# Hongyang-Du/VideoGPA

Measured on AMD Instinct MI355X. Metric: DPO preference-pair steps/sec, CogVideoX-5B 49f@480x720, higher is better.
Workload: dtype bf16; 1 GPU; BASELINE configs[1]: CogVideoX-5B T2V full (42 blocks, D=3072, 48x64 heads), 49f x 480x720 -> paired latents [1,2,13,16,60,90], S=17776 tokens, 42 blocks, LoRA r=64 on to_q/to_k/to_v/to_out.0, 1 pair/GPU/step, optimizer step every step; random-init weights; layers=42, pairs_per_gpu=1, parallelism=dp1

## Files before the change

### include/videogpa_hip.h

```cpp
#ifndef VIDEOGPA_HIP_H
#define VIDEOGPA_HIP_H

#include <stddef.h>
#include <stdint.h>

#ifdef __cplusplus
extern "C" {
#endif

typedef struct ihipStream_t* vgpa_stream_t;

#define VGPA_OK 0
#define VGPA_ERR_INVALID (-1)
#define VGPA_ERR_LAUNCH (-2)
#define VGPA_ERR_WORKSPACE (-3)

size_t vgpa_dpo_loss_workspace_bytes(int64_t B);
int32_t vgpa_dpo_loss_fwd(const void* v_win, const void* v_lose, const void* v_win_ref, const void* v_lose_ref,
                          const void* tgt_win, const void* tgt_lose, int64_t B, int64_t N, int64_t stride_pred,
                          int64_t stride_ref, int64_t stride_tgt, int32_t dtype, float beta, float label_smoothing,
                          int32_t loss_type, int32_t flags, float* out5, float* dlogit, float* errs, void* workspace,
                          size_t ws_bytes, vgpa_stream_t stream);
int32_t vgpa_dpo_loss_bwd(const void* v_win, const void* v_lose, const void* tgt_win, const void* tgt_lose, int64_t B,
                          int64_t N, int64_t stride_pred, int64_t stride_tgt, int64_t stride_grad, int32_t dtype, float beta,
                          int32_t flags, const float* dlogit, const float* grad_out, void* grad_win, void* grad_lose,
                          vgpa_stream_t stream);

int32_t vgpa_noise_velocity_paired(const void* x_pair, const void* noise, const int64_t* t, const float* sqrt_abar,
                                   const float* sqrt_1m_abar, int64_t B, int64_t N, int32_t num_train_timesteps,
                                   int32_t dtype, void* x_noisy_pair, void* v_target_pair, vgpa_stream_t stream);

int32_t vgpa_flow_noise_velocity_paired(const void* x_pair, const void* noise, const float* sigma, int64_t B, int64_t N,
                                        int32_t dtype, int32_t xt_f32, void* x_noisy_pair, void* v_target_pair,
                                        vgpa_stream_t stream);

int32_t vgpa_ln_modulate_fwd(const void* x, const float* ln_w, const float* ln_b, const float* shift_v,
                             const float* scale1p_v, const float* shift_t, const float* scale1p_t, int64_t mod_stride,
                             int64_t B, int64_t S, int64_t D, int64_t text_len, float eps, void* out, float* mean,
                             float* rstd, vgpa_stream_t stream);
int32_t vgpa_ln_modulate_bwd(const void* dy, const void* x, const float* mean, const float* rstd, const float* ln_w,
                             const float* scale1p_v, const float* scale1p_t, int64_t mod_stride, int64_t B, int64_t S,
                             int64_t D, int64_t text_len, const void* dres, void* dx, vgpa_stream_t stream);
int32_t vgpa_residual_ln_fwd(const void* x, const void* y, const float* gate_v, const float* gate_t, int64_t gate_stride,
                             const float* ln_w, const float* ln_b, const float* shift_v, const float* scale1p_v,
                             const float* shift_t, const float* scale1p_t, int64_t mod_stride, int64_t B, int64_t S, int64_t D,
                             int64_t text_len, float eps, void* x_new, void* n_out,
                             int64_t n_stride ,
                             float* mean, float* rstd, vgpa_stream_t stream);
int32_t vgpa_residual_ln_bwd(const void* dn, const void* x_new, const float* mean, const float* rstd, const float* ln_w,
                             const float* scale1p_v, const float* scale1p_t, int64_t mod_stride, const float* gate_v,
                             const float* gate_t, int64_t gate_stride, const void* dres, int64_t B, int64_t S, int64_t D,
                             int64_t text_len, void* dx, void* dy, int64_t dy_stride ,
                             vgpa_stream_t stream);
int32_t vgpa_residual_ln_fwd_q8(const void* x, const void* y, const float* gate_v, const float* gate_t, int64_t gate_stride,
                                const float* ln_w, const float* ln_b, const float* shift_v, const float* scale1p_v,
                                const float* shift_t, const float* scale1p_t, int64_t mod_stride, int64_t B, int64_t S, int64_t D,
                                int64_t text_len, float eps, void* x_new, void* q8, float* q8_scale, float* mean, float* rstd,
                                vgpa_stream_t stream);
int32_t vgpa_residual_ln_bwd_q8(const void* dn, const void* x_new, const float* mean, const float* rstd, const float* ln_w,
                                const float* scale1p_v, const float* scale1p_t, int64_t mod_stride, const float* gate_v,
                                const float* gate_t, int64_t gate_stride, const void* dres, int64_t B, int64_t S, int64_t D,
                                int64_t text_len, void* dx, void* dy_q8, float* dy_scale, vgpa_stream_t stream);
int32_t vgpa_gate_residual(const void* x, const void* y, const float* gate_v, const float* gate_t, int64_t mod_stride,
                           int64_t B, int64_t S, int64_t D, int64_t text_len, void* out, vgpa_stream_t stream);
int32_t vgpa_gelu_tanh_fwd(const void* u, int64_t n, void* out, vgpa_stream_t stream);
int32_t vgpa_gelu_tanh_bwd(const void* u, const void* dy, int64_t n, void* du, vgpa_stream_t stream);

int32_t vgpa_qknorm_rope_fwd(const void* q_in, const void* k_in, void* q_out, void* k_out, const int64_t* qin_strides,
                             const int64_t* kin_strides, const int64_t* qout_strides, const int64_t* kout_strides,
                             const float* wq, const float* bq, const float* wk, const float* bk, const float* rope_cos,
                             const float* rope_sin, int64_t text_len, int64_t B, int64_t H, int64_t S, int64_t head_dim,
                             float eps, float q_out_scale, int32_t rope_mode, vgpa_stream_t stream);
int32_t vgpa_qknorm_rope_bwd(const void* dq_out, const void* dk_out, const void* q_in, const void* k_in, void* dq_in,
                             void* dk_in, const int64_t* dqout_strides, const int64_t* dkout_strides,
                             const int64_t* qin_strides, const int64_t* kin_strides, const int64_t* dqin_strides,
                             const int64_t* dkin_strides, const float* wq, const float* wk, const float* rope_cos,
                             const float* rope_sin, int64_t text_len, int64_t B, int64_t H, int64_t S, int64_t head_dim,
                             float eps, int32_t rope_mode, vgpa_stream_t stream);

int32_t vgpa_attn_bwd_delta_res(const void* o, const void* o_res, int32_t res_kind, const void* d_o, const int64_t* o_strides, const int64_t* ores_strides,
                                const int64_t* do_strides, float* delta, int64_t B, int64_t H, int64_t S, int64_t head_dim,
                                vgpa_stream_t stream);
size_t vgpa_attn_bwd_split_workspace_bytes(int64_t B, int64_t H, int64_t S);
int32_t vgpa_attn_bwd_dq_w1(const void* q, const void* k, const void* v, const void* d_o, const float* lse2, const float* delta,
                            void* dq, const int64_t* q_strides, const int64_t* k_strides, const int64_t* v_strides,
                            const int64_t* do_strides, const int64_t* dq_strides, int64_t B, int64_t H, int64_t S, int64_t head_dim,
                            float scale, int32_t split_mode, void* workspace, size_t ws_bytes, vgpa_stream_t stream);
size_t vgpa_attn_fwd_w1_workspace_bytes(int64_t B, int64_t H, int64_t S);
#define VGPA_RES_NONE 0
#define VGPA_RES_BF16 1
#define VGPA_RES_8 2
int32_t vgpa_attn_fwd_w1_res(const void* q, const void* k, const void* v, void* o, void* o_res, int32_t res_kind, float* lse2, const int64_t* q_strides,
                             const int64_t* k_strides, const int64_t* v_strides, const int64_t* o_strides, const int64_t* ores_strides,
                             int64_t B, int64_t H, int64_t S, int64_t head_dim, float scale, int32_t split_mode, void* workspace,
                             size_t ws_bytes, vgpa_stream_t stream);
int32_t vgpa_attn_fwd_online_res(const void* q, const void* k, const void* v, void* o, void* o_res, int32_t res_kind, float* lse2, const int64_t* q_strides,
                                 const int64_t* k_strides, const int64_t* v_strides, const int64_t* o_strides, const int64_t* ores_strides,
                                 int64_t B, int64_t H, int64_t S, int64_t head_dim, float scale, int32_t split_mode, void* workspace,
                                 size_t ws_bytes, vgpa_stream_t stream);
int32_t vgpa_attn_bwd_prep_w1_res(const void* o, const void* o_res, int32_t res_kind, const void* d_o, const float* lse2, const int64_t* o_strides,
                                  const int64_t* ores_strides, const int64_t* do_strides, float* delta, float* stats, int64_t B, int64_t H,
                                  int64_t S, int64_t head_dim, vgpa_stream_t stream);
int32_t vgpa_attn_bwd_dkv_w1(const void* q, const void* k, const void* v, const void* d_o, const float* stats, void* dk, void* dv,
                             const int64_t* q_strides, const int64_t* k_strides, const int64_t* v_strides, const int64_t* do_strides,
                             const int64_t* dk_strides, const int64_t* dv_strides, int64_t B, int64_t H, int64_t S, int64_t head_dim,
                             float scale, int32_t split_mode, void* workspace, size_t ws_bytes, vgpa_stream_t stream);

int32_t vgpa_lora_down(const void* X, int64_t ldx, const void* A, void* T, int64_t ldt, int64_t M, int64_t K, int64_t R,
                       vgpa_stream_t stream);
int32_t vgpa_lora_up_add(void* Y, int64_t ldy, const void* T, int64_t ldt, const void* Bw, int64_t ldb, float s, int64_t M,
                         int64_t N, int64_t rp, int32_t accumulate, vgpa_stream_t stream);
size_t vgpa_lora_grad_workspace_bytes(int64_t M, int64_t P, int64_t Q);
int32_t vgpa_lora_grad_ws(const void* U, int64_t ldu, const void* V, int64_t ldv, float* G, int64_t ldg, float s, int64_t M,
                          int64_t P, int64_t Q, void* workspace, size_t ws_bytes, vgpa_stream_t stream);
int32_t vgpa_lora_ext_refresh(const float* A, const float* B, float s, int64_t r, int64_t K, int64_t Dn, void* a_cat, void* wt_tail, int64_t ld_wt,
                              void* w_tail, int64_t ld_w, void* sbt, vgpa_stream_t stream);

#ifdef VGPA_VARIANTS
int32_t vgpa_gemm_bf16(const void* X, int64_t ldx, const void* W, int64_t ldw, const void* bias, void* C, int64_t ldc, void* aux,
                       int64_t ldaux, int32_t M, int32_t N, int32_t K, int32_t epilogue, vgpa_stream_t stream);
#endif

size_t vgpa_attn128_fwd_workspace_bytes(int64_t B, int64_t H, int64_t Sq);
int32_t vgpa_attn128_fwd(const void* q, const void* k, const void* v, void* o, float* lse2, const int64_t* q_strides, const int64_t* k_strides,
                         const int64_t* v_strides, const int64_t* o_strides, void* o_res8, const int64_t* ores_strides, int64_t B, int64_t H,
                         int64_t Sq, int64_t Skv, float scale, void* workspace, size_t ws_bytes, vgpa_stream_t stream);
size_t vgpa_attn128_fwd_f8_workspace_bytes(int64_t B, int64_t H, int64_t Sq, int64_t Skv);
int32_t vgpa_attn128_fwd_f8(const void* q, const void* k, const void* v, void* o, float* lse2, const int64_t* q_strides, const int64_t* k_strides,
                            const int64_t* v_strides, const int64_t* o_strides, void* o_res8, const int64_t* ores_strides, void* q_deq, void* k_deq,
                            void* v_deq, const int64_t* qd_strides, const int64_t* kd_strides, const int64_t* vd_strides, int64_t B, int64_t H,
                            int64_t Sq, int64_t Skv, float scale, void* workspace, size_t ws_bytes, vgpa_stream_t stream);
size_t vgpa_attn128_bwd_workspace_bytes(int64_t B, int64_t H, int64_t Sq);
int32_t vgpa_attn128_bwd(const void* q, const void* k, const void* v, const void* o, const void* d_o, const float* lse2, void* dq, void* dk,
                         void* dv, const int64_t* q_strides, const int64_t* k_strides, const int64_t* v_strides,
                         const int64_t* o_strides, const int64_t* do_strides, const int64_t* dq_strides, const int64_t* dk_strides,
                         const int64_t* dv_strides, const void* o_res8, const int64_t* ores_strides, int64_t B, int64_t H, int64_t Sq, int64_t Skv,
                         float scale, int32_t dkv_mode, void* workspace, size_t ws_bytes, vgpa_stream_t stream);
int32_t vgpa_attn128_bwd_prescaled(const void* q, const void* k, const void* v, const void* o, const void* d_o, const float* lse2, void* dq, void* dk,
                                   void* dv, const int64_t* q_strides, const int64_t* k_strides, const int64_t* v_strides,
                                   const int64_t* o_strides, const int64_t* do_strides, const int64_t* dq_strides, const int64_t* dk_strides,
                                   const int64_t* dv_strides, const void* o_res8, const int64_t* ores_strides, int64_t B, int64_t H, int64_t Sq, int64_t Skv,
                                   float scale, int32_t dkv_mode, void* workspace, size_t ws_bytes, vgpa_stream_t stream);

int32_t vgpa_wan_ln_mod_fwd(const void* x, int32_t x_dtype, const void* y, const float* gate, float* x_out, const int32_t* gid, const float* ln_w,
                            const float* ln_b, const float* shift, const float* scale, int64_t mod_stride, int64_t rows, int64_t D, float eps,
                            int32_t round_xhat, void* out, int32_t out_dtype, int64_t out_ld, void* q8, float* q8_scale, float* mean, float* rstd,
                            vgpa_stream_t stream);
int32_t vgpa_wan_ln_mod_bwd(const void* dy, int32_t dy_dtype, const void* x, int32_t x_dtype, const float* mean, const float* rstd, const int32_t* gid,
                            const float* ln_w, const float* scale, int64_t mod_stride, int64_t rows, int64_t D, const float* dres, float* dx,
                            const float* gate_prev, void* dy_prev, int64_t ld_dy_prev, vgpa_stream_t stream);
int32_t vgpa_wan_gate_residual(const float* x, const void* y, const int32_t* gid, const float* gate, int64_t mod_stride, int64_t rows, int64_t D, float* out,
                               vgpa_stream_t stream);
int32_t vgpa_wan_gate_bwd(const float* dout, const int32_t* gid, const float* gate, int64_t mod_stride, int64_t rows, int64_t D, void* dy, int64_t ld_dy,
                          vgpa_stream_t stream);
int32_t vgpa_wan_gate_bwd_q8(const float* dout, const int32_t* gid, const float* gate, int64_t mod_stride, int64_t rows, int64_t D, void* q8,
                             float* q8_scale, vgpa_stream_t stream);
int32_t vgpa_wan_rms_rope_fwd(const void* u, int64_t ld_u, const void* w, const float* rope_cos, const float* rope_sin, int64_t L, int64_t head_dim,
                              int64_t rows, int64_t D, float eps, void* out, int64_t ld_out, float* rstd, vgpa_stream_t stream);
int32_t vgpa_wan_rms_rope_bwd(const void* dout, int64_t ld_dout, const void* u, int64_t ld_u, const float* rstd, const void* w, const float* rope_cos,
                              const float* rope_sin, int64_t L, int64_t head_dim, int64_t rows, int64_t D, void* du, int64_t ld_du, vgpa_stream_t stream);

int32_t vgpa_quant_fp8_rows(const void* x, int64_t ldx, void* q, float* scale, int64_t M, int64_t K, vgpa_stream_t stream);
int32_t vgpa_gelu_tanh_fwd_q8(const void* u, int64_t rows, int64_t K, void* q8, float* q8_scale, vgpa_stream_t stream);
int32_t vgpa_gelu_tanh_bwd_q8(const void* u, const void* dy, int64_t rows, int64_t K, void* q8, float* q8_scale, vgpa_stream_t stream);

int32_t vgpa_preprocess_shape(int32_t H, int32_t W, int32_t mode, int32_t* out_h, int32_t* out_w);
size_t vgpa_preprocess_workspace_bytes(int32_t T, int32_t H, int32_t W, int32_t mode);
int32_t vgpa_preprocess_frames(const void* frames, int32_t T, int32_t H, int32_t W, int32_t mode, float* out, void* workspace,
                               size_t ws_bytes, vgpa_stream_t stream);

size_t vgpa_grad_norm_workspace_bytes(void);
int32_t vgpa_grad_norm(const float* grad, int64_t n, float grad_scale, float* norm_out, void* workspace, size_t ws_bytes,
                       vgpa_stream_t stream);
int32_t vgpa_adamw_step(float* param, const float* grad, float* exp_avg, float* exp_avg_sq, int64_t n, float lr, float beta1,
                        float beta2, float eps, float weight_decay, int64_t step, float grad_scale, float max_norm,
                        const float* total_norm, vgpa_stream_t stream);

size_t vgpa_project_points_workspace_bytes(int64_t T, int64_t H, int64_t W);
int32_t vgpa_project_points(const float* pc, const float* colors, const float* conf, float conf_thr,
                            const float* conf_thr_dev , const float* K,
                            const float* E, int32_t e_rows, int64_t N, int64_t T, int64_t H, int64_t W, uint8_t* canvas,
                            float* out_f, void* workspace, size_t ws_bytes, vgpa_stream_t stream);
int32_t vgpa_motion_score(const float* E, int32_t e_rows, int64_t T, float* out, vgpa_stream_t stream);
int32_t vgpa_epipolar_sampson(const float* p1, const float* p2, const int64_t* offsets, int64_t n_pairs, float* err_out,
                              float* F_out, vgpa_stream_t stream);

size_t vgpa_conf_threshold_workspace_bytes(void);
int32_t vgpa_conf_threshold(const float* conf, int64_t N, float conf_thres, float* thr_out, void* workspace, size_t ws_bytes,
                            vgpa_stream_t stream);
size_t vgpa_frame_metric_workspace_bytes(void);
int32_t vgpa_frame_metric(const void* gt, int32_t gt_dtype, int32_t gt_layout, int32_t gt_is_tensor, const void* rep,
                          int32_t rep_dtype, int32_t rep_layout, int32_t rep_is_tensor, int64_t T, int64_t C, int64_t H,
                          int64_t W, int64_t H2, int64_t W2, int32_t psnr, float* out, void* workspace, size_t ws_bytes,
                          vgpa_stream_t stream);
size_t vgpa_frame_ssim_workspace_bytes(int64_t T, int64_t C, int64_t H, int64_t W);
int32_t vgpa_frame_ssim(const void* gt, int32_t gt_dtype, int32_t gt_layout, int32_t gt_is_tensor, const void* rep, int32_t rep_dtype,
                        int32_t rep_layout, int32_t rep_is_tensor, int64_t T, int64_t C, int64_t H, int64_t W, int32_t downsample,
                        float* out_per_frame, float* out_mean, void* workspace, size_t ws_bytes, vgpa_stream_t stream);
int32_t vgpa_frames_to_pm1(const void* src, int32_t dtype, int32_t layout, int32_t is_tensor, int64_t T, int64_t C, int64_t H,
                           int64_t W, int64_t Ho, int64_t Wo, float* out, void* workspace, size_t ws_bytes, vgpa_stream_t stream);
size_t vgpa_mvcs_workspace_bytes(int64_t T);
int32_t vgpa_mvcs(const float* depth, const float* K, int32_t k_dim, const float* E, int32_t e_rows, int64_t T, int64_t H,
                  int64_t W, float* out, void* workspace, size_t ws_bytes, vgpa_stream_t stream);
int32_t vgpa_unproject_depth(const float* depth, const float* K, const float* E, int32_t e_rows, int64_t T, int64_t H,
                             int64_t W, float* world, vgpa_stream_t stream);
int32_t vgpa_pose_decode(const float* pose_enc, int64_t n, float image_h, float image_w, float* ext, float* intr,
                         vgpa_stream_t stream);

int32_t vgpa_conv3x3_f32(const float* x, const float* w_packed, const float* bias, const float* res, const float* res2, float* out,
                         int64_t N, int64_t H, int64_t W, int64_t Cin, int64_t Cout, int64_t stride, int32_t flags,
                         vgpa_stream_t stream);
int32_t vgpa_conv1x1_f32(const float* x, const float* w_packed, const float* bias, float* out, int64_t M, int64_t Cin, int64_t Cout,
                         vgpa_stream_t stream);
int32_t vgpa_dpt_tail_f32(const float* x, const float* xtab, const float* ytab, const float* w1_packed, const float* b1,
                          const float* w2, const float* b2, float* preds, float* conf, int64_t N, int64_t h, int64_t w, int64_t C,
                          int64_t H, int64_t W, int32_t output_dim, int32_t activation, vgpa_stream_t stream);
int32_t vgpa_upsample_bilinear_ac_f32(const float* x, const float* xtab, const float* ytab, float* out, int64_t N, int64_t h,
                                      int64_t w, int64_t C, int64_t H, int64_t W, vgpa_stream_t stream);
int32_t vgpa_attn_small_f32(const float* q, const float* k, const float* v, int64_t stride_b, int64_t stride_h, int64_t stride_s,
                            float* o, int64_t B, int64_t H, int64_t S, int64_t D, float scale, vgpa_stream_t stream);

int32_t vgpa_dino_embed(const void* images, int32_t in_dtype, const float* w_packed, int64_t k_packed, const float* bias,
                        const float* cls_token, const float* register_tokens, const float* pos, void* out, int32_t out_dtype, int64_t N,
                        int64_t H, int64_t W, int64_t patch, int64_t C, int64_t R, vgpa_stream_t stream);
int32_t vgpa_stream_ln_f32(const float* x, const void* y, const float* gamma, const float* ln_w, const float* ln_b, float* x_new, void* n,
                           int32_t n_dtype, int64_t M, int64_t D, float eps, vgpa_stream_t stream);

int32_t vgpa_lpips_input_f32(const float* x, float* out, int64_t N, int64_t H, int64_t W, float shift0, float shift1, float shift2,
                             float scale0, float scale1, float scale2, int32_t flags, vgpa_stream_t stream);
int32_t vgpa_maxpool2x2_f32(const float* x, float* out, int64_t N, int64_t H, int64_t W, int64_t C, int32_t flags, vgpa_stream_t stream);
size_t vgpa_lpips_layer_workspace_bytes(int64_t N, int64_t H, int64_t W, int64_t C);
int32_t vgpa_lpips_layer_f32(const float* f0, const float* f1, const float* w, float* out, double* total, int64_t N, int64_t H, int64_t W,
                             int64_t C, int32_t flags, void* workspace, size_t ws_bytes, vgpa_stream_t stream);

int32_t vgpa_da3_ref_view(const float* x, int64_t B, int64_t S, int64_t N, int64_t C, int32_t strategy, double* metrics, int32_t* ref_idx,
                          vgpa_stream_t stream);
int32_t vgpa_da3_view_gather(const float* a_in, float* a_out, const float* b_in, float* b_out, const int32_t* ref_idx, int32_t inverse, int64_t B,
                             int64_t S, int64_t N, int64_t C, vgpa_stream_t stream);
int32_t vgpa_da3_cam_token(float* x, const float* cam, int32_t per_view, int64_t B, int64_t S, int64_t N, int64_t C, vgpa_stream_t stream);
int32_t vgpa_da3_tap(const float* local_x, const float* x, const float* ln_w, const float* ln_b, float eps, const int32_t* ref_idx, float* feats,
                     float* cam, int64_t B, int64_t S, int64_t N, int64_t C, vgpa_stream_t stream);
int32_t vgpa_da3_pose_decode(const float* pose_enc, int64_t n, float image_h, float image_w, float* ext, float* intr, vgpa_stream_t stream);
int32_t vgpa_dualdpt_aux_tail_f32(const float* x, const float* xtab, const float* ytab, const float* w1_packed, const float* b1,
                                  const float* ln_w, const float* ln_b, float eps, const float* w2, const float* b2, float* preds, float* conf,
                                  int64_t N, int64_t h, int64_t w, int64_t C, int32_t output_dim, vgpa_stream_t stream);

#ifdef __cplusplus
}
#endif
#endif
```

### videogpa_amd/_lib.py

```python
import ctypes
import os

import torch

from ctypes import c_float, c_int32, c_int64, c_size_t, c_void_p

_HERE = os.path.dirname(os.path.abspath(__file__))
LIB_PATH = os.environ.get("VGPA_LIB") or os.path.join(_HERE, "csrc", "libvgpa_hip.so")

P, I64, I32, F32, SZ = c_void_p, c_int64, c_int32, c_float, c_size_t

SIGNATURES = {
    "vgpa_dpo_loss_workspace_bytes": (SZ, [I64]),
    "vgpa_dpo_loss_fwd": (I32, [P, P, P, P, P, P, I64, I64, I64, I64, I64, I32, F32, F32, I32, I32, P, P, P, P, SZ, P]),
    "vgpa_dpo_loss_bwd": (I32, [P, P, P, P, I64, I64, I64, I64, I64, I32, F32, I32, P, P, P, P, P]),
    "vgpa_noise_velocity_paired": (I32, [P, P, P, P, P, I64, I64, I32, I32, P, P, P]),
    "vgpa_flow_noise_velocity_paired": (I32, [P, P, P, I64, I64, I32, I32, P, P, P]),
    "vgpa_ln_modulate_fwd": (I32, [P, P, P, P, P, P, P, I64, I64, I64, I64, I64, F32, P, P, P, P]),
    "vgpa_ln_modulate_bwd": (I32, [P, P, P, P, P, P, P, I64, I64, I64, I64, I64, P, P, P]),
    "vgpa_residual_ln_fwd": (I32, [P, P, P, P, I64, P, P, P, P, P, P, I64, I64, I64, I64, I64, F32, P, P, I64, P, P, P]),
    "vgpa_residual_ln_bwd": (I32, [P, P, P, P, P, P, P, I64, P, P, I64, P, I64, I64, I64, I64, P, P, I64, P]),
    "vgpa_residual_ln_fwd_q8": (I32, [P, P, P, P, I64, P, P, P, P, P, P, I64, I64, I64, I64, I64, F32, P, P, P, P, P, P]),
    "vgpa_residual_ln_bwd_q8": (I32, [P, P, P, P, P, P, P, I64, P, P, I64, P, I64, I64, I64, I64, P, P, P, P]),
    "vgpa_gate_residual": (I32, [P, P, P, P, I64, I64, I64, I64, I64, P, P]),
    "vgpa_gelu_tanh_fwd": (I32, [P, I64, P, P]),
    "vgpa_gelu_tanh_bwd": (I32, [P, P, I64, P, P]),
    "vgpa_qknorm_rope_fwd": (I32, [P, P, P, P, P, P, P, P, P, P, P, P, P, P, I64, I64, I64, I64, I64, F32, F32, I32, P]),
    "vgpa_qknorm_rope_bwd": (I32, [P, P, P, P, P, P, P, P, P, P, P, P, P, P, P, P, I64, I64, I64, I64, I64, F32, I32, P]),
    "vgpa_grad_norm_workspace_bytes": (SZ, []),
    "vgpa_grad_norm": (I32, [P, I64, F32, P, P, SZ, P]),
    "vgpa_adamw_step": (I32, [P, P, P, P, I64, F32, F32, F32, F32, F32, I64, F32, F32, P, P]),
    "vgpa_attn_bwd_delta_res": (I32, [P, P, I32, P, P, P, P, P, I64, I64, I64, I64, P]),
    "vgpa_attn_bwd_dq_w1": (I32, [P, P, P, P, P, P, P, P, P, P, P, P, I64, I64, I64, I64, F32, I32, P, SZ, P]),
    "vgpa_attn_fwd_w1_workspace_bytes": (SZ, [I64, I64, I64]),
    "vgpa_attn_bwd_prep_w1_res": (I32, [P, P, I32, P, P, P, P, P, P, P, I64, I64, I64, I64, P]),
    "vgpa_attn_fwd_w1_res": (I32, [P, P, P, P, P, I32, P, P, P, P, P, P, I64, I64, I64, I64, F32, I32, P, SZ, P]),
    "vgpa_attn_fwd_online_res": (I32, [P, P, P, P, P, I32, P, P, P, P, P, P, I64, I64, I64, I64, F32, I32, P, SZ, P]),
    "vgpa_attn_bwd_dkv_w1": (I32, [P, P, P, P, P, P, P, P, P, P, P, P, P, I64, I64, I64, I64, F32, I32, P, SZ, P]),
    "vgpa_attn_bwd_split_workspace_bytes": (SZ, [I64, I64, I64]),
    "vgpa_lora_down": (I32, [P, I64, P, P, I64, I64, I64, I64, P]),
    "vgpa_lora_up_add": (I32, [P, I64, P, I64, P, I64, F32, I64, I64, I64, I32, P]),
    "vgpa_lora_grad_workspace_bytes": (SZ, [I64, I64, I64]),
    "vgpa_lora_grad_ws": (I32, [P, I64, P, I64, P, I64, F32, I64, I64, I64, P, SZ, P]),
    "vgpa_lora_ext_refresh": (I32, [P, P, F32, I64, I64, I64, P, P, I64, P, I64, P, P]),
    "vgpa_attn128_fwd_workspace_bytes": (SZ, [I64, I64, I64]),
    "vgpa_attn128_fwd": (I32, [P, P, P, P, P, P, P, P, P, P, P, I64, I64, I64, I64, F32, P, SZ, P]),
    "vgpa_attn128_fwd_f8_workspace_bytes": (SZ, [I64, I64, I64, I64]),
    "vgpa_attn128_fwd_f8": (I32, [P] * 17 + [I64, I64, I64, I64, F32, P, SZ, P]),
    "vgpa_attn128_bwd_workspace_bytes": (SZ, [I64, I64, I64]),
    "vgpa_attn128_bwd": (I32, [P] * 19 + [I64, I64, I64, I64, F32, I32, P, SZ, P]),
    "vgpa_attn128_bwd_prescaled": (I32, [P] * 19 + [I64, I64, I64, I64, F32, I32, P, SZ, P]),
    "vgpa_wan_ln_mod_fwd": (I32, [P, I32, P, P, P, P, P, P, P, P, I64, I64, I64, F32, I32, P, I32, I64, P, P, P, P, P]),
    "vgpa_wan_ln_mod_bwd": (I32, [P, I32, P, I32, P, P, P, P, P, I64, I64, I64, P, P, P, P, I64, P]),
    "vgpa_wan_gate_residual": (I32, [P, P, P, P, I64, I64, I64, P, P]),
    "vgpa_wan_gate_bwd": (I32, [P, P, P, I64, I64, I64, P, I64, P]),
    "vgpa_wan_gate_bwd_q8": (I32, [P, P, P, I64, I64, I64, P, P, P]),
    "vgpa_wan_rms_rope_fwd": (I32, [P, I64, P, P, P, I64, I64, I64, I64, F32, P, I64, P, P]),
    "vgpa_wan_rms_rope_bwd": (I32, [P, I64, P, I64, P, P, P, P, I64, I64, I64, I64, P, I64, P]),
    "vgpa_quant_fp8_rows": (I32, [P, I64, P, P, I64, I64, P]),
    "vgpa_gelu_tanh_fwd_q8": (I32, [P, I64, I64, P, P, P]),
    "vgpa_gelu_tanh_bwd_q8": (I32, [P, P, I64, I64, P, P, P]),
    "vgpa_preprocess_shape": (I32, [I32, I32, I32, P, P]),
    "vgpa_preprocess_workspace_bytes": (SZ, [I32, I32, I32, I32]),
    "vgpa_preprocess_frames": (I32, [P, I32, I32, I32, I32, P, P, SZ, P]),
    "vgpa_project_points_workspace_bytes": (SZ, [I64, I64, I64]),
    "vgpa_project_points": (I32, [P, P, P, F32, P, P, P, I32, I64, I64, I64, I64, P, P, P, SZ, P]),
    "vgpa_conf_threshold_workspace_bytes": (SZ, []),
    "vgpa_conf_threshold": (I32, [P, I64, F32, P, P, SZ, P]),
    "vgpa_frame_metric_workspace_bytes": (SZ, []),
    "vgpa_frame_metric": (I32, [P, I32, I32, I32, P, I32, I32, I32, I64, I64, I64, I64, I64, I64, I32, P, P, SZ, P]),
    "vgpa_frame_ssim_workspace_bytes": (SZ, [I64, I64, I64, I64]),
    "vgpa_frame_ssim": (I32, [P, I32, I32, I32, P, I32, I32, I32, I64, I64, I64, I64, I32, P, P, P, SZ, P]),
    "vgpa_frames_to_pm1": (I32, [P, I32, I32, I32, I64, I64, I64, I64, I64, I64, P, P, SZ, P]),
    "vgpa_mvcs_workspace_bytes": (SZ, [I64]),
    "vgpa_mvcs": (I32, [P, P, I32, P, I32, I64, I64, I64, P, P, SZ, P]),
    "vgpa_unproject_depth": (I32, [P, P, P, I32, I64, I64, I64, P, P]),
    "vgpa_pose_decode": (I32, [P, I64, F32, F32, P, P, P]),
    "vgpa_motion_score": (I32, [P, I32, I64, P, P]),
    "vgpa_epipolar_sampson": (I32, [P, P, P, I64, P, P, P]),
    "vgpa_conv3x3_f32": (I32, [P, P, P, P, P, P, I64, I64, I64, I64, I64, I64, I32, P]),
    "vgpa_conv1x1_f32": (I32, [P, P, P, P, I64, I64, I64, P]),
    "vgpa_dpt_tail_f32": (I32, [P, P, P, P, P, P, P, P, P, I64, I64, I64, I64, I64, I64, I32, I32, P]),
    "vgpa_upsample_bilinear_ac_f32": (I32, [P, P, P, P, I64, I64, I64, I64, I64, I64, P]),
    "vgpa_attn_small_f32": (I32, [P, P, P, I64, I64, I64, P, I64, I64, I64, I64, F32, P]),
    "vgpa_dino_embed": (I32, [P, I32, P, I64, P, P, P, P, P, I32, I64, I64, I64, I64, I64, I64, P]),
    "vgpa_stream_ln_f32": (I32, [P, P, P, P, P, P, P, I32, I64, I64, F32, P]),
    "vgpa_lpips_input_f32": (I32, [P, P, I64, I64, I64, F32, F32, F32, F32, F32, F32, I32, P]),
    "vgpa_maxpool2x2_f32": (I32, [P, P, I64, I64, I64, I64, I32, P]),
    "vgpa_lpips_layer_workspace_bytes": (SZ, [I64, I64, I64, I64]),
    "vgpa_lpips_layer_f32": (I32, [P, P, P, P, P, I64, I64, I64, I64, I32, P, SZ, P]),
    "vgpa_da3_ref_view": (I32, [P, I64, I64, I64, I64, I32, P, P, P]),
    "vgpa_da3_view_gather": (I32, [P, P, P, P, P, I32, I64, I64, I64, I64, P]),
    "vgpa_da3_cam_token": (I32, [P, P, I32, I64, I64, I64, I64, P]),
    "vgpa_da3_tap": (I32, [P, P, P, P, F32, P, P, P, I64, I64, I64, I64, P]),
    "vgpa_da3_pose_decode": (I32, [P, I64, F32, F32, P, P, P]),
    "vgpa_dualdpt_aux_tail_f32": (I32, [P, P, P, P, P, P, P, F32, P, P, P, P, I64, I64, I64, I64, I32, P]),
}

OPTIONAL_SIGNATURES = {
    "vgpa_gemm_bf16": (I32, [P, I64, P, I64, P, P, I64, P, I64, I32, I32, I32, I32, P]),
}

_ERR = {-1: "invalid argument", -2: "kernel launch failed", -3: "workspace too small"}
_lib = None


def load():
    global _lib
    if _lib is None:
        if not os.path.exists(LIB_PATH):
            raise RuntimeError(
                f"videogpa_amd: HIP library not built ({LIB_PATH} missing). Run `python -m videogpa_amd.build` "
                "(or __graft_entry__.build()). There is no CPU / PyTorch fallback.")
        lib = ctypes.CDLL(LIB_PATH)
        for name, (res, args) in SIGNATURES.items():
            fn = getattr(lib, name)
            fn.restype = res
            fn.argtypes = args
        for name, (res, args) in OPTIONAL_SIGNATURES.items():
            fn = getattr(lib, name, None)
            if fn is not None:
                fn.restype = res
                fn.argtypes = args
        _lib = lib
    return _lib


def _conv(a):
    if a is None:
        return None
    if hasattr(a, "data_ptr"):
        return a.data_ptr()
    return a


def call(name, *args):
    fn = getattr(load(), name)
    rc = fn(*[_conv(a) for a in args])
    if rc != 0:
        raise RuntimeError(f"{name} failed: {_ERR.get(rc, rc)}")


def query(name, *args):
    return getattr(load(), name)(*args)


def has(name):
    return hasattr(load(), name)
```

### videogpa_amd/csrc/attention_w1.hip

```cpp
#include <type_traits>

#include "attn_w1.h"

#define W1_DQ_PART_FLOATS (256 * HD)
#define W1_DKV_PART_FLOATS (2 * 256 * HD)

template <bool SPLIT>
__global__ __launch_bounds__(256, 1) void attn_bwd_dq_w1_kernel(const bf16_t* __restrict__ Q, const bf16_t* __restrict__ K,
                                                                  const bf16_t* __restrict__ V, const bf16_t* __restrict__ dO,
                                                                  const float* __restrict__ LSE2, const float* __restrict__ DELTA,
                                                                  bf16_t* __restrict__ dQ, TStride sq, TStride sk, TStride sv, TStride sdo,
                                                                  TStride sdq, int S, int H, int n_qt, float scale, int task0, int nsplit,
                                                                  float* __restrict__ part) {
    constexpr int QB = 2;
    __shared__ __attribute__((aligned(1024))) uint8_t lds[W1_RING_BYTES];
    int vid, chunk;
    w1_task<SPLIT>(task0, nsplit, vid, chunk);
    const int bh = vid / n_qt, qt = vid % n_qt;
    const int b = bh / H, h = bh % H;
    const int lane = threadIdx.x & 63, hi = lane >> 5;
    const int wave = __builtin_amdgcn_readfirstlane((int)threadIdx.x >> 6);
    const int q0 = (qt * 4 + wave) * (32 * QB);

    bf16x8_t qf[QB][4], dof[QB][4];
// ... 424 lines not shown
    const int c8 = (int)(gid & 7);
    float acc = 0.f;
    int64_t bh = 0;
    int q = 0;
    if (row < total) {
        q = (int)(row % S);
        bh = row / S;
        const int h = (int)(bh % H), b = (int)(bh / H);
        float a[8], o[8];
        unpack8(*reinterpret_cast<const u32x4_t*>(dO + ((size_t)b * sdo.b + (size_t)h * sdo.h + (size_t)q * sdo.s + c8 * 8)), a);
        const u32x4_t ob = *reinterpret_cast<const u32x4_t*>(O + ((size_t)b * so.b + (size_t)h * so.h + (size_t)q * so.s + c8 * 8));
        const size_t ro = (size_t)b * sor.b + (size_t)h * sor.h + (size_t)q * sor.s + c8 * 8;
        if (res_kind == VGPA_RES_8) {
            unpack8_res8(ob, *reinterpret_cast<const u32x2_t*>((const uint8_t*)ORES + ro), o);
        } else {
            unpack8(ob, o);
            if (res_kind == VGPA_RES_BF16) {
                float r[8];
                unpack8(*reinterpret_cast<const u32x4_t*>((const bf16_t*)ORES + ro), r);
#pragma unroll
                for (int j = 0; j < 8; ++j) o[j] += r[j];
            }
        }
#pragma unroll
        for (int j = 0; j < 8; ++j) acc += a[j] * o[j];
    }
    acc += __shfl_xor(acc, 1, 64);
    acc += __shfl_xor(acc, 2, 64);
    acc += __shfl_xor(acc, 4, 64);
    if (row < total && c8 == 0) {
        delta[row] = acc;
        stats[bh * 2 * S + q] = -LSE2[row];
        stats[bh * 2 * S + S + q] = -acc;
    }
}

__global__ __launch_bounds__(256) void w1_dq_merge_kernel(const float* __restrict__ part, int nsplit, int task0, int n_qt, int rows_per_task,
                                                            bf16_t* __restrict__ dQ, TStride sdq, int S, int H, float scale) {
    const int lane = threadIdx.x & 63, rows4 = rows_per_task >> 2;
    const int r = ((int)blockIdx.x % rows4) * 4 + (threadIdx.x >> 6), tl = (int)blockIdx.x / rows4;
    const int vid = task0 + tl, bh = vid / n_qt, qt = vid % n_qt;
    const int q = qt * rows_per_task + r;
    if (q >= S) return;
    const float* pb = part + (size_t)tl * nsplit * rows_per_task * HD + r * HD + lane;
    float acc = 0.f;
    for (int c = 0; c < nsplit; ++c) acc += pb[(size_t)c * rows_per_task * HD];
    const int b = bh / H, h = bh % H;
    dQ[(size_t)b * sdq.b + (size_t)h * sdq.h + (size_t)q * sdq.s + lane] = f32_to_bf16(acc * scale);
}

#define W1_MAX_SPLIT 16
static inline int64_t w1_slots() { return wg_slots() / 2; }

extern "C" {


size_t vgpa_attn_bwd_split_workspace_bytes(int64_t B, int64_t H, int64_t S) {
    if (B <= 0 || H <= 0 || S <= 0) return 0;
    const int64_t tasks = (S + 255) / 256 * B * H;
    const size_t part = W1_DKV_PART_FLOATS > W1_DQ_PART_FLOATS ? W1_DKV_PART_FLOATS : W1_DQ_PART_FLOATS;
    return (size_t)max_split_parts(tasks, W1_MAX_SPLIT, w1_slots()) * part * sizeof(float);
}

int32_t vgpa_attn_bwd_dq_w1(const void* q, const void* k, const void* v, const void* d_o, const float* lse2, const float* delta, void* dq,
                            const int64_t* q_strides, const int64_t* k_strides, const int64_t* v_strides, const int64_t* do_strides,
                            const int64_t* dq_strides, int64_t B, int64_t H, int64_t S, int64_t head_dim, float scale, int32_t split_mode,
                            void* workspace, size_t ws_bytes, hipStream_t stream) {
    if (!q || !k || !v || !d_o || !lse2 || !delta || !dq || head_dim != HD || B <= 0 || H <= 0 || S <= 0 || S > (1 << 24)) return VGPA_ERR_INVALID;
    if (!view_ok(q_strides, B, H, S, HD) || !view_ok(k_strides, B, H, S, HD) || !view_ok(v_strides, B, H, S, HD) || !view_ok(do_strides, B, H, S, HD) ||
        !view_ok(dq_strides, B, H, S, HD) || !al16(q) || !al16(k) || !al16(v) || !al16(d_o) || !al16(dq) || (workspace && !al16(workspace)))
        return VGPA_ERR_INVALID;
    const int rows = 256;
    W1Plan pl;
    const int32_t rc = plan_w1(B, H, S, split_mode, W1_MAX_SPLIT, w1_slots(), W1_DQ_PART_FLOATS * sizeof(float), workspace, ws_bytes, 0, &pl);
    if (rc) return rc;
    const int n_t = pl.n_t;
    const TailSplit& p = pl.p;
    if (p.n_main > 0) {
        VGPA_LAUNCH((attn_bwd_dq_w1_kernel<false>), dim3((unsigned)p.n_main), dim3(256), 0, stream, (const bf16_t*)q, (const bf16_t*)k,
                    (const bf16_t*)v, (const bf16_t*)d_o, lse2, delta, (bf16_t*)dq, mk(q_strides), mk(k_strides), mk(v_strides), mk(do_strides),
                    mk(dq_strides), (int)S, (int)H, n_t, scale, 0, 1, (float*)nullptr);
        VGPA_CHECK_LAUNCH();
    }
    if (p.n_tail > 0) {
        VGPA_LAUNCH((attn_bwd_dq_w1_kernel<true>), dim3((unsigned)(p.n_tail * p.nsplit)), dim3(256), 0, stream, (const bf16_t*)q, (const bf16_t*)k,
                    (const bf16_t*)v, (const bf16_t*)d_o, lse2, delta, (bf16_t*)dq, mk(q_strides), mk(k_strides), mk(v_strides), mk(do_strides),
                    mk(dq_strides), (int)S, (int)H, n_t, scale, (int)p.n_main, p.nsplit, (float*)workspace);
        VGPA_CHECK_LAUNCH();
        VGPA_LAUNCH(w1_dq_merge_kernel, dim3((unsigned)(p.n_tail * (rows / 4))), dim3(256), 0, stream, (const float*)workspace, p.nsplit, (int)p.n_main, n_t,
                    rows, (bf16_t*)dq, mk(dq_strides), (int)S, (int)H, scale);
        VGPA_CHECK_LAUNCH();
    }
    return VGPA_OK;
}


int32_t vgpa_attn_bwd_prep_w1_res(const void* o, const void* o_res, int32_t res_kind, const void* d_o, const float* lse2, const int64_t* o_strides,
                                  const int64_t* ores_strides, const int64_t* do_strides, float* delta, float* stats, int64_t B, int64_t H, int64_t S,
                                  int64_t head_dim, hipStream_t stream) {
    if (!o || !d_o || !lse2 || !delta || !stats || head_dim != HD || B <= 0 || H <= 0 || S <= 0 || S > (1 << 24)) return VGPA_ERR_INVALID;
    if (!view_ok(o_strides, B, H, S, HD) || !view_ok(do_strides, B, H, S, HD) || !al16(o) || !al16(d_o)) return VGPA_ERR_INVALID;
    if (o_res && (!view_ok(ores_strides, B, H, S, HD) || !al16(o_res) || (res_kind != VGPA_RES_BF16 && res_kind != VGPA_RES_8))) return VGPA_ERR_INVALID;
    const int64_t total = B * H * S;
    VGPA_LAUNCH(w1_bwd_prep_kernel, dim3((unsigned)((total * 8 + 255) / 256)), dim3(256), 0, stream, (const bf16_t*)d_o, (const bf16_t*)o, lse2,
                mk(do_strides), mk(o_strides), (int)S, (int)H, total, delta, stats, o_res, o_res ? mk(ores_strides) : mk(o_strides),
                o_res ? (int)res_kind : VGPA_RES_NONE);
    VGPA_CHECK_LAUNCH();
    return VGPA_OK;
}

int32_t vgpa_attn_bwd_dkv_w1(const void* q, const void* k, const void* v, const void* d_o, const float* stats, void* dk, void* dv,
                             const int64_t* q_strides, const int64_t* k_strides, const int64_t* v_strides, const int64_t* do_strides,
                             const int64_t* dk_strides, const int64_t* dv_strides, int64_t B, int64_t H, int64_t S, int64_t head_dim, float scale,
                             int32_t split_mode, void* workspace, size_t ws_bytes, hipStream_t stream) {
    (void)scale;
    if (!q || !k || !v || !d_o || !stats || !dk || !dv || head_dim != HD || B <= 0 || H <= 0 || S <= 0 || S > (1 << 24)) return VGPA_ERR_INVALID;
    if (!view_ok(q_strides, B, H, S, HD) || !view_ok(k_strides, B, H, S, HD) || !view_ok(v_strides, B, H, S, HD) || !view_ok(do_strides, B, H, S, HD) ||
        !view_ok(dk_strides, B, H, S, HD) || !view_ok(dv_strides, B, H, S, HD) || !al16(q) || !al16(k) || !al16(v) || !al16(d_o) || !al16(dk) ||
        !al16(dv) || (workspace && !al16(workspace)))
        return VGPA_ERR_INVALID;
    const float kscale = 0.6931471805599453f;
    W1Plan pl;
    const int32_t rc = plan_w1(B, H, S, split_mode, W1_MAX_SPLIT, w1_slots(), W1_DKV_PART_FLOATS * sizeof(float), workspace, ws_bytes, 0, &pl);
    if (rc) return rc;
    const int n_t = pl.n_t;
    const TailSplit& p = pl.p;
    if (p.n_main > 0) {
        VGPA_LAUNCH((attn_bwd_dkv_w1_kernel<false>), dim3((unsigned)p.n_main), dim3(256), 0, stream, (const bf16_t*)q, (const bf16_t*)k, (const bf16_t*)v,
                    (const bf16_t*)d_o, stats, (bf16_t*)dk, (bf16_t*)dv, mk(q_strides), mk(k_strides), mk(v_strides), mk(do_strides), mk(dk_strides),
                    mk(dv_strides), (int)S, (int)H, n_t, kscale, 0, 1, (float*)nullptr);
        VGPA_CHECK_LAUNCH();
    }
    if (p.n_tail > 0) {
        VGPA_LAUNCH((attn_bwd_dkv_w1_kernel<true>), dim3((unsigned)(p.n_tail * p.nsplit)), dim3(256), 0, stream, (const bf16_t*)q, (const bf16_t*)k,
                    (const bf16_t*)v, (const bf16_t*)d_o, stats, (bf16_t*)dk, (bf16_t*)dv, mk(q_strides), mk(k_strides), mk(v_strides), mk(do_strides),
                    mk(dk_strides), mk(dv_strides), (int)S, (int)H, n_t, kscale, (int)p.n_main, p.nsplit, (float*)workspace);
        VGPA_CHECK_LAUNCH();
        VGPA_LAUNCH(w1_dkv_merge_kernel, dim3((unsigned)(p.n_tail * 64)), dim3(256), 0, stream, (const float*)workspace, p.nsplit, (int)p.n_main, n_t,
                    (bf16_t*)dk, (bf16_t*)dv, mk(dk_strides), mk(dv_strides), (int)S, (int)H, kscale);
        VGPA_CHECK_LAUNCH();
    }
    return VGPA_OK;
}


static inline size_t fwd_w1_ws_head(int64_t B, int64_t H, int64_t tasks) { return (((size_t)(B * H) + (size_t)tasks) * 4 + 255) / 256 * 256; }
size_t vgpa_attn_fwd_w1_workspace_bytes(int64_t B, int64_t H, int64_t S) {
    const int64_t tasks = (S + 255) / 256 * B * H;
    return fwd_w1_ws_head(B, H, tasks) + (size_t)max_split_parts(tasks, W1_MAX_SPLIT, w1_slots()) * W1_FWD_PART_FLOATS * sizeof(float);
}
static int32_t fwd_w1_impl(const void* q, const void* k, const void* v, void* o, void* o_res, int32_t res_kind, float* lse2, const int64_t* q_strides,
                           const int64_t* k_strides, const int64_t* v_strides, const int64_t* o_strides, const int64_t* ores_strides, int64_t B,
                           int64_t H, int64_t S, int64_t head_dim, float scale, int32_t split_mode, void* workspace, size_t ws_bytes,
                           hipStream_t stream, bool force_online) {
    (void)scale;
    if (!q || !k || !v || !o || !lse2 || !workspace || head_dim != HD || B <= 0 || H <= 0 || S <= 0 || S > (1 << 24)) return VGPA_ERR_INVALID;
    if (!view_ok(q_strides, B, H, S, HD) || !view_ok(k_strides, B, H, S, HD) || !view_ok(v_strides, B, H, S, HD) || !view_ok(o_strides, B, H, S, HD) ||
        !al16(q) || !al16(k) || !al16(v) || !al16(o) || !al16(workspace))
        return VGPA_ERR_INVALID;
    if (o_res && (!view_ok(ores_strides, B, H, S, HD) || !al16(o_res) || (res_kind != VGPA_RES_BF16 && res_kind != VGPA_RES_8))) return VGPA_ERR_INVALID;
    void* ores = o_res;
    const int rk = o_res ? (int)res_kind : VGPA_RES_NONE;
    const TStride sor = o_res ? mk(ores_strides) : mk(o_strides);
    if (B * H > 65535) return VGPA_ERR_INVALID;
    const size_t head = fwd_w1_ws_head(B, H, (S + 255) / 256 * B * H);
    W1Plan pl;
    const int32_t rc = plan_w1(B, H, S, force_online ? 0 : split_mode, W1_MAX_SPLIT, w1_slots(), W1_FWD_PART_FLOATS * sizeof(float), workspace, ws_bytes, head, &pl);
    if (rc) return rc;
    if (ws_bytes < head) return VGPA_ERR_WORKSPACE;
    const int n_qt = pl.n_t;
    const int64_t tasks = pl.tasks;
    const TailSplit& p = pl.p;
    unsigned* kmax2 = (unsigned*)workspace;
    int* flags = (int*)workspace + B * H;
    float* part = (float*)((char*)workspace + head);
    if (S < W1_FWD_MIN_S || force_online) {
        if (hipMemsetAsync(workspace, 0xff, head, stream) != hipSuccess) return VGPA_ERR_LAUNCH;
        return vgpa_internal_attn_fwd_redo(q, k, v, o, lse2, mk(q_strides), mk(k_strides), mk(v_strides), mk(o_strides), (int)S, (int)H, n_qt, tasks,
                                           flags, stream, ores, sor, rk);
    }
    if (hipMemsetAsync(workspace, 0, head, stream) != hipSuccess) return VGPA_ERR_LAUNCH;
    VGPA_LAUNCH((w1_kmax_kernel<HD / 8>), dim3(16, (unsigned)(B * H)), dim3(256), 0, stream, (const bf16_t*)k, mk(k_strides), (int)S, (int)H, kmax2);
    VGPA_CHECK_LAUNCH();
    if (p.n_main > 0) {
        VGPA_LAUNCH((attn_fwd_w1_kernel<false>), dim3((unsigned)p.n_main), dim3(256), 0, stream, (const bf16_t*)q, (const bf16_t*)k, (const bf16_t*)v,
                    (bf16_t*)o, lse2, (const unsigned*)kmax2, flags, mk(q_strides), mk(k_strides), mk(v_strides), mk(o_strides), (int)S, (int)H, n_qt, 0, 1,
                    (float*)nullptr, ores, sor, rk);
        VGPA_CHECK_LAUNCH();
    }
    if (p.n_tail > 0) {
        VGPA_LAUNCH((attn_fwd_w1_kernel<true>), dim3((unsigned)(p.n_tail * p.nsplit)), dim3(256), 0, stream, (const bf16_t*)q, (const bf16_t*)k,
                    (const bf16_t*)v, (bf16_t*)o, lse2, (const unsigned*)kmax2, flags, mk(q_strides), mk(k_strides), mk(v_strides), mk(o_strides), (int)S,
                    (int)H, n_qt, (int)p.n_main, p.nsplit, part, ores, sor, rk);
        VGPA_CHECK_LAUNCH();
        VGPA_LAUNCH(w1_fwd_merge_kernel, dim3((unsigned)(p.n_tail * 64)), dim3(256), 0, stream, (const float*)part, p.nsplit, (int)p.n_main, n_qt, (bf16_t*)o,
                    mk(o_strides), lse2, flags, (int)S, (int)H, ores, sor, rk);
        VGPA_CHECK_LAUNCH();
    }
    return vgpa_internal_attn_fwd_redo(q, k, v, o, lse2, mk(q_strides), mk(k_strides), mk(v_strides), mk(o_strides), (int)S, (int)H, n_qt, tasks, flags, stream,
                                       ores, sor, rk);
}
int32_t vgpa_attn_fwd_w1_res(const void* q, const void* k, const void* v, void* o, void* o_res, int32_t res_kind, float* lse2, const int64_t* q_strides,
                             const int64_t* k_strides, const int64_t* v_strides, const int64_t* o_strides, const int64_t* ores_strides, int64_t B,
                             int64_t H, int64_t S, int64_t head_dim, float scale, int32_t split_mode, void* workspace, size_t ws_bytes,
                             hipStream_t stream) {
    return fwd_w1_impl(q, k, v, o, o_res, res_kind, lse2, q_strides, k_strides, v_strides, o_strides, ores_strides, B, H, S, head_dim, scale, split_mode, workspace,
                       ws_bytes, stream, false);
}
int32_t vgpa_attn_fwd_online_res(const void* q, const void* k, const void* v, void* o, void* o_res, int32_t res_kind, float* lse2, const int64_t* q_strides,
                                 const int64_t* k_strides, const int64_t* v_strides, const int64_t* o_strides, const int64_t* ores_strides, int64_t B,
                                 int64_t H, int64_t S, int64_t head_dim, float scale, int32_t split_mode, void* workspace, size_t ws_bytes,
                                 hipStream_t stream) {
    return fwd_w1_impl(q, k, v, o, o_res, res_kind, lse2, q_strides, k_strides, v_strides, o_strides, ores_strides, B, H, S, head_dim, scale, split_mode, workspace,
                       ws_bytes, stream, true);
}

}
```

### videogpa_amd/csrc/attn_w1.h

```cpp
#pragma once
#include "attn_common.h"

#define W1_TILE_BYTES 8192
#define W1_SLOT_BYTES (2 * W1_TILE_BYTES)
#define W1_SLOTS 4
#define W1_RING_BYTES (W1_SLOTS * W1_SLOT_BYTES)
#define W1_STAT_BYTES 1024

typedef __attribute__((address_space(3))) bf16x4_t* w1_lds_b64_t;
typedef __attribute__((ext_vector_type(16))) uint32_t u32x16_t;
typedef __attribute__((ext_vector_type(8))) uint32_t u32x8_t;

__device__ __forceinline__ uint32_t w1_swz(uint32_t r) { return (((r >> 1) & 1u) << 2) | (((r >> 2) & 1u) << 1) | ((r >> 3) & 1u); }
__device__ __forceinline__ uint32_t w1h_swz(uint32_t r) { return ((r & 3u) << 2) | ((r >> 2) & 3u); }

template <int D>
struct W1Tile {
    static constexpr uint32_t ROW_BYTES = 2 * D;
    static constexpr uint32_t TILE_BYTES = 64 * ROW_BYTES;
    static constexpr uint32_t SLOT_BYTES = 2 * TILE_BYTES;
    static constexpr uint32_t RING_BYTES = W1_SLOTS * SLOT_BYTES;
    static constexpr int PW = TILE_BYTES / 1024 / 4;
    static constexpr uint32_t CHUNKS = ROW_BYTES / 16;
    static constexpr uint32_t PIECE_ROWS = 64 / CHUNKS;
// ... 80 lines not shown
__device__ __forceinline__ typename W1Tile<D>::table_t w1_read_offsets(int lane, uint32_t base = 0u) {
    typedef W1Tile<D> G;
    typename G::table_t a;
    const uint32_t m = lane & 31, hi = lane >> 5;
#pragma unroll
    for (int ks = 0; ks < G::KS; ++ks) a[ks] = base + m * G::ROW_BYTES + ((((uint32_t)(2 * ks) + hi) ^ G::swz(m)) << 4);
#pragma unroll
    for (int db = 0; db < D / 32; ++db)
#pragma unroll
        for (int r3 = 0; r3 < 2; ++r3) {
            const uint32_t rr = 4u * hi + ((uint32_t)(lane & 15) >> 2) + 8u * r3;
            const uint32_t c = 4u * db + 2u * ((uint32_t)(lane >> 4) & 1u) + (((uint32_t)lane & 3u) >> 1);
            a[G::KS + 2 * db + r3] = base + rr * G::ROW_BYTES + ((c ^ G::swz(rr)) << 4) + ((uint32_t)lane & 1u) * 8u;
        }
    return a;
}

struct W1Lane {
    uint32_t row[4];
    uint32_t tr[2][2];
};
__device__ __forceinline__ W1Lane w1_lane_offsets(int lane) {
    W1Lane a;
    const uint32_t m = lane & 31, hi = lane >> 5;
    const uint32_t sw = w1_swz(m);
#pragma unroll
    for (int ks = 0; ks < 4; ++ks) a.row[ks] = m * 128u + ((((uint32_t)(2 * ks) + hi) ^ sw) << 4);
    const uint32_t r = 4u * hi + ((uint32_t)(lane & 15) >> 2);
#pragma unroll
    for (int db = 0; db < 2; ++db)
#pragma unroll
        for (int r3 = 0; r3 < 2; ++r3) {
            const uint32_t rr = r + 8u * r3;
            const uint32_t c = 4u * db + 2u * ((uint32_t)(lane >> 4) & 1u) + (((uint32_t)lane & 3u) >> 1);
            a.tr[db][r3] = rr * 128u + ((c ^ w1_swz(rr)) << 4) + ((uint32_t)lane & 1u) * 8u;
        }
    return a;
}

__device__ __forceinline__ bf16x8_t w1_frag_row(const uint8_t* lds, uint32_t tile_off, const W1Lane& a, int rb , int ks) {
    return *reinterpret_cast<const bf16x8_t*>(lds + (tile_off + a.row[ks] + 4096u * rb));
}
__device__ __forceinline__ bf16x8_t w1_frag_tr(const uint8_t* lds, uint32_t tile_off, const W1Lane& a, int rb, int cc, int db) {
    const uint32_t o = tile_off + 4096u * rb + 2048u * cc;
    bf16x4_t lo = __builtin_amdgcn_ds_read_tr16_b64_v4bf16((w1_lds_b64_t)(lds + (o + a.tr[db][0])));
    bf16x4_t hi4 = __builtin_amdgcn_ds_read_tr16_b64_v4bf16((w1_lds_b64_t)(lds + (o + a.tr[db][1])));
    bf16x8_t r;
#pragma unroll
    for (int i = 0; i < 4; ++i) { r[i] = lo[i]; r[i + 4] = hi4[i]; }
    return r;
}

__device__ __forceinline__ u32x16_t w1_pack4(const bf16x8_t& a, const bf16x8_t& b, const bf16x8_t& c, const bf16x8_t& d) {
    const u32x4_t w[4] = {__builtin_bit_cast(u32x4_t, a), __builtin_bit_cast(u32x4_t, b), __builtin_bit_cast(u32x4_t, c), __builtin_bit_cast(u32x4_t, d)};
    u32x16_t r;
#pragma unroll
    for (int i = 0; i < 16; ++i) r[i] = w[i >> 2][i & 3];
    return r;
}

template <bool SPLIT>
__device__ __forceinline__ void w1_task(int task0, int nsplit, int& vid, int& chunk) {
    vid = task0 + (SPLIT ? (int)blockIdx.x / nsplit : xcd_remap(blockIdx.x, gridDim.x));
    chunk = SPLIT ? (int)blockIdx.x % nsplit : 0;
}
struct W1Range { int tb, nt; };
__device__ __forceinline__ W1Range w1_split_range(int S, int chunk, int nsplit, bool split) {
    const int nt_all = (S + TILE - 1) / TILE;
    return W1Range{split ? nt_all * chunk / nsplit : 0, split ? nt_all * (chunk + 1) / nsplit : nt_all};
}

__device__ __forceinline__ void w1_store_part_row(float* part, int r, const f32x16_t (&acc)[2], int hi) {
#pragma unroll
    for (int db = 0; db < 2; ++db)
#pragma unroll
        for (int g = 0; g < 4; ++g) {
            const f32x4_t w = {acc[db][4 * g], acc[db][4 * g + 1], acc[db][4 * g + 2], acc[db][4 * g + 3]};
            *reinterpret_cast<f32x4_t*>(part + r * HD + db * 32 + 8 * g + 4 * hi) = w;
        }
}
__device__ __forceinline__ u32x2_t w1_pack_bf16x4(const f32x16_t& a, int g, float scale, float (&x)[4]) {
#pragma unroll
    for (int i = 0; i < 4; ++i) x[i] = a[4 * g + i] * scale;
    u32x2_t w;
    w[0] = pack_bf16x2(x[0], x[1]);
    w[1] = pack_bf16x2(x[2], x[3]);
    return w;
}
__device__ __forceinline__ void w1_store_bf16_row(bf16_t* row, const f32x16_t (&acc)[2], float scale, int hi) {
#pragma unroll
    for (int db = 0; db < 2; ++db)
#pragma unroll
        for (int gp = 0; gp < 2; ++gp) {
            u32x2_t w[2];
            float x[4];
#pragma unroll
            for (int e = 0; e < 2; ++e) w[e] = w1_pack_bf16x4(acc[db], 2 * gp + e, scale, x);
            *reinterpret_cast<u32x4_t*>(row + db * 32 + 8 * (2 * gp + hi)) = pair_rows8(w[0], w[1]);
        }
}

#define W1_L_MIN 7.8886e-31f
#define W1_L_MAX 3.3230699e35f
#define W1_SAMPLE_KEYS 64
#define W1_SAMPLE_UP 64.0f
#define W1_M_MAX 1024.0f

__device__ __forceinline__ bool w1_stats_bad(float l, float M) { return !(l >= W1_L_MIN && l < W1_L_MAX) || !(M <= W1_M_MAX); }
template <int NB>
__device__ __forceinline__ bool w1_strip_bad(float l, float M, const f32x16_t (&o)[NB]) {
    float oabs = 0.f;
#pragma unroll
    for (int db = 0; db < NB; ++db)
#pragma unroll
        for (int i = 0; i < 16; ++i) oabs += fabsf(o[db][i]);
    return w1_stats_bad(l, M) || !(oabs < INFINITY);
}

template <int KS, void (*LOAD)(const bf16_t*, uint32_t, int, int, int, bf16x8_t (&)[KS])>
__device__ __forceinline__ void w1_sampled_max(const bf16_t* Ks, uint32_t row_stride, int S, int lane, const bf16x8_t (&qf)[2][KS], float (&ms)[2]) {
    const uint32_t step = (uint32_t)S / W1_SAMPLE_KEYS;
#pragma unroll
    for (int j = 0; j < 2; ++j) ms[j] = -INFINITY;
#pragma unroll
    for (int kb = 0; kb < W1_SAMPLE_KEYS / 32; ++kb) {
        bf16x8_t kf[KS];
        LOAD(Ks, row_stride * step, 32 * kb, W1_SAMPLE_KEYS, lane, kf);
#pragma unroll
        for (int ks = 0; ks < KS; ++ks) asm volatile("" ::"v"(kf[ks]));
#pragma unroll
        for (int j = 0; j < 2; ++j) {
            f32x16_t acc = {0.f, 0.f, 0.f, 0.f, 0.f, 0.f, 0.f, 0.f, 0.f, 0.f, 0.f, 0.f, 0.f, 0.f, 0.f, 0.f};
#pragma unroll
            for (int ks = 0; ks < KS; ++ks) acc = mfma32(kf[ks], qf[j][ks], acc);
            float m = acc[0];
#pragma unroll
            for (int i = 1; i < 16; ++i) m = fmaxf(m, acc[i]);
            ms[j] = fmaxf(ms[j], fmaxf(m, other_half(m)));
        }
    }
}

template <int LANES_PER_ROW>
__global__ __launch_bounds__(256) void w1_kmax_kernel(const bf16_t* __restrict__ K, TStride sk, int S, int H, unsigned* __restrict__ kmax2) {
    constexpr int SH = LANES_PER_ROW == 8 ? 3 : 4;
    static_assert(LANES_PER_ROW == 1 << SH, "8 or 16 lanes per row");
    const int bh = blockIdx.y, b = bh / H, h = bh % H;
    const bf16_t* Kb = K + ((size_t)b * sk.b + (size_t)h * sk.h);
    float mx = 0.f;
    for (int64_t i = (int64_t)blockIdx.x * 256 + threadIdx.x; i < (int64_t)S * LANES_PER_ROW; i += (int64_t)gridDim.x * 256) {
        const int row = (int)(i >> SH), c = (int)(i & (LANES_PER_ROW - 1));
        float f[8];
        unpack8(*reinterpret_cast<const u32x4_t*>(Kb + ((size_t)row * sk.s + c * 8)), f);
        float a = 0.f;
#pragma unroll
        for (int j = 0; j < 8; ++j) a += f[j] * f[j];
        a += __shfl_xor(a, 1, 64);
        a += __shfl_xor(a, 2, 64);
        a += __shfl_xor(a, 4, 64);
        if (LANES_PER_ROW == 16) a += __shfl_xor(a, 8, 64);
        mx = fmaxf(mx, a);
    }
    mx = wave_max(mx);
    if ((threadIdx.x & 63) == 0) atomicMax(kmax2 + bh, __float_as_uint(mx));
}
```

### videogpa_amd/csrc/common.h

```cpp
#pragma once
#include <hip/hip_runtime.h>
#include <stdint.h>

#define VGPA_OK 0
#define VGPA_ERR_INVALID (-1)
#define VGPA_ERR_LAUNCH (-2)
#define VGPA_ERR_WORKSPACE (-3)

#define VGPA_DTYPE_F32 0
#define VGPA_DTYPE_BF16 1

#define VGPA_LAUNCH(...)                 \
    do {                                 \
        (void)hipGetLastError();         \
        hipLaunchKernelGGL(__VA_ARGS__); \
    } while (0)

#define VGPA_CHECK_LAUNCH()                               \
    do {                                                  \
        if (hipGetLastError() != hipSuccess) return VGPA_ERR_LAUNCH; \
    } while (0)

typedef uint16_t bf16_t;
typedef __attribute__((ext_vector_type(8))) __bf16 bf16x8_t;
typedef __attribute__((ext_vector_type(16))) float f32x16_t;
typedef __attribute__((ext_vector_type(4))) float f32x4_t;
typedef __attribute__((ext_vector_type(4))) uint32_t u32x4_t;
typedef __attribute__((ext_vector_type(2))) uint32_t u32x2_t;

__device__ __forceinline__ float bf16_to_f32(bf16_t h) { return __uint_as_float(((uint32_t)h) << 16); }
__device__ __forceinline__ float bf16lo_to_f32(uint32_t w) { return __uint_as_float(w << 16); }
__device__ __forceinline__ float bf16hi_to_f32(uint32_t w) { return __uint_as_float(w & 0xffff0000u); }

typedef __attribute__((ext_vector_type(2))) float vgpa_f32x2_t;
typedef __attribute__((ext_vector_type(2))) __bf16 vgpa_bf16x2_t;
__device__ __forceinline__ uint32_t pack_bf16x2(float lo, float hi) {
    const vgpa_f32x2_t f = {lo, hi};
    return __builtin_bit_cast(uint32_t, __builtin_convertvector(f, vgpa_bf16x2_t));
}
__device__ __forceinline__ bf16_t f32_to_bf16(float f) { return (bf16_t)(pack_bf16x2(f, 0.f) & 0xffffu); }
__device__ __forceinline__ float round_bf16(float f) { return bf16_to_f32(f32_to_bf16(f)); }

__device__ __forceinline__ void unpack8(const u32x4_t v, float* f) {
#pragma unroll
    for (int i = 0; i < 4; ++i) {
        f[2 * i] = bf16lo_to_f32(v[i]);
        f[2 * i + 1] = bf16hi_to_f32(v[i]);
    }
}
__device__ __forceinline__ u32x4_t pack8(const float* f) {
    u32x4_t v;
#pragma unroll
    for (int i = 0; i < 4; ++i) v[i] = pack_bf16x2(f[2 * i], f[2 * i + 1]);
    return v;
}

#define VGPA_RES_NONE 0
#define VGPA_RES_BF16 1
#define VGPA_RES_8 2
__device__ __forceinline__ uint32_t res8_byte(float x, uint32_t xb ) {
    const uint32_t E = (xb >> 7) & 0xffu;
    const float r = x - __uint_as_float(xb << 16);
    const float t = __builtin_rintf(r * __uint_as_float((269u - E) << 23));
    const int q = E > 15u ? (int)fminf(fmaxf(t, -128.f), 127.f) : 0;
    return (uint32_t)(q + 128);
}
__device__ __forceinline__ uint32_t res8_pack4(const float* x, u32x2_t packed) {
    return res8_byte(x[0], packed[0] & 0xffffu) | (res8_byte(x[1], packed[0] >> 16) << 8) | (res8_byte(x[2], packed[1] & 0xffffu) << 16) |
           (res8_byte(x[3], packed[1] >> 16) << 24);
}
__device__ __forceinline__ float res8_value(uint32_t xb , uint32_t byte) {
    const uint32_t E = (xb >> 7) & 0xffu;
    const float sc = E > 15u ? __uint_as_float((E - 15u) << 23) : 0.f;
    return __uint_as_float(xb << 16) + ((float)byte - 128.f) * sc;
}
__device__ __forceinline__ void unpack8_res8(const u32x4_t v, const u32x2_t r, float* f) {
#pragma unroll
    for (int i = 0; i < 4; ++i) {
        const uint32_t rb = r[i >> 1] >> (16 * (i & 1));
        f[2 * i] = res8_value(v[i] & 0xffffu, rb & 0xffu);
        f[2 * i + 1] = res8_value(v[i] >> 16, (rb >> 8) & 0xffu);
    }
}

__device__ __forceinline__ u32x4_t pair_rows8(u32x2_t even, u32x2_t odd) {
    const auto a = __builtin_amdgcn_permlane32_swap(even[0], odd[0], false, false);
    const auto b = __builtin_amdgcn_permlane32_swap(even[1], odd[1], false, false);
    return u32x4_t{a[0], b[0], a[1], b[1]};
}
__device__ __forceinline__ u32x2_t pair_rows8_dword(uint32_t even, uint32_t odd) {
    const auto a = __builtin_amdgcn_permlane32_swap(even, odd, false, false);
    return u32x2_t{a[0], a[1]};
}

template <typename T>
__device__ __forceinline__ T wave_sum(T v) {
#pragma unroll
    for (int o = 32; o > 0; o >>= 1) v += __shfl_xor(v, o, 64);
    return v;
}
__device__ __forceinline__ float wave_max(float v) {
#pragma unroll
    for (int o = 32; o > 0; o >>= 1) v = fmaxf(v, __shfl_xor(v, o, 64));
    return v;
}

template <typename T>
__device__ __forceinline__ T block_sum(T v, T* smem ) {
    v = wave_sum(v);
    const int lane = threadIdx.x & 63, wid = threadIdx.x >> 6, nw = blockDim.x >> 6;
    __syncthreads();
    if (lane == 0) smem[wid] = v;
    __syncthreads();
    T r = 0;
    for (int i = 0; i < nw; ++i) r += smem[i];
    return r;
}

template <int DT>
__device__ __forceinline__ void load8(const void* base, size_t idx, float* f) {
    if (DT == VGPA_DTYPE_BF16) {
        u32x4_t v = *reinterpret_cast<const u32x4_t*>(reinterpret_cast<const bf16_t*>(base) + idx);
        unpack8(v, f);
    } else {
        const float4* p = reinterpret_cast<const float4*>(reinterpret_cast<const float*>(base) + idx);
        float4 a = p[0], b = p[1];
        f[0] = a.x; f[1] = a.y; f[2] = a.z; f[3] = a.w; f[4] = b.x; f[5] = b.y; f[6] = b.z; f[7] = b.w;
    }
}
template <int DT>
__device__ __forceinline__ void store8(void* base, size_t idx, const float* f) {
    if (DT == VGPA_DTYPE_BF16) {
        *reinterpret_cast<u32x4_t*>(reinterpret_cast<bf16_t*>(base) + idx) = pack8(f);
    } else {
        float4* p = reinterpret_cast<float4*>(reinterpret_cast<float*>(base) + idx);
        p[0] = make_float4(f[0], f[1], f[2], f[3]);
        p[1] = make_float4(f[4], f[5], f[6], f[7]);
    }
}
template <int DT>
struct Raw8;
template <>
struct Raw8<VGPA_DTYPE_BF16> {
    u32x4_t a;
    __device__ __forceinline__ void load(const void* base, size_t idx, bool in) {
        const u32x4_t z = {0u, 0u, 0u, 0u};
        a = in ? *reinterpret_cast<const u32x4_t*>(reinterpret_cast<const bf16_t*>(base) + idx) : z;
    }
    __device__ __forceinline__ void get(float* f) const { unpack8(a, f); }
};
template <>
struct Raw8<VGPA_DTYPE_F32> {
    f32x4_t a, b;
    __device__ __forceinline__ void load(const void* base, size_t idx, bool in) {
        const f32x4_t z = {0.f, 0.f, 0.f, 0.f};
        const f32x4_t* p = reinterpret_cast<const f32x4_t*>(reinterpret_cast<const float*>(base) + idx);
        a = in ? p[0] : z;
        b = in ? p[1] : z;
    }
    __device__ __forceinline__ void get(float* f) const {
        f[0] = a[0]; f[1] = a[1]; f[2] = a[2]; f[3] = a[3]; f[4] = b[0]; f[5] = b[1]; f[6] = b[2]; f[7] = b[3];
    }
};

#define FP8_E4M3_MAX 448.0f
__device__ __forceinline__ float e4m3_row_scale(float amax) { return amax > 0.f ? amax / FP8_E4M3_MAX : 1.f; }
__device__ __forceinline__ void store8_e4m3(uint8_t* row, int i0, const float* v, float sc) {
    float t[8];
#pragma unroll
    for (int j = 0; j < 8; ++j) t[j] = fminf(fmaxf(v[j] / sc, -FP8_E4M3_MAX), FP8_E4M3_MAX);
    u32x2_t w;
    int p = 0;
    p = __builtin_amdgcn_cvt_pk_fp8_f32(t[0], t[1], p, false);
    p = __builtin_amdgcn_cvt_pk_fp8_f32(t[2], t[3], p, true);
    w[0] = (uint32_t)p;
    p = 0;
    p = __builtin_amdgcn_cvt_pk_fp8_f32(t[4], t[5], p, false);
    p = __builtin_amdgcn_cvt_pk_fp8_f32(t[6], t[7], p, true);
    w[1] = (uint32_t)p;
    *reinterpret_cast<u32x2_t*>(row + i0) = w;
}

#define GELU_K1 (-2.302208198f)
#define GELU_K2 (-0.1029432396f)
__device__ __forceinline__ float gelu_sig(float x, float x2) {
    return __builtin_amdgcn_rcpf(1.f + __builtin_amdgcn_exp2f(x * (GELU_K1 + GELU_K2 * x2)));
}
__device__ __forceinline__ float gelu_tanh_value(float x) { return x * gelu_sig(x, x * x); }
__device__ __forceinline__ float gelu_tanh_deriv(float x) {
    const float x2 = x * x, sg = gelu_sig(x, x2);
    const float dz2 = 1.5957691216057308f + 0.2140644488f * x2;
    return sg + x * (sg - sg * sg) * dz2;
}

template <int DT>
__device__ __forceinline__ float load1(const void* base, size_t idx) {
    if (DT == VGPA_DTYPE_BF16) return bf16_to_f32(reinterpret_cast<const bf16_t*>(base)[idx]);
    return reinterpret_cast<const float*>(base)[idx];
}
template <int DT>
__device__ __forceinline__ void store1(void* base, size_t idx, float f) {
    if (DT == VGPA_DTYPE_BF16) reinterpret_cast<bf16_t*>(base)[idx] = f32_to_bf16(f);
    else reinterpret_cast<float*>(base)[idx] = f;
}
```

### videogpa_amd/csrc/lora.hip

```cpp
#include "attn_w1.h"

#ifndef LORA_DOWN_DMA
#define LORA_DOWN_DMA 1
#endif
#ifndef LORA_DOWN_DMA_NCB
#define LORA_DOWN_DMA_NCB 2
#endif
#ifndef LORA_DOWN_NS
#define LORA_DOWN_NS 4
#endif
#ifndef LORA_GRAD_WGS
#define LORA_GRAD_WGS 768
#endif

#include <cstdlib>

__device__ __forceinline__ void tile_load_zfill(const bf16_t* base, int64_t ld, int64_t row0, int64_t nrows, int col0, int ncols,
                                                u32x4_t (&r)[2]) {
#pragma unroll
    for (int j = 0; j < 2; ++j) {
        const int c = threadIdx.x + 256 * j;
        const int64_t row = row0 + (c >> 3);
        const int col = col0 + (c & 7) * 8;
        u32x4_t z = {0u, 0u, 0u, 0u};
        r[j] = (row < nrows && col < ncols) ? *reinterpret_cast<const u32x4_t*>(base + row * ld + col) : z;
    }
}

template <int NCB>
__global__ __launch_bounds__(256) void lora_down_kernel(const bf16_t* __restrict__ X, int64_t ldx, const bf16_t* __restrict__ A,
                                                          bf16_t* __restrict__ T, int64_t ldt, int64_t M, int K, int R) {
    extern __shared__ __attribute__((aligned(16))) bf16_t smem[];
    constexpr int RP = 32 * NCB;
    constexpr int NACC = (NCB + 1) / 2;
    constexpr int BUF = (64 + RP) * PITCH;
    const int lane = threadIdx.x & 63, wave = threadIdx.x >> 6, hi = lane >> 5;
    const int rb = wave & 1, cg = wave >> 1;
    const int64_t row0 = (int64_t)blockIdx.x * 64;

    f32x16_t acc[NACC];
#pragma unroll
    for (int a = 0; a < NACC; ++a)
#pragma unroll
        for (int i = 0; i < 16; ++i) acc[a][i] = 0.f;

    u32x4_t xr[2], ar[NCB];
    auto load = [&](int k0) {
        tile_load_zfill(X, ldx, row0, M, k0, K, xr);
#pragma unroll
        for (int j = 0; j < NCB; ++j) {
            const int c = threadIdx.x + 256 * j;
            const int row = c >> 3;
            u32x4_t z = {0u, 0u, 0u, 0u};
            ar[j] = (row < R) ? *reinterpret_cast<const u32x4_t*>(A + (int64_t)row * K + k0 + (c & 7) * 8) : z;
        }
    };
    auto store = [&](int buf) {
        bf16_t* xl = smem + buf * BUF;
        bf16_t* al = xl + 64 * PITCH;
        tile_store(xl, xr);
#pragma unroll
        for (int j = 0; j < NCB; ++j) {
            const int c = threadIdx.x + 256 * j;
            *reinterpret_cast<u32x4_t*>(al + (c >> 3) * PITCH + (c & 7) * 8) = ar[j];
        }
    };
    const int nk = K / 64;
    load(0);
    store(0);
    __syncthreads();
    for (int t = 0; t < nk; ++t) {
        const bf16_t* xl = smem + (t & 1) * BUF;
        const bf16_t* al = xl + 64 * PITCH;
        if (t + 1 < nk) load((t + 1) * 64);
#pragma unroll
        for (int ks = 0; ks < 4; ++ks) {
            const bf16x8_t xf = frag_row(xl, rb * 32, ks, lane);
#pragma unroll
            for (int a = 0; a < NACC; ++a) {
                const int cb = cg + 2 * a;
                if (cb < NCB) acc[a] = mfma32(frag_row(al, cb * 32, ks, lane), xf, acc[a]);
            }
        }
        if (t + 1 < nk) store((t + 1) & 1);
        __syncthreads();
    }
    const int64_t m = row0 + rb * 32 + (lane & 31);
    if (m < M) {
#pragma unroll
        for (int a = 0; a < NACC; ++a) {
            const int cb = cg + 2 * a;
            if (cb < NCB) {
#pragma unroll
                for (int g = 0; g < 4; ++g) {
                    const int n = cb * 32 + 8 * g + 4 * hi;
                    if (n + 3 < R || n < R) {
                        if (n + 3 < R) {
                            u32x2_t w;
                            w[0] = pack_bf16x2(acc[a][4 * g], acc[a][4 * g + 1]);
                            w[1] = pack_bf16x2(acc[a][4 * g + 2], acc[a][4 * g + 3]);
                            *reinterpret_cast<u32x2_t*>(T + m * ldt + n) = w;
                        } else {
                            for (int i = 0; i < 4; ++i)
                                if (n + i < R) T[m * ldt + n + i] = f32_to_bf16(acc[a][4 * g + i]);
                        }
                    }
                }
            }
        }
    }
}

template <int N>
__device__ __forceinline__ void lora_wait_vm() { asm volatile("s_waitcnt vmcnt(%0) lgkmcnt(0)" ::"n"(N) : "memory"); }

template <int NCB, int NS>
__global__ __launch_bounds__(256) void lora_down_dma_kernel(const bf16_t* __restrict__ X, int64_t ldx, const bf16_t* __restrict__ A, bf16_t* __restrict__ T,
                                                              int64_t ldt, int64_t M, int K, int R) {
    constexpr int RP = 32 * NCB;
    constexpr int NACC = (NCB + 1) / 2;
    constexpr int STAGE = 8192 + RP * 128;
    constexpr int PW = 2 + NCB;
    __shared__ __attribute__((aligned(1024))) uint8_t lds[NS * STAGE];
    const int lane = threadIdx.x & 63, hi = lane >> 5;
    const int wave = __builtin_amdgcn_readfirstlane((int)threadIdx.x >> 6);
    const int rb = wave & 1, cg = wave >> 1;
    const int64_t row0 = (int64_t)blockIdx.x * 64;
    const int64_t rows = (M - row0) < 64 ? (M - row0) : 64;

    const W1Rsrc xrs = w1_rsrc(X + row0 * ldx, (uint32_t)(((rows - 1) * ldx + K) * 2));
    const W1Rsrc ars = w1_rsrc(A, (uint32_t)((int64_t)R * K * 2));
    uint32_t xo[2], ao[NCB];
#pragma unroll
    for (int i = 0; i < 2; ++i) {
        const uint32_t row = 8u * (uint32_t)(wave * 2 + i) + (uint32_t)(lane >> 3);
        xo[i] = (uint32_t)((row * (uint64_t)ldx + (((uint32_t)(lane & 7) ^ w1_swz(row)) * 8u)) * 2u);
    }
#pragma unroll
    for (int i = 0; i < NCB; ++i) {
        const uint32_t row = 8u * (uint32_t)(wave * NCB + i) + (uint32_t)(lane >> 3);
        ao[i] = (row * (uint32_t)K + (((uint32_t)(lane & 7) ^ w1_swz(row)) * 8u)) * 2u;
    }
    const uint32_t lds0 = (uint32_t)(uintptr_t)(__attribute__((address_space(3))) uint8_t*)lds;
    const uint32_t xdst = __builtin_amdgcn_readfirstlane(lds0 + (uint32_t)wave * 2048u);
    const uint32_t adst = __builtin_amdgcn_readfirstlane(lds0 + 8192u + (uint32_t)wave * (uint32_t)NCB * 1024u);
    auto issue = [&](int slot) {
        const uint32_t so = (uint32_t)slot * (uint32_t)STAGE;
#pragma unroll
        for (int i = 0; i < 2; ++i) { w1_dma(xdst + so + 1024u * i, xrs, xo[i], 0u); xo[i] += 128u; }
#pragma unroll
        for (int i = 0; i < NCB; ++i) { w1_dma(adst + so + 1024u * i, ars, ao[i], 0u); ao[i] += 128u; }
    };
    f32x16_t acc[NACC];
#pragma unroll
    for (int a = 0; a < NACC; ++a)
#pragma unroll
        for (int i = 0; i < 16; ++i) acc[a][i] = 0.f;
    const W1Lane la = w1_lane_offsets(lane);
    const int nk = K / 64;
#pragma unroll
    for (int t = 0; t < NS - 1; ++t) issue(t);
    for (int t = 0; t < nk; ++t) {
        lora_wait_vm<PW * (NS - 2)>();
        __syncthreads();
        issue((t + NS - 1) % NS);
        const uint32_t xb = (uint32_t)(t % NS) * (uint32_t)STAGE, ab = xb + 8192u;
#pragma unroll
        for (int ks = 0; ks < 4; ++ks) {
            const bf16x8_t xf = w1_frag_row(lds, xb, la, rb, ks);
#pragma unroll
            for (int a = 0; a < NACC; ++a) {
                const int cb = cg + 2 * a;
                if (cb < NCB) acc[a] = mfma32(w1_frag_row(lds, ab, la, cb, ks), xf, acc[a]);
            }
        }
    }
    lora_wait_vm<0>();
    const int64_t m = row0 + rb * 32 + (lane & 31);
    if (m < M) {
#pragma unroll
        for (int a = 0; a < NACC; ++a) {
            const int cb = cg + 2 * a;
            if (cb < NCB) {
#pragma unroll
                for (int g = 0; g < 4; ++g) {
                    const int n = cb * 32 + 8 * g + 4 * hi;
                    if (n + 3 < R) {
                        u32x2_t w;
                        w[0] = pack_bf16x2(acc[a][4 * g], acc[a][4 * g + 1]);
                        w[1] = pack_bf16x2(acc[a][4 * g + 2], acc[a][4 * g + 3]);
                        *reinterpret_cast<u32x2_t*>(T + m * ldt + n) = w;
                    } else {
                        for (int i = 0; i < 4; ++i)
                            if (n + i < R) T[m * ldt + n + i] = f32_to_bf16(acc[a][4 * g + i]);
                    }
                }
            }
        }
    }
}

#ifndef UP_COLS
#define UP_COLS 128
#endif
#define UP_PITCH (UP_COLS + 4)
template <int KS>
__global__ __launch_bounds__(256) void lora_up_add_kernel(bf16_t* __restrict__ Y, int64_t ldy, const bf16_t* __restrict__ T, int64_t ldt,
                                                            const bf16_t* __restrict__ Bw, int64_t ldb, float s, int64_t M, int N,
                                                            int accumulate) {
    __shared__ __attribute__((aligned(16))) float tile[64 * UP_PITCH];
    const int lane = threadIdx.x & 63, wave = threadIdx.x >> 6, hi = lane >> 5;
    const int64_t m0 = (int64_t)blockIdx.x * 64;
    const int n0 = blockIdx.y * UP_COLS;
    const int rb = wave & 1, cg = wave >> 1;
    int64_t mr = m0 + rb * 32 + (lane & 31);
    mr = mr < M ? mr : M - 1;
    bf16x8_t tf[KS];
#pragma unroll
    for (int ks = 0; ks < KS; ++ks) tf[ks] = *reinterpret_cast<const bf16x8_t*>(T + mr * ldt + ks * 16 + hi * 8);
#pragma unroll
    for (int cbi = 0; cbi < UP_COLS / 64; ++cbi) {
        const int nl = cg * (UP_COLS / 2) + cbi * 32;
        int nrow = n0 + nl + (lane & 31);
        nrow = nrow < N ? nrow : N - 1;
        f32x16_t acc;
#pragma unroll
        for (int i = 0; i < 16; ++i) acc[i] = 0.f;
        const bf16_t* bp = Bw + (int64_t)nrow * ldb + hi * 8;
#pragma unroll
        for (int ks = 0; ks < KS; ++ks) acc = mfma32(*reinterpret_cast<const bf16x8_t*>(bp + ks * 16), tf[ks], acc);
        float* tp = tile + (rb * 32 + (lane & 31)) * UP_PITCH + nl + 4 * hi;
#pragma unroll
        for (int g = 0; g < 4; ++g) {
            f32x4_t v = {s * acc[4 * g], s * acc[4 * g + 1], s * acc[4 * g + 2], s * acc[4 * g + 3]};
            *reinterpret_cast<f32x4_t*>(tp + 8 * g) = v;
        }
    }
    __syncthreads();
#pragma unroll
    for (int j = 0; j < UP_COLS / 32; ++j) {
        const int c = threadIdx.x + 256 * j;
        const int row = c / (UP_COLS / 8), col = (c % (UP_COLS / 8)) * 8;
        const int64_t m = m0 + row;
        if (m < M && n0 + col < N) {
            const float* tp = tile + row * UP_PITCH + col;
            const f32x4_t a0 = *reinterpret_cast<const f32x4_t*>(tp), a1 = *reinterpret_cast<const f32x4_t*>(tp + 4);
            float o[8] = {a0[0], a0[1], a0[2], a0[3], a1[0], a1[1], a1[2], a1[3]};
            bf16_t* yp = Y + m * ldy + n0 + col;
            if (accumulate) {
                float y[8];
                unpack8(*reinterpret_cast<const u32x4_t*>(yp), y);
#pragma unroll
                for (int i = 0; i < 8; ++i) o[i] += y[i];
            }
            *reinterpret_cast<u32x4_t*>(yp) = pack8(o);
        }
    }
}

__global__ __launch_bounds__(256) void lora_grad_kernel(const bf16_t* __restrict__ U, int64_t ldu, const bf16_t* __restrict__ V, int64_t ldv,
                                                          float* __restrict__ G, int64_t ldg, float s, int64_t M, int P, int Q,
                                                          int64_t rows_per_split, int n_qt, float* __restrict__ part) {
    __shared__ __attribute__((aligned(16))) bf16_t lds[4 * TILE_ELEMS];
    const int lane = threadIdx.x & 63, wave = threadIdx.x >> 6, hi = lane >> 5;
    const int pb = wave & 1, qb = wave >> 1;
    const int p0 = (blockIdx.x / n_qt) * 64, q0 = (blockIdx.x % n_qt) * 64;
    const int64_t mbeg = (int64_t)blockIdx.y * rows_per_split;
    int64_t mend = mbeg + rows_per_split;
    mend = mend < M ? mend : M;
    if (mbeg >= mend) return;
    f32x16_t acc;
#pragma unroll
    for (int i = 0; i < 16; ++i) acc[i] = 0.f;
    u32x4_t ur[2], vr[2];
    const int nt = (int)((mend - mbeg + 63) / 64);
    tile_load_zfill(U, ldu, mbeg, mend, p0, P, ur);
    tile_load_zfill(V, ldv, mbeg, mend, q0, Q, vr);
    tile_store(lds, ur);
    tile_store(lds + 2 * TILE_ELEMS, vr);
    __syncthreads();
    for (int t = 0; t < nt; ++t) {
        const bf16_t* ul = lds + (t & 1) * TILE_ELEMS;
        const bf16_t* vl = lds + (2 + (t & 1)) * TILE_ELEMS;
        if (t + 1 < nt) {
            tile_load_zfill(U, ldu, mbeg + (int64_t)(t + 1) * 64, mend, p0, P, ur);
            tile_load_zfill(V, ldv, mbeg + (int64_t)(t + 1) * 64, mend, q0, Q, vr);
        }
#pragma unroll
        for (int kc = 0; kc < 4; ++kc) acc = mfma32(frag_tr(ul, 16 * kc, pb * 32, lane), frag_tr(vl, 16 * kc, qb * 32, lane), acc);
        if (t + 1 < nt) {
            tile_store(lds + ((t + 1) & 1) * TILE_ELEMS, ur);
            tile_store(lds + (2 + ((t + 1) & 1)) * TILE_ELEMS, vr);
        }
        __syncthreads();
    }
    const int q = q0 + qb * 32 + (lane & 31);
    if (q < Q) {
        float* slab = part ? part + (int64_t)blockIdx.y * P * Q : nullptr;
#pragma unroll
        for (int r = 0; r < 16; ++r) {
            const int p = p0 + pb * 32 + acc_row(r, hi);
            if (p < P) {
                if (slab) slab[(int64_t)p * Q + q] = acc[r];
                else atomicAdd(&G[(int64_t)p * ldg + q], s * acc[r]);
            }
        }
    }
}

__global__ __launch_bounds__(256) void lora_grad_merge_kernel(const float* __restrict__ part, int nsplit, float* __restrict__ G, int64_t ldg, float s,
                                                                int P, int Q) {
    const int64_t i = (int64_t)blockIdx.x * 256 + threadIdx.x;
    if (i >= (int64_t)P * Q) return;
    float a = 0.f;
    for (int c = 0; c < nsplit; ++c) a += part[(int64_t)c * P * Q + i];
    G[(i / Q) * ldg + (i % Q)] = s * a;
}

__global__ __launch_bounds__(256) void lora_ext_refresh_kernel(const float* __restrict__ A, const float* __restrict__ B, float s, int r, int K, int Dn,
                                                                 bf16_t* __restrict__ a_cat, bf16_t* __restrict__ wt_tail, int64_t ld_wt,
                                                                 bf16_t* __restrict__ w_tail, int64_t ld_w, bf16_t* __restrict__ sbt) {
    const int64_t idx = (int64_t)blockIdx.x * 256 + threadIdx.x;
    const int64_t na = (int64_t)r * K;
    if (idx < na) {
        const int rr = (int)(idx / K), kk = (int)(idx % K);
        const bf16_t a = f32_to_bf16(A[idx]);
        a_cat[idx] = a;
        wt_tail[(int64_t)kk * ld_wt + rr] = a;
    } else if (idx < na + (int64_t)Dn * r) {
        const int64_t e = idx - na;
        const int n = (int)(e / r), rr = (int)(e % r);
        const bf16_t v = f32_to_bf16(bf16_to_f32(f32_to_bf16(B[e])) * s);
        w_tail[(int64_t)n * ld_w + rr] = v;
        sbt[(int64_t)rr * Dn + n] = v;
    }
}

static inline bool a16(const void* p) { return ((uintptr_t)p & 15) == 0; }

extern "C" {

int32_t vgpa_lora_down(const void* X, int64_t ldx, const void* A, void* T, int64_t ldt, int64_t M, int64_t K, int64_t R, hipStream_t stream) {
    if (!X || !A || !T || M <= 0 || K <= 0 || K % 64 != 0 || R <= 0 || R > 256 || ldx % 8 || ldt % 8 || ldt < R || !a16(X) || !a16(A)) return VGPA_ERR_INVALID;
    if (M > ((int64_t)1 << 31) * 32) return VGPA_ERR_INVALID;
    const int ncb = (int)((R + 31) / 32);
    const dim3 grid((unsigned)((M + 63) / 64));
    constexpr bool dma_off = LORA_DOWN_DMA == 0;
    constexpr int dma_max_ncb = LORA_DOWN_DMA_NCB;
    if (!dma_off && ncb <= dma_max_ncb && (uint64_t)64 * (uint64_t)ldx * 2 + (uint64_t)K * 2 + 1024 < (1ull << 32) && ((uint64_t)R + 8) * (uint64_t)K * 2 + 1024 < (1ull << 32)) {
#define LDD(N, S) VGPA_LAUNCH((lora_down_dma_kernel<N, S>), grid, dim3(256), 0, stream, (const bf16_t*)X, ldx, (const bf16_t*)A, (bf16_t*)T, ldt, M, (int)K, (int)R)
        constexpr int ns = LORA_DOWN_NS;
        switch (ncb * 10 + ns) {
            case 14: LDD(1, 4); break; case 24: LDD(2, 4); break;
            case 13: LDD(1, 3); break; case 23: LDD(2, 3); break;
            case 63: LDD(6, 3); break; case 64: LDD(6, 4); break;
            default: return VGPA_ERR_INVALID;
        }
#undef LDD
        VGPA_CHECK_LAUNCH();
        return VGPA_OK;
    }
    const size_t shmem = (size_t)2 * (64 + 32 * ncb) * PITCH * sizeof(bf16_t);
#define LD(N)                                                                                                                      \
    if (hipFuncSetAttribute((const void*)lora_down_kernel<N>, hipFuncAttributeMaxDynamicSharedMemorySize, (int)shmem) != hipSuccess) \
        return VGPA_ERR_LAUNCH;                                                                                                    \
    VGPA_LAUNCH((lora_down_kernel<N>), grid, dim3(256), shmem, stream, (const bf16_t*)X, ldx, (const bf16_t*)A, (bf16_t*)T, ldt, M, (int)K, (int)R)
    switch (ncb) {
        case 1: LD(1); break; case 2: LD(2); break; case 3: LD(3); break; case 4: LD(4); break;
        case 5: LD(5); break; case 6: LD(6); break; case 7: LD(7); break; case 8: LD(8); break;
        default: return VGPA_ERR_INVALID;
    }
#undef LD
    VGPA_CHECK_LAUNCH();
    return VGPA_OK;
}

int32_t vgpa_lora_up_add(void* Y, int64_t ldy, const void* T, int64_t ldt, const void* Bw, int64_t ldb, float s, int64_t M, int64_t N,
                         int64_t rp, int32_t accumulate, hipStream_t stream) {
    if (!Y || !T || !Bw || M <= 0 || N <= 0 || N % 8 != 0 || ldy % 8 || ldt % 8 || ldb % 8 || !a16(T) || !a16(Bw) || !a16(Y))
        return VGPA_ERR_INVALID;
    const dim3 grid((unsigned)((M + 63) / 64), (unsigned)((N + UP_COLS - 1) / UP_COLS));
#define UP(KS) VGPA_LAUNCH((lora_up_add_kernel<KS>), grid, dim3(256), 0, stream, (bf16_t*)Y, ldy, (const bf16_t*)T, ldt, (const bf16_t*)Bw, ldb, s, M, (int)N, (int)accumulate)
    switch (rp) {
        case 16: UP(1); break; case 32: UP(2); break; case 48: UP(3); break; case 64: UP(4); break;
        case 96: UP(6); break; case 128: UP(8); break; case 192: UP(12); break;
        default: return VGPA_ERR_INVALID;
    }
#undef UP
    VGPA_CHECK_LAUNCH();
    return VGPA_OK;
}

static void lora_grad_plan(int64_t M, int64_t P, int64_t Q, int* n_pt, int* n_qt, int64_t* rows, int64_t* splits) {
    *n_pt = (int)((P + 63) / 64);
    *n_qt = (int)((Q + 63) / 64);
    constexpr int64_t target = LORA_GRAD_WGS;
    int64_t sp = target / ((int64_t)*n_pt * *n_qt);
    if (sp < 1) sp = 1;
    const int64_t max_splits = (M + 255) / 256;
    if (sp > max_splits) sp = max_splits;
    int64_t r = (M + sp - 1) / sp;
    r = (r + 63) / 64 * 64;
    *rows = r;
    *splits = (M + r - 1) / r;
}

size_t vgpa_lora_grad_workspace_bytes(int64_t M, int64_t P, int64_t Q) {
    if (M <= 0 || P <= 0 || Q <= 0) return 0;
    int n_pt, n_qt;
    int64_t rows, splits;
    lora_grad_plan(M, P, Q, &n_pt, &n_qt, &rows, &splits);
    return (size_t)splits * (size_t)P * (size_t)Q * sizeof(float);
}
int32_t vgpa_lora_grad_ws(const void* U, int64_t ldu, const void* V, int64_t ldv, float* G, int64_t ldg, float s, int64_t M, int64_t P,
                          int64_t Q, void* workspace, size_t ws_bytes, hipStream_t stream) {
    if (!U || !V || !G || !workspace || M <= 0 || P <= 0 || Q <= 0 || P % 8 || Q % 8 || ldu % 8 || ldv % 8 || !a16(U) || !a16(V) || !a16(workspace))
        return VGPA_ERR_INVALID;
    int n_pt, n_qt;
    int64_t rows, splits;
    lora_grad_plan(M, P, Q, &n_pt, &n_qt, &rows, &splits);
    if (ws_bytes < (size_t)splits * (size_t)P * (size_t)Q * sizeof(float)) return VGPA_ERR_WORKSPACE;
    VGPA_LAUNCH(lora_grad_kernel, dim3((unsigned)(n_pt * n_qt), (unsigned)splits), dim3(256), 0, stream, (const bf16_t*)U, ldu, (const bf16_t*)V, ldv,
                G, ldg, s, M, (int)P, (int)Q, rows, n_qt, (float*)workspace);
    VGPA_CHECK_LAUNCH();
    VGPA_LAUNCH(lora_grad_merge_kernel, dim3((unsigned)((P * Q + 255) / 256)), dim3(256), 0, stream, (const float*)workspace, (int)splits, G, ldg, s,
                (int)P, (int)Q);
    VGPA_CHECK_LAUNCH();
    return VGPA_OK;
}

int32_t vgpa_lora_ext_refresh(const float* A, const float* B, float s, int64_t r, int64_t K, int64_t Dn, void* a_cat, void* wt_tail, int64_t ld_wt, void* w_tail,
                              int64_t ld_w, void* sbt, hipStream_t stream) {
    if (!A || !B || !a_cat || !wt_tail || !w_tail || !sbt || r <= 0 || K <= 0 || Dn <= 0 || ld_wt < r || ld_w < r) return VGPA_ERR_INVALID;
    const int64_t total = r * K + Dn * r;
    if (total >= ((int64_t)1 << 31)) return VGPA_ERR_INVALID;
    VGPA_LAUNCH(lora_ext_refresh_kernel, dim3((unsigned)((total + 255) / 256)), dim3(256), 0, stream, A, B, s, (int)r, (int)K, (int)Dn, (bf16_t*)a_cat, (bf16_t*)wt_tail,
                ld_wt, (bf16_t*)w_tail, ld_w, (bf16_t*)sbt);
    VGPA_CHECK_LAUNCH();
    return VGPA_OK;
}

}
```

### videogpa_amd/csrc/qknorm.hip

```cpp
#include "common.h"

struct QStride { int64_t b, h, s; };

__device__ __forceinline__ float group8_sum(float v) {
    v += __shfl_xor(v, 1, 64);
    v += __shfl_xor(v, 2, 64);
    v += __shfl_xor(v, 4, 64);
    return v;
}

__global__ __launch_bounds__(256) void qknorm_rope_fwd_kernel(const bf16_t* __restrict__ q_in, const bf16_t* __restrict__ k_in,
                                                                bf16_t* __restrict__ q_out, bf16_t* __restrict__ k_out, QStride si_q,
                                                                QStride si_k, QStride so_q, QStride so_k, const float* __restrict__ wq,
                                                                const float* __restrict__ bq, const float* __restrict__ wk,
                                                                const float* __restrict__ bk, const float* __restrict__ rope_cos,
                                                                const float* __restrict__ rope_sin, int text_len, int B, int H, int S,
                                                                float eps, float q_out_scale, int rope_mode) {
    const int64_t nvec = (int64_t)B * S * H;
    const int64_t gid = (int64_t)blockIdx.x * 256 + threadIdx.x;
    const int64_t vid = gid >> 3;
    const int c8 = (int)(gid & 7);
    if (vid >= 2 * nvec) return;
    const int which = vid >= nvec;
    uint32_t r = (uint32_t)(which ? vid - nvec : vid);
    const int h = (int)(r % (uint32_t)H); r /= (uint32_t)H;
    const int s = (int)(r % (uint32_t)S);
    const int b = (int)(r / (uint32_t)S);
    const bf16_t* ip = which ? (k_in + b * si_k.b + h * si_k.h + (int64_t)s * si_k.s) : (q_in + b * si_q.b + h * si_q.h + (int64_t)s * si_q.s);
    bf16_t* op = which ? (k_out + b * so_k.b + h * so_k.h + (int64_t)s * so_k.s) : (q_out + b * so_q.b + h * so_q.h + (int64_t)s * so_q.s);
    const float* w = which ? wk : wq;
    const float* bb = which ? bk : bq;
    float x[8];
    unpack8(*reinterpret_cast<const u32x4_t*>(ip + c8 * 8), x);
    float sum = 0.f;
#pragma unroll
    for (int j = 0; j < 8; ++j) sum += x[j];
    const float mean = group8_sum(sum) * (1.f / 64.f);
    float sq = 0.f;
#pragma unroll
    for (int j = 0; j < 8; ++j) { const float d = x[j] - mean; sq += d * d; }
    const float rstd = rsqrtf(group8_sum(sq) * (1.f / 64.f) + eps);
    float y[8];
#pragma unroll
    for (int j = 0; j < 8; ++j) y[j] = (x[j] - mean) * rstd * w[c8 * 8 + j] + bb[c8 * 8 + j];
    if (rope_cos && rope_mode == 1) {
        const bool on = s >= text_len;
        const float* cp = rope_cos + (int64_t)(on ? s - text_len : 0) * 64 + c8 * 8;
        const float* sp = rope_sin + (int64_t)(on ? s - text_len : 0) * 64 + c8 * 8;
        const float sgn = (c8 & 2) ? 1.f : -1.f;
#pragma unroll
        for (int j = 0; j < 8; ++j) {
            const float partner = __shfl_xor(y[j], 2, 64);
            if (on) y[j] = y[j] * cp[j] + sgn * partner * sp[j];
        }
    } else if (rope_cos && s >= text_len) {
        const float* cp = rope_cos + (int64_t)(s - text_len) * 64 + c8 * 8;
        const float* sp = rope_sin + (int64_t)(s - text_len) * 64 + c8 * 8;
#pragma unroll
        for (int j = 0; j < 8; j += 2) {
            const float a = y[j], bq2 = y[j + 1];
            y[j] = a * cp[j] - bq2 * sp[j];
            y[j + 1] = bq2 * cp[j + 1] + a * sp[j + 1];
        }
    }
    if (!which) {
#pragma unroll
        for (int j = 0; j < 8; ++j) y[j] *= q_out_scale;
    }
    *reinterpret_cast<u32x4_t*>(op + c8 * 8) = pack8(y);
}

__global__ __launch_bounds__(256) void qknorm_rope_bwd_kernel(const bf16_t* __restrict__ dq_out, const bf16_t* __restrict__ dk_out,
                                                                const bf16_t* __restrict__ q_in, const bf16_t* __restrict__ k_in,
                                                                bf16_t* __restrict__ dq_in, bf16_t* __restrict__ dk_in, QStride sg_q,
                                                                QStride sg_k, QStride si_q, QStride si_k, QStride sd_q, QStride sd_k,
                                                                const float* __restrict__ wq, const float* __restrict__ wk,
                                                                const float* __restrict__ rope_cos, const float* __restrict__ rope_sin,
                                                                int text_len, int B, int H, int S, float eps, int rope_mode) {
    const int64_t nvec = (int64_t)B * S * H;
    const int64_t gid = (int64_t)blockIdx.x * 256 + threadIdx.x;
    const int64_t vid = gid >> 3;
    const int c8 = (int)(gid & 7);
    if (vid >= 2 * nvec) return;
    const int which = vid >= nvec;
    uint32_t r = (uint32_t)(which ? vid - nvec : vid);
    const int h = (int)(r % (uint32_t)H); r /= (uint32_t)H;
    const int s = (int)(r % (uint32_t)S);
    const int b = (int)(r / (uint32_t)S);
    const QStride sg = which ? sg_k : sg_q, si = which ? si_k : si_q, sd = which ? sd_k : sd_q;
    const bf16_t* gp = (which ? dk_out : dq_out) + b * sg.b + h * sg.h + (int64_t)s * sg.s;
    const bf16_t* ip = (which ? k_in : q_in) + b * si.b + h * si.h + (int64_t)s * si.s;
    bf16_t* op = (which ? dk_in : dq_in) + b * sd.b + h * sd.h + (int64_t)s * sd.s;
    const float* w = which ? wk : wq;
    float g[8], x[8];
    unpack8(*reinterpret_cast<const u32x4_t*>(gp + c8 * 8), g);
    unpack8(*reinterpret_cast<const u32x4_t*>(ip + c8 * 8), x);
    if (rope_cos && rope_mode == 1) {
        const bool on = s >= text_len;
        const int64_t row = (int64_t)(on ? s - text_len : 0) * 64;
        const float* cp = rope_cos + row + c8 * 8;
        const float* spp = rope_sin + row + (c8 ^ 2) * 8;
        const float sgn = (c8 & 2) ? -1.f : 1.f;
#pragma unroll
        for (int j = 0; j < 8; ++j) {
            const float partner = __shfl_xor(g[j], 2, 64);
            if (on) g[j] = g[j] * cp[j] + sgn * partner * spp[j];
        }
    } else if (rope_cos && s >= text_len) {
        const float* cp = rope_cos + (int64_t)(s - text_len) * 64 + c8 * 8;
        const float* sp = rope_sin + (int64_t)(s - text_len) * 64 + c8 * 8;
#pragma unroll
        for (int j = 0; j < 8; j += 2) {
            const float d0 = g[j], d1 = g[j + 1];
            g[j] = d0 * cp[j] + d1 * sp[j + 1];
            g[j + 1] = d1 * cp[j + 1] - d0 * sp[j];
        }
    }
    float sum = 0.f;
#pragma unroll
    for (int j = 0; j < 8; ++j) sum += x[j];
    const float mean = group8_sum(sum) * (1.f / 64.f);
    float sq = 0.f;
#pragma unroll
    for (int j = 0; j < 8; ++j) { x[j] -= mean; sq += x[j] * x[j]; }
    const float rstd = rsqrtf(group8_sum(sq) * (1.f / 64.f) + eps);
    float s1 = 0.f, s2 = 0.f;
#pragma unroll
    for (int j = 0; j < 8; ++j) {
        x[j] *= rstd;
        g[j] *= w[c8 * 8 + j];
        s1 += g[j];
        s2 += g[j] * x[j];
    }
    const float c1 = group8_sum(s1) * (1.f / 64.f), c2 = group8_sum(s2) * (1.f / 64.f);
#pragma unroll
    for (int j = 0; j < 8; ++j) g[j] = rstd * (g[j] - c1 - x[j] * c2);
    *reinterpret_cast<u32x4_t*>(op + c8 * 8) = pack8(g);
}

static inline bool qs_ok(const int64_t* st) { return st && (st[0] % 8 == 0) && (st[1] % 8 == 0) && (st[2] % 8 == 0); }
static inline QStride qmk(const int64_t* st) { QStride t; t.b = st[0]; t.h = st[1]; t.s = st[2]; return t; }

extern "C" {

int32_t vgpa_qknorm_rope_fwd(const void* q_in, const void* k_in, void* q_out, void* k_out, const int64_t* qin_strides,
                             const int64_t* kin_strides, const int64_t* qout_strides, const int64_t* kout_strides, const float* wq,
                             const float* bq, const float* wk, const float* bk, const float* rope_cos, const float* rope_sin,
                             int64_t text_len, int64_t B, int64_t H, int64_t S, int64_t head_dim, float eps, float q_out_scale,
                             int32_t rope_mode, hipStream_t stream) {
    if (!q_in || !k_in || !q_out || !k_out || !wq || !bq || !wk || !bk || head_dim != 64 || B <= 0 || H <= 0 || S <= 0) return VGPA_ERR_INVALID;
    if (!qs_ok(qin_strides) || !qs_ok(kin_strides) || !qs_ok(qout_strides) || !qs_ok(kout_strides)) return VGPA_ERR_INVALID;
    if ((rope_cos == nullptr) != (rope_sin == nullptr) || text_len < 0 || text_len > S || (rope_mode != 0 && rope_mode != 1)) return VGPA_ERR_INVALID;
    const int64_t threads = 2 * B * S * H * 8;
    if (2 * B * S * H >= ((int64_t)1 << 31) || threads / 256 >= ((int64_t)1 << 31)) return VGPA_ERR_INVALID;
    VGPA_LAUNCH(qknorm_rope_fwd_kernel, dim3((unsigned)((threads + 255) / 256)), dim3(256), 0, stream, (const bf16_t*)q_in,
                       (const bf16_t*)k_in, (bf16_t*)q_out, (bf16_t*)k_out, qmk(qin_strides), qmk(kin_strides), qmk(qout_strides),
                       qmk(kout_strides), wq, bq, wk, bk, rope_cos, rope_sin, (int)text_len, (int)B, (int)H, (int)S, eps, q_out_scale, (int)rope_mode);
    VGPA_CHECK_LAUNCH();
    return VGPA_OK;
}

int32_t vgpa_qknorm_rope_bwd(const void* dq_out, const void* dk_out, const void* q_in, const void* k_in, void* dq_in, void* dk_in,
                             const int64_t* dqout_strides, const int64_t* dkout_strides, const int64_t* qin_strides,
                             const int64_t* kin_strides, const int64_t* dqin_strides, const int64_t* dkin_strides, const float* wq,
                             const float* wk, const float* rope_cos, const float* rope_sin, int64_t text_len, int64_t B, int64_t H,
                             int64_t S, int64_t head_dim, float eps, int32_t rope_mode, hipStream_t stream) {
    if (!dq_out || !dk_out || !q_in || !k_in || !dq_in || !dk_in || !wq || !wk || head_dim != 64 || B <= 0 || H <= 0 || S <= 0) return VGPA_ERR_INVALID;
    if (!qs_ok(dqout_strides) || !qs_ok(dkout_strides) || !qs_ok(qin_strides) || !qs_ok(kin_strides) || !qs_ok(dqin_strides) || !qs_ok(dkin_strides))
        return VGPA_ERR_INVALID;
    if ((rope_cos == nullptr) != (rope_sin == nullptr) || text_len < 0 || text_len > S || (rope_mode != 0 && rope_mode != 1)) return VGPA_ERR_INVALID;
    const int64_t threads = 2 * B * S * H * 8;
    if (2 * B * S * H >= ((int64_t)1 << 31) || threads / 256 >= ((int64_t)1 << 31)) return VGPA_ERR_INVALID;
    VGPA_LAUNCH(qknorm_rope_bwd_kernel, dim3((unsigned)((threads + 255) / 256)), dim3(256), 0, stream, (const bf16_t*)dq_out,
                       (const bf16_t*)dk_out, (const bf16_t*)q_in, (const bf16_t*)k_in, (bf16_t*)dq_in, (bf16_t*)dk_in, qmk(dqout_strides),
                       qmk(dkout_strides), qmk(qin_strides), qmk(kin_strides), qmk(dqin_strides), qmk(dkin_strides), wq, wk, rope_cos,
                       rope_sin, (int)text_len, (int)B, (int)H, (int)S, eps, (int)rope_mode);
    VGPA_CHECK_LAUNCH();
    return VGPA_OK;
}

}
```

### videogpa_amd/ops.py

```python
import contextlib as _contextlib
import contextvars as _contextvars
import ctypes
import os as _os

import torch

from . import _lib

_DT = {torch.float32: 0, torch.bfloat16: 1}


def _stream():
    return torch.cuda.current_stream().cuda_stream


def _req(t, dtype=None, contiguous=True):
    if not t.is_cuda:
        raise RuntimeError("videogpa_amd ops need GPU tensors (no CPU fallback)")
    if dtype is not None and t.dtype != dtype:
        raise RuntimeError(f"expected {dtype}, got {t.dtype}")
    if contiguous and not t.is_contiguous():
        raise RuntimeError("expected a contiguous tensor")
    return t

# ... 205 lines not shown
    def backward(ctx, dy):
        x, mean, rstd, ln_w, mod = ctx.saved_tensors
        B, S, D = x.shape
        dy = dy.contiguous()
        dx = torch.empty_like(x)
        if mod is not None:
            s1v, s1t, stride = mod[:, 1], mod[:, 3], mod.stride(0)
        else:
            s1v = s1t = None
            stride = 0
        _lib.call("vgpa_ln_modulate_bwd", dy, x, mean, rstd, ln_w, s1v, s1t, stride, B, S, D, ctx.text_len, None, dx, _stream())
        return dx, None, None, None, None, None


def ln_modulate(x, ln_w, ln_b, mod=None, text_len=0, eps=1e-5, n_pad=0):
    return _ResidualLNFn.apply(x, None, None, ln_w, ln_b, mod, text_len, eps, n_pad, 0)[1]


def ln_modulate_recompute(x, ln_w, ln_b, mod=None, text_len=0, eps=1e-5):
    B, S, D = x.shape
    n = torch.empty_like(x)
    mean = torch.empty(B, S, dtype=torch.float32, device=x.device)
    rstd = torch.empty_like(mean)
    sv, s1v, st, s1t, mstride = _mod_ptrs(mod)
    _timed("ln_modulate_fwd", 4.0 * B * S * D, lambda: _lib.call("vgpa_residual_ln_fwd", x, None, None, None, 0, ln_w, ln_b, sv, s1v, st, s1t, mstride, B, S, D,
                                                                  text_len, float(eps), None, n, D, mean, rstd, _stream()), "byte")
    return n


def ln_modulate_v1(x, ln_w, ln_b, mod=None, text_len=0, eps=1e-5):
    return _LNModulateFn.apply(x, ln_w, ln_b, mod, text_len, eps)


def _mod_ptrs(mod):
    if mod is None:
        return None, None, None, None, 0
    return mod[:, 0], mod[:, 1], mod[:, 2], mod[:, 3], mod.stride(0)


class _ResidualLNFn(torch.autograd.Function):

    @staticmethod
    def forward(ctx, x, y, gates, ln_w, ln_b, mod, text_len, eps, n_pad, dy_pad):
        _req(x, torch.bfloat16), _req(ln_w, torch.float32), _req(ln_b, torch.float32)
        B, S, D = x.shape
        n = _padded_empty((B, S), D, n_pad, x.dtype, x.device) if n_pad else _empty_rows(x.shape, x.dtype, x.device)
        mean = torch.empty(B, S, dtype=torch.float32, device=x.device)
        rstd = torch.empty_like(mean)
        sv, s1v, st, s1t, mstride = _mod_ptrs(mod)
        if y is not None:
            _req(y, torch.bfloat16), _req(gates, torch.float32)
            x_new = torch.empty_like(x)
            gv, gt, gstride = gates[:, 0], gates[:, 1], gates.stride(0)
        else:
            x_new, gv, gt, gstride = None, None, None, 0
        _timed("residual_ln_fwd" if y is not None else "ln_modulate_fwd", (8.0 if y is not None else 4.0) * B * S * D,
               lambda: _lib.call("vgpa_residual_ln_fwd", x, y, gv, gt, gstride, ln_w, ln_b, sv, s1v, st, s1t, mstride, B, S, D, text_len,
                                 float(eps), x_new, n, D + n_pad, mean, rstd, _stream()), "byte")
        xs = x if y is None else x_new
        ctx.save_for_backward(xs, mean, rstd, ln_w, mod, gates if y is not None else None)
        ctx.text_len = text_len
        ctx.has_y = y is not None
        ctx.dy_pad = dy_pad
        return x_new, n

    @staticmethod
    def backward(ctx, dx_new, dn):
        xs, mean, rstd, ln_w, mod, gates = ctx.saved_tensors
        B, S, D = xs.shape
        if dn is None:
            dn = torch.zeros_like(xs)
        dn = dn.contiguous()
        dres = None if dx_new is None else dx_new.contiguous()
        dx = torch.empty_like(xs)
        _, s1v, _, s1t, mstride = _mod_ptrs(mod)
        dyp = ctx.dy_pad
        if ctx.has_y:
            dy = _padded_empty((B, S), D, dyp, xs.dtype, xs.device) if dyp else _empty_rows(xs.shape, xs.dtype, xs.device)
            gv, gt, gstride = gates[:, 0], gates[:, 1], gates.stride(0)
        else:
            dy, gv, gt, gstride = None, None, None, 0
        passes = 3 + (1 if dres is not None else 0) + (1 if ctx.has_y else 0)
        _timed("residual_ln_bwd" if ctx.has_y else "ln_modulate_bwd", 2.0 * passes * B * S * D,
               lambda: _lib.call("vgpa_residual_ln_bwd", dn, xs, mean, rstd, ln_w, s1v, s1t, mstride, gv, gt, gstride, dres, B, S, D,
                                 ctx.text_len, dx, dy, D + dyp, _stream()), "byte")
        return dx, dy, None, None, None, None, None, None, None, None


def residual_ln(x, y, gates, ln_w, ln_b, mod=None, text_len=0, eps=1e-5, n_pad=0, dy_pad=0):
    return _ResidualLNFn.apply(x, y, gates, ln_w, ln_b, mod, text_len, eps, n_pad, dy_pad)


class _GateResidualFn(torch.autograd.Function):
    @staticmethod
    def forward(ctx, x, y, gates, text_len):
        _req(x, torch.bfloat16), _req(y, torch.bfloat16), _req(gates, torch.float32)
        B, S, D = x.shape
        out = torch.empty_like(x)
        _lib.call("vgpa_gate_residual", x, y, gates[:, 0], gates[:, 1], gates.stride(0), B, S, D, text_len, out, _stream())
        ctx.save_for_backward(gates)
        ctx.text_len = text_len
        return out

    @staticmethod
    def backward(ctx, dout):
        (gates,) = ctx.saved_tensors
        dout = dout.contiguous()
        B, S, D = dout.shape
        dy = _empty_rows(dout.shape, dout.dtype, dout.device)
        _lib.call("vgpa_gate_residual", None, dout, gates[:, 0], gates[:, 1], gates.stride(0), B, S, D, ctx.text_len, dy, _stream())
        return dout, dy, None, None


def gate_residual(x, y, gates, text_len):
    return _GateResidualFn.apply(x, y, gates, text_len)


class _GeluTanhFn(torch.autograd.Function):
    @staticmethod
    def forward(ctx, u):
        _req(u, torch.bfloat16)
        out = _empty_rows(u.shape, u.dtype, u.device, wide=True)
        _timed("gelu_tanh_fwd", 4.0 * u.numel(), lambda: _lib.call("vgpa_gelu_tanh_fwd", u, u.numel(), out, _stream()), "byte")
        ctx.save_for_backward(u)
        return out

    @staticmethod
    def backward(ctx, dy):
        (u,) = ctx.saved_tensors
        dy = dy.contiguous()
        du = _empty_rows(u.shape, u.dtype, u.device, wide=True)
        _timed("gelu_tanh_bwd", 6.0 * u.numel(), lambda: _lib.call("vgpa_gelu_tanh_bwd", u, dy, u.numel(), du, _stream()), "byte")
        return du


def gelu_tanh(u):
    return _GeluTanhFn.apply(u)


def _pad_rank(r):
    rp = 16
    while rp < r:
        rp *= 2
    return rp


def lora_down(x2, a_cat, out=None):
    M, K = x2.shape
    R = a_cat.shape[0]
    t = torch.empty(M, R, dtype=torch.bfloat16, device=x2.device) if out is None else out
    _timed("lora_down_kernel", 2.0 * M * (K + R), lambda: _lib.call("vgpa_lora_down", x2, x2.stride(0), a_cat, t, t.stride(0), M, K, R, _stream()),
           "byte")
    return t


def lora_up_add(y2, t, bw, s, accumulate=True):
    M, N = y2.shape
    _timed("lora_up_add_kernel", (4.0 if accumulate else 2.0) * M * N + 2.0 * M * t.shape[1],
           lambda: _lib.call("vgpa_lora_up_add", y2, y2.stride(0), t, t.stride(0), bw, bw.stride(0), float(s), M, N, t.shape[1],
                             1 if accumulate else 0, _stream()), "byte")


def lora_grad(u, v, s=1.0):
    M, P = u.shape
    Q = v.shape[1]
    g = torch.empty(P, Q, dtype=torch.float32, device=u.device)
    ws_bytes = _lib.query("vgpa_lora_grad_workspace_bytes", M, P, Q)
    ws = torch.empty(ws_bytes, dtype=torch.uint8, device=u.device)
    _timed("lora_grad_kernel", 2.0 * M * (P + Q), lambda: _lib.call("vgpa_lora_grad_ws", u, u.stride(0), v, v.stride(0), g, Q, float(s), M, P, Q,
                                                                     ws, ws_bytes, _stream()), "byte")
    return g


TUNED_GEMM_FILE = _os.path.join(_os.path.dirname(_os.path.abspath(__file__)), "tuned", "tunableop_gfx950.csv")
_TUNED_GEMMS = None


def use_tuned_gemms(enabled=True, path=None):
    global _TUNED_GEMMS
    import torch.cuda.tunable as tn
    if _os.environ.get("PYTORCH_TUNABLEOP_ENABLED") is not None:
        gpu = torch.cuda.is_available()
        _TUNED_GEMMS = {"enabled": tn.is_enabled() if gpu else False, "file": tn.get_filename() if gpu else None, "entries": None,
                        "note": "PYTORCH_TUNABLEOP_* set by the caller: left as is"}
        return _TUNED_GEMMS
    path = path or TUNED_GEMM_FILE
    if not torch.cuda.is_available():
        _TUNED_GEMMS = {"enabled": False, "file": None, "entries": 0}
        return _TUNED_GEMMS
    if not enabled or not _os.path.isfile(path):
        if _TUNED_GEMMS is not None and _TUNED_GEMMS.get("enabled"):
            tn.enable(False)
        _TUNED_GEMMS = {"enabled": False, "file": None, "entries": 0}
        return _TUNED_GEMMS
    if _TUNED_GEMMS is not None and _TUNED_GEMMS.get("enabled") and _TUNED_GEMMS.get("file") == path:
        return _TUNED_GEMMS
    with open(path) as f:
        entries = sum(1 for ln in f if ln.startswith(("Gemm", "ScaledGemm")))
    tn.enable(True)
    tn.tuning_enable(False)
    tn.record_untuned_enable(False)
    tn.set_filename(path, False)
    _TUNED_GEMMS = {"enabled": True, "file": path, "entries": entries}
    return _TUNED_GEMMS


def tuned_gemms_state():
    return _TUNED_GEMMS


_WT_CACHE = True


def _transposed(W):
    if not _WT_CACHE:
        return None
    c = getattr(W, "_vgpa_wt", None)
    if c is None or c[0] != W._version or c[1].device != W.device or c[1].dtype != W.dtype:
        c = (W._version, W.detach().t().contiguous())
        W._vgpa_wt = c
    return c[1]


GEMM_SPLIT_OVERRIDE = None
GEMM_SPLIT_EXT_ONLY = False
_GEMM_ROWS = _contextvars.ContextVar("vgpa_gemm_rows_per_call", default=0)


@_contextlib.contextmanager
def gemm_rows_per_call(rows):
    tok = _GEMM_ROWS.set(int(rows))
    try:
        yield
    finally:
        _GEMM_ROWS.reset(tok)


def current_gemm_rows():
    return int(GEMM_SPLIT_OVERRIDE) if GEMM_SPLIT_OVERRIDE is not None else _GEMM_ROWS.get()


def _slack_rows(x2):
    base = x2 if x2._base is None else x2._base
    tag = getattr(base, "_vgpa_rows", None)
    if tag is None or x2.dim() != 2 or x2.stride(1) != 1:
        return x2.shape[0]
    rows, Mp, width = tag
    if x2.shape[0] != rows or x2.stride(0) != width or x2.data_ptr() != base.data_ptr() or x2.shape[1] > width:
        return x2.shape[0]
    return Mp


def _linear_rows(x2, W, bias, ext=False, split=0):
    M = x2.shape[0]
    if GEMM_ROW_SLACK and 16384 <= M <= 65536 and x2.is_cuda and x2.dim() == 2 and x2.stride(1) == 1 and (split <= 0 or M % split):
        room = _slack_rows(x2)
        for Mp in (gemm_rows(M, W.shape[0], W.shape[1]), gemm_rows(M)):
            if M < Mp <= room:
                xp = torch.as_strided(x2, (Mp, x2.shape[1]), x2.stride(), x2.storage_offset())
                return torch.nn.functional.linear(xp, W, bias)[:M]
    if split <= 0 or M < 2 * split or M % split or not x2.is_cuda or x2.dim() != 2 or (GEMM_SPLIT_EXT_ONLY and not ext):
        return torch.nn.functional.linear(x2, W, bias)
    out = torch.empty(M, W.shape[0], dtype=x2.dtype, device=x2.device)
    for a in range(0, M, split):
        b = a + split
        if bias is None:
            torch.mm(x2[a:b], W.t(), out=out[a:b])
        else:
            torch.addmm(bias, x2[a:b], W.t(), out=out[a:b])
    return out


def _gemm(x2, W, bias=None, ext=False, split=None):
    split = current_gemm_rows() if split is None else split
    if TIMER is None:
        return _linear_rows(x2, W, bias, ext, split)
    out = []
    _timed("hipblaslt_gemm (vendor)", 2.0 * x2.shape[0] * W.shape[0] * W.shape[1], lambda: out.append(_linear_rows(x2, W, bias, ext, split)))
    return out[0]


def _frozen_dx(dy2, W, split=0):
    Wt = _transposed(W)
    return dy2 @ W if Wt is None else _gemm(dy2, Wt, split=split)


class _FrozenLinearFn(torch.autograd.Function):

    @staticmethod
    def forward(ctx, x, W, bias):
        ctx.save_for_backward(W)
        ctx.rows_per_call = current_gemm_rows()
        return _gemm(x.reshape(-1, x.shape[-1]), W, bias, split=ctx.rows_per_call).view(*x.shape[:-1], W.shape[0])

    @staticmethod
    def backward(ctx, dy):
        (W,) = ctx.saved_tensors
        dy2 = dy.reshape(-1, dy.shape[-1])
        if dy2.stride(1) != 1:
            dy2 = dy2.contiguous()
        return _frozen_dx(dy2, W, ctx.rows_per_call).view(*dy.shape[:-1], W.shape[1]), None, None


def frozen_linear(x, W, bias):
    if W.requires_grad or (bias is not None and bias.requires_grad):
        return torch.nn.functional.linear(x, W, bias)
# ... 148 lines not shown
def _fp8_gemm(xq, sx, wq, sw, bias=None):
    M, N, K = xq.shape[0], wq.shape[0], xq.shape[1]
    out = []

    _timed("hipblaslt_gemm_fp8 (vendor)", 2.0 * M * N * K,
           lambda: out.append(torch._scaled_mm(xq, wq.t(), scale_a=sx, scale_b=sw, bias=bias, out_dtype=torch.bfloat16)))
    return out[0]


class _Fp8FrozenLinearFn(torch.autograd.Function):
    @staticmethod
    def forward(ctx, x, W, bias):
        w8 = Fp8Weight.of(W)
        x2 = x.reshape(-1, x.shape[-1])
        if x2.stride(1) != 1:
            x2 = x2.contiguous()
        xq, sx = quant_fp8_rows(x2)
        ctx.w8 = w8
        return _fp8_gemm(xq, sx, w8.q, w8.s, bias).view(*x.shape[:-1], W.shape[0])

    @staticmethod
    def backward(ctx, dy):
        w8 = ctx.w8
        dy2 = dy.reshape(-1, dy.shape[-1])
        if dy2.stride(1) != 1:
            dy2 = dy2.contiguous()
        dq, sd = quant_fp8_rows(dy2)
        return _fp8_gemm(dq, sd, w8.qt, w8.st).view(*dy.shape[:-1], w8.qt.shape[0]), None, None


def frozen_linear_fp8(x, W, bias):
    if W.requires_grad or (bias is not None and bias.requires_grad):
        raise RuntimeError("videogpa_amd: the fp8 path is for frozen projections only")
    if x.dtype != torch.bfloat16:
        raise TypeError("frozen_linear_fp8: bf16 activations")
    return _Fp8FrozenLinearFn.apply(x, W, bias)


class _FfnTailFp8Fn(torch.autograd.Function):

    @staticmethod
    def forward(ctx, x, a, gates1, ln_w, ln_b, mod2, W1, b1, W2, b2, gates2, nxt_w, nxt_b, nxt_mod, nxt_eps, text_len, eps, n_pad, dy_pad):
        _req(x, torch.bfloat16), _req(a, torch.bfloat16), _req(gates1, torch.float32), _req(gates2, torch.float32)
        _req(ln_w, torch.float32), _req(ln_b, torch.float32), _req(nxt_w, torch.float32), _req(nxt_b, torch.float32)
        B, S, D = x.shape
        rows, dev = B * S, x.device
        keep = any(ctx.needs_input_grad)
        w1, w2 = Fp8Weight.of(W1), Fp8Weight.of(W2)
        x1 = torch.empty_like(x)
        hq = torch.empty(rows, D, dtype=torch.float8_e4m3fn, device=dev)
        hs = torch.empty(rows, 1, dtype=torch.float32, device=dev)
        mean1 = torch.empty(B, S, dtype=torch.float32, device=dev) if keep else None
        rstd1 = torch.empty_like(mean1) if keep else None
        sv, s1v, st, s1t, mstride = _mod_ptrs(mod2)
        _timed("residual_ln_fwd_fp8", 7.0 * rows * D,
               lambda: _lib.call("vgpa_residual_ln_fwd_q8", x, a, gates1[:, 0], gates1[:, 1], gates1.stride(0), ln_w, ln_b, sv, s1v, st, s1t, mstride,
                                 B, S, D, text_len, float(eps), x1, hq, hs, mean1, rstd1, _stream()), "byte")
        u = _fp8_gemm(hq, hs, w1.q, w1.s, b1)
        del hq, hs
        gq, gs = gelu_tanh_fwd_q8(u)
        f = _fp8_gemm(gq, gs, w2.q, w2.s, b2)
        del gq, gs
        x2 = torch.empty_like(x)
        n = _padded_empty((B, S), D, n_pad, x.dtype, dev) if n_pad else _empty_rows(x.shape, x.dtype, dev)
        mean2 = torch.empty(B, S, dtype=torch.float32, device=dev) if keep else None
        rstd2 = torch.empty_like(mean2) if keep else None
        nv, n1v, nt, n1t, nstride = _mod_ptrs(nxt_mod)
        _timed("residual_ln_fwd", 8.0 * rows * D,
               lambda: _lib.call("vgpa_residual_ln_fwd", x1, f, gates2[:, 0], gates2[:, 1], gates2.stride(0), nxt_w, nxt_b, nv, n1v, nt, n1t, nstride,
                                 B, S, D, text_len, float(nxt_eps), x2, n, D + n_pad, mean2, rstd2, _stream()), "byte")
        if keep:
            ctx.save_for_backward(x1, mean1, rstd1, u, x2, mean2, rstd2, ln_w, mod2, gates1, nxt_w, nxt_mod, gates2)
            ctx.w, ctx.text_len, ctx.dy_pad = (w1, w2), text_len, dy_pad
        return x2, n

    @staticmethod
    def backward(ctx, dx2, dn):
        x1, mean1, rstd1, u, x2, mean2, rstd2, ln_w, mod2, gates1, nxt_w, nxt_mod, gates2 = ctx.saved_tensors
        w1, w2 = ctx.w
        B, S, D = x1.shape
        rows, dev = B * S, x1.device
        dn = torch.zeros_like(x2) if dn is None else dn.contiguous()
        dres = None if dx2 is None else dx2.contiguous()
        dx1 = torch.empty_like(x1)
        dfq = torch.empty(rows, D, dtype=torch.float8_e4m3fn, device=dev)
        dfs = torch.empty(rows, 1, dtype=torch.float32, device=dev)
        _, n1v, _, n1t, nstride = _mod_ptrs(nxt_mod)
        _timed("residual_ln_bwd_fp8", (7.0 + (2.0 if dres is not None else 0.0)) * rows * D,
               lambda: _lib.call("vgpa_residual_ln_bwd_q8", dn, x2, mean2, rstd2, nxt_w, n1v, n1t, nstride, gates2[:, 0], gates2[:, 1], gates2.stride(0),
                                 dres, B, S, D, ctx.text_len, dx1, dfq, dfs, _stream()), "byte")
        dg = _fp8_gemm(dfq, dfs, w2.qt, w2.st)
        del dfq, dfs
        duq, dus = gelu_tanh_bwd_q8(u, dg)
        del dg
        dh = _fp8_gemm(duq, dus, w1.qt, w1.st)
        del duq, dus
        dx = torch.empty_like(x1)
        dyp = ctx.dy_pad
        da = _padded_empty((B, S), D, dyp, x1.dtype, dev) if dyp else _empty_rows(x1.shape, x1.dtype, dev)
        _, s1v, _, s1t, mstride = _mod_ptrs(mod2)
        _timed("residual_ln_bwd", 10.0 * rows * D,
               lambda: _lib.call("vgpa_residual_ln_bwd", dh, x1, mean1, rstd1, ln_w, s1v, s1t, mstride, gates1[:, 0], gates1[:, 1], gates1.stride(0),
                                 dx1, B, S, D, ctx.text_len, dx, da, D + dyp, _stream()), "byte")
        return (dx, da) + (None,) * 17


def ffn_tail_fp8(x, a, gates1, ln_w, ln_b, mod2, W1, b1, W2, b2, gates2, nxt_w, nxt_b, nxt_mod=None, nxt_eps=1e-5, text_len=0, eps=1e-5, n_pad=0, dy_pad=0):
    if W1.requires_grad or W2.requires_grad or (b1 is not None and b1.requires_grad) or (b2 is not None and b2.requires_grad):
        raise RuntimeError("videogpa_amd: the fp8 path is for frozen projections only")
    if W1.shape[0] > 16384:
        raise RuntimeError(f"ffn_tail_fp8: the GELU -> e4m3 kernels hold one feed-forward row per workgroup, inner <= 16384; got {W1.shape[0]}")
    return _FfnTailFp8Fn.apply(x, a, gates1, ln_w, ln_b, mod2, W1, b1, W2, b2, gates2, nxt_w, nxt_b, nxt_mod, nxt_eps, int(text_len), eps, int(n_pad),
                               int(dy_pad))


class _LinearLoraExtFn(torch.autograd.Function):

    @staticmethod
    def forward(ctx, x, bias, ext, enabled, scalings, x_recompute, *AB):
        K, R, N = ext.K, ext.R, ext.N
        x2 = x.reshape(-1, K)
        M = x2.shape[0]
        x_ext = _padded_base(x2, K + R)
        if x_ext is None:
            x_ext = torch.zeros(M, K + R, dtype=x.dtype, device=x.device) if not enabled else torch.empty(M, K + R, dtype=x.dtype, device=x.device)
            x_ext[:, :K].copy_(x2)
        xv, tv = x_ext[:, :K], x_ext[:, K:]
        if enabled:
            lora_down(xv, ext.A_cat, out=tv)
        ctx.rows_per_call = current_gemm_rows()
        y = _gemm(x_ext, ext.W_ext, bias, ext=True, split=ctx.rows_per_call)
        if x_recompute is not None and enabled:
            fn, srcs = x_recompute
            ctx.save_for_backward(tv.contiguous(), *srcs)
            ctx.x_fn = fn
        else:
            ctx.save_for_backward(x_ext)
            ctx.x_fn = None
        ctx.ext, ctx.enabled, ctx.xshape, ctx.scalings = ext, enabled, x.shape, scalings
        return y.view(*x.shape[:-1], N)

    @staticmethod
    def backward(ctx, dy):
        ext, enabled = ctx.ext, ctx.enabled
        saved, *srcs = ctx.saved_tensors
        K, R, N, Dn, rp, r, act = ext.K, ext.R, ext.N, ext.Dn, ext.rp, ext.r, ext.act
        dy2 = dy.reshape(-1, N)
        M = dy2.shape[0]
        dy_ext = _padded_base(dy2, N + R) if dy2.stride(1) == 1 else None
        if dy_ext is None:
            dy_ext = torch.zeros(M, N + R, dtype=dy.dtype, device=dy.device) if not enabled else torch.empty(M, N + R, dtype=dy.dtype, device=dy.device)
            dy_ext[:, :N].copy_(dy2)
        if enabled:
            for j, i in enumerate(act):
                lora_down(dy_ext[:, i * Dn:(i + 1) * Dn], ext.sBt[j], out=dy_ext[:, N + j * rp:N + (j + 1) * rp])
        dx = _gemm(dy_ext, ext.Wt_ext, ext=True, split=ctx.rows_per_call)
        out_grads = [None] * len(ctx.needs_input_grad[6:])
        if enabled:
            if ctx.x_fn is not None:
                t_all, xh = saved, ctx.x_fn(*srcs).reshape(M, K)
            else:
                t_all, xh = saved[:, K:], saved[:, :K]
            for j, i in enumerate(act):
                out_grads[2 * i + 1] = lora_grad(dy_ext[:, i * Dn:(i + 1) * Dn], t_all[:, j * rp:(j + 1) * rp], ctx.scalings[j])[:, :r]
            dA = lora_grad(dy_ext[:, N:], xh)
            for j, i in enumerate(act):
                out_grads[2 * i] = dA[j * rp:j * rp + r]
        return (dx.view(ctx.xshape), None, None, None, None, None, *out_grads)


def linear_lora_ext(x, W, bias, ext, loras, enabled=True, x_recompute=None):
    if W.requires_grad or (bias is not None and bias.requires_grad):
        raise RuntimeError("videogpa_amd: base weights are frozen on this path (LoRA-only training, as in the reference)")
    ext.refresh(W, len(loras), loras)
    flat = []
    for l in loras:
        flat += [None, None] if l is None else [l[0], l[1]]
    return _LinearLoraExtFn.apply(x, bias, ext, bool(enabled), tuple(float(loras[i][2]) for i in ext.act), x_recompute, *flat)


def linear_lora(x, W, bias, loras, ext=None):
    if all(l is None for l in loras):
        return frozen_linear(x, W, bias)
    if ext is None:
        ext = getattr(W, "_vgpa_lora_ext", None)
        if ext is None:
            ext = LoraExt()
            W._vgpa_lora_ext = ext
    return linear_lora_ext(x, W, bias, ext, loras, True)


def _bhs_strides(t):
    assert t.stride(3) == 1
    return _i64x3(t.stride(0), t.stride(1), t.stride(2))


LOG2E = 1.4426950408889634
ATTN_SPLIT_MODE = -1
def precise_delta_default():
    v = _os.environ.get("VGPA_PRECISE_DELTA", "int8").lower()
    if v in ("0", "off", "none", "false"):
        return None
    if v in ("1", "int8", "res8", "true"):
        return "int8"
    if v == "bf16":
        return "bf16"
    raise ValueError(f"VGPA_PRECISE_DELTA={v!r}: expected 0 | off | int8 | bf16")


def _res_kind(o_res):
    if o_res is None:
        return 0
    if o_res.dtype == torch.bfloat16:
        return 1
    if o_res.dtype == torch.uint8:
        return 2
    raise TypeError(f"o_res: bf16 (rounding residual) or uint8 (eight further mantissa bits), got {o_res.dtype}")


def res8_decode(o, o_res8):
    E = (o.contiguous().view(torch.int16).to(torch.int32) >> 7) & 0xFF
    sc = torch.where(E > 15, torch.ldexp(torch.ones((), device=o.device), E - 142), torch.zeros((), device=o.device))
    return o.float() + (o_res8.float() - 128.0) * sc


def prescale_q(q, scale=None):
    scale = q.shape[-1] ** -0.5 if scale is None else scale
    return (q.float() * (scale * LOG2E)).to(q.dtype)


class AttnFwdPolicy:
    SWITCH, CHECKS, RECHECK = 0.5, 2, 1024

    def __init__(self, mode="bound", fixed=False):
        self.mode, self.fixed = mode, fixed
        self.calls = 0
        self.redo_fraction = None
        self.switched_at = None

    def wants_flags(self):
        return self.mode == "bound" and not self.fixed and (self.calls < self.CHECKS or self.calls % self.RECHECK == 0)

    def observe(self, fraction):
        self.redo_fraction = fraction
        if not self.fixed and fraction > self.SWITCH:
            self.mode, self.switched_at = "online", self.calls


def _strip_flags(ws, head_words, B, H, Sq):
    strips = (Sq + 255) // 256
    return ws[:4 * (head_words + B * H * strips)].view(torch.int32)[head_words:].view(B, H, strips)


def attention_redo_fraction(ws, B, H, S):
    return float((_strip_flags(ws, B * H, B, H, S) != 0).float().mean())


def attention_fwd_raw(q, k, v, scale=None, q_prescaled=False, split_mode=None, o_pad=0, o_res=None, policy=None):
    B, H, S, Dh = q.shape
    scale = Dh ** -0.5 if scale is None else scale
    if not q_prescaled:
        q = prescale_q(q, scale)
    o = _padded_empty((B, S), H * Dh, o_pad, torch.bfloat16, q.device) if o_pad else torch.empty(B, S, H * Dh, dtype=torch.bfloat16, device=q.device)
    lse = torch.empty(B, H, S, dtype=torch.float32, device=q.device)
    ov = o.unflatten(-1, (H, Dh)).permute(0, 2, 1, 3)
    split_mode = ATTN_SPLIT_MODE if split_mode is None else split_mode
    ws_bytes = _lib.query("vgpa_attn_fwd_w1_workspace_bytes", B, H, S)
    ws = torch.empty(ws_bytes, dtype=torch.uint8, device=q.device)
    rv = None if o_res is None else o_res.unflatten(-1, (H, Dh)).permute(0, 2, 1, 3)
    entry = "vgpa_attn_fwd_online_res" if (policy is not None and policy.mode == "online") else "vgpa_attn_fwd_w1_res"
    _timed("attn_fwd_kernel", 4.0 * S * S * Dh * B * H, lambda: _lib.call(
        entry, q, k, v, o, o_res, _res_kind(o_res), lse, _bhs_strides(q), _bhs_strides(k), _bhs_strides(v), _bhs_strides(ov), None if rv is None else _bhs_strides(rv),
        B, H, S, Dh, float(scale), int(split_mode), ws, ws_bytes, _stream()))
    if policy is not None:
        if policy.wants_flags() and not torch.cuda.is_current_stream_capturing():
            policy.observe(attention_redo_fraction(ws, B, H, S))
        policy.calls += 1
    return o, lse


def attention_bwd_raw(q, k, v, o, do, lse, dq, dk, dv, scale=None, q_prescaled=False, split_mode=None, o_res=None):
    B, H, S, Dh = q.shape
    scale = Dh ** -0.5 if scale is None else scale
    if not q_prescaled:
        q = prescale_q(q, scale)
    delta = torch.empty(B, H, S, dtype=torch.float32, device=q.device)
    st = _stream()
    stats = torch.empty(B, H, 2, S, dtype=torch.float32, device=q.device)
    _timed("attn_delta_kernel", (4.0 + (0 if o_res is None else o_res.element_size())) * B * H * S * Dh, lambda: _lib.call(
        "vgpa_attn_bwd_prep_w1_res", o, o_res, _res_kind(o_res), do, lse, _bhs_strides(o), None if o_res is None else _bhs_strides(o_res), _bhs_strides(do),
        delta, stats, B, H, S, Dh, st), "byte")
    split_mode = ATTN_SPLIT_MODE if split_mode is None else split_mode
    ws_bytes = _lib.query("vgpa_attn_bwd_split_workspace_bytes", B, H, S) if split_mode != 0 else 0
    ws = torch.empty(max(ws_bytes, 16), dtype=torch.uint8, device=q.device)
    wsp = ws if ws_bytes else None
    _timed("attn_bwd_dkv_kernel", 6.0 * S * S * Dh * B * H, lambda: _lib.call(
        "vgpa_attn_bwd_dkv_w1", q, k, v, do, stats, dk, dv, _bhs_strides(q), _bhs_strides(k), _bhs_strides(v), _bhs_strides(do),
        _bhs_strides(dk), _bhs_strides(dv), B, H, S, Dh, float(scale), int(split_mode), wsp, ws_bytes, st))
    _timed("attn_bwd_dq_kernel", 2.0 * S * S * Dh * B * H, lambda: _lib.call(
        "vgpa_attn_bwd_dq_w1", q, k, v, do, lse, delta, dq, _bhs_strides(q), _bhs_strides(k), _bhs_strides(v), _bhs_strides(do),
        _bhs_strides(dq), B, H, S, Dh, float(scale), int(split_mode), wsp, ws_bytes, st))


ATTN128_W1 = True


ATTN128_F8_MIN_KEYS = 1024


def attention128_uses_f8(f8, Skv):
    return bool(f8) and Skv >= ATTN128_F8_MIN_KEYS


class F8AttnPolicy:
    ERR_PER_BOUND = 0.004

    def __init__(self, mode="f8", fixed=False, threshold=0.5):
        self.mode, self.fixed, self.threshold = mode, fixed, float(threshold)
        self.decided = False
        self.estimated_score_error = None

    def reset(self):
        self.decided = False

    @staticmethod
    def score_error_estimate(q, k, H, scale):
        B, Lq, D = q.shape
        d = D // H
        qn = q.view(B, Lq, H, d).float().pow(2).sum(-1).amax(dim=1).sqrt()
        kn = k.view(B, k.shape[1], H, d).float().pow(2).sum(-1).amax(dim=1).sqrt()
        return float((qn * kn).amax()) * float(scale) * LOG2E * F8AttnPolicy.ERR_PER_BOUND

    def use_f8(self, q, k, H, scale):
        if not self.fixed and not self.decided and self.mode == "f8":
            self.estimated_score_error = self.score_error_estimate(q, k, H, scale)
            if self.estimated_score_error > self.threshold:
                self.mode = "bf16"
        self.decided = True
        return self.mode == "f8"


def attention128_f8_redo_fraction(ws, B, H, Sq):
    return float((_strip_flags(ws, 5 * B * H, B, H, Sq) != 0).float().mean())


def attention128_fwd_raw(q, k, v, scale, o_pad=0, f8=False, o_res8=None, deq=None, report=None):
    B, H, Sq, D = q.shape
    Skv = k.shape[2]
    assert D == 128 and k.shape == (B, H, Skv, 128) and v.shape == k.shape and q.dtype == k.dtype == v.dtype == torch.bfloat16
    o2 = _padded_empty((B, Sq), H * D, o_pad, torch.bfloat16, q.device) if o_pad else torch.empty(B, Sq, H * D, dtype=torch.bfloat16, device=q.device)
    o = o2.unflatten(-1, (H, D)).permute(0, 2, 1, 3)
    lse = torch.empty(B, H, Sq, dtype=torch.float32, device=q.device)
    rv = rs = None
    if o_res8 is not None:
        if o_res8.dtype != torch.uint8 or o_res8.shape != (B, Sq, H * D) or not o_res8.is_contiguous():
            raise TypeError("attention128_fwd_raw: o_res8 is a contiguous uint8 [B, Sq, H*128] buffer")
        rv = o_res8.unflatten(-1, (H, D)).permute(0, 2, 1, 3)
        rs = _bhs_strides(rv)
    if attention128_uses_f8(f8, Skv):
        ws_bytes = _lib.query("vgpa_attn128_fwd_f8_workspace_bytes", B, H, Sq, Skv)
        ws = torch.empty(ws_bytes, dtype=torch.uint8, device=q.device)
        dv_ = [None] * 3
        if deq is not None:
            for t, S_ in zip(deq, (Sq, Skv, Skv)):
                if t.dtype != torch.bfloat16 or t.shape != (B, S_, H * D) or not t.is_contiguous():
                    raise TypeError("attention128_fwd_raw: deq = three contiguous bf16 [B, S, H*128] buffers (q, k, v)")
            dv_ = [t.unflatten(-1, (H, D)).permute(0, 2, 1, 3) for t in deq]
        ds_ = [None if t is None else _bhs_strides(t) for t in dv_]
        _timed("attn128_fwd_f8", 4.0 * B * H * Sq * Skv * D, lambda: _lib.call(
            "vgpa_attn128_fwd_f8", q, k, v, o, lse, _bhs_strides(q), _bhs_strides(k), _bhs_strides(v), _bhs_strides(o), rv, rs, dv_[0], dv_[1], dv_[2],
            ds_[0], ds_[1], ds_[2], B, H, Sq, Skv, float(scale), ws, ws_bytes, _stream()))
        if report is not None:
            report["redo_fraction"] = attention128_f8_redo_fraction(ws, B, H, Sq)
            report["strip_flags"] = _strip_flags(ws, 5 * B * H, B, H, Sq) != 0
        return o, lse
    if deq is not None:
        raise ValueError("attention128_fwd_raw: deq buffers are written by the e4m3 forward only (f8=True and at least ATTN128_F8_MIN_KEYS keys)")
    ws_bytes = _lib.query("vgpa_attn128_fwd_workspace_bytes", B, H, Sq) if ATTN128_W1 else 0
    ws = torch.empty(ws_bytes, dtype=torch.uint8, device=q.device) if ws_bytes else None
    _timed("attn128_fwd" if Skv >= 1024 else "attn128_fwd (short keys)", 4.0 * B * H * Sq * Skv * D, lambda: _lib.call(
        "vgpa_attn128_fwd", q, k, v, o, lse, _bhs_strides(q), _bhs_strides(k), _bhs_strides(v), _bhs_strides(o), rv, rs, B, H, Sq, Skv, float(scale),
        ws, ws_bytes, _stream()))
    return o, lse


def attention128_bwd_raw(q, k, v, o, do, lse, dq, dk, dv, scale, o_res8=None, q_prescaled=False):
    B, H, Sq, D = q.shape
    Skv = k.shape[2]
    rv = None if o_res8 is None else o_res8.unflatten(-1, (H, D)).permute(0, 2, 1, 3)
    ws_bytes = _lib.query("vgpa_attn128_bwd_workspace_bytes", B, H, Sq)
    ws = torch.empty(ws_bytes, dtype=torch.uint8, device=q.device)
    _timed("attn128_bwd" if Skv >= 1024 else "attn128_bwd (short keys)", 8.0 * B * H * Sq * Skv * D, lambda: _lib.call(
        "vgpa_attn128_bwd_prescaled" if q_prescaled else "vgpa_attn128_bwd", q, k, v, o, do, lse, dq, dk, dv, _bhs_strides(q), _bhs_strides(k), _bhs_strides(v), _bhs_strides(o), _bhs_strides(do),
        _bhs_strides(dq), _bhs_strides(dk), _bhs_strides(dv), rv, None if rv is None else _bhs_strides(rv), B, H, Sq, Skv, float(scale),
        -1 if ATTN128_W1 else 0, ws, ws_bytes, _stream()))


class _Attention128Fn(torch.autograd.Function):

    @staticmethod
    def forward(ctx, q, k, v, scale, o_pad, precise_delta):
        q, k, v = (t if t.stride(3) == 1 else t.contiguous() for t in (q, k, v))
        o_res8 = None
        if precise_delta and any(ctx.needs_input_grad[:3]):
            o_res8 = torch.empty(q.shape[0], q.shape[2], q.shape[1] * q.shape[3], dtype=torch.uint8, device=q.device)
        o, lse = attention128_fwd_raw(q, k, v, scale, o_pad, o_res8=o_res8)
        ctx.save_for_backward(q, k, v, o, lse, o_res8)
        ctx.scale = float(scale)
        return o

    @staticmethod
    def backward(ctx, do):
        q, k, v, o, lse, o_res8 = ctx.saved_tensors
        B, H, Sq, D = q.shape
        Skv = k.shape[2]
        do = do if do.stride(3) == 1 else do.contiguous()
        dq = torch.empty(B, Sq, H, D, dtype=torch.bfloat16, device=q.device).permute(0, 2, 1, 3)
        dk = torch.empty(B, Skv, H, D, dtype=torch.bfloat16, device=q.device).permute(0, 2, 1, 3)
        dv = torch.empty(B, Skv, H, D, dtype=torch.bfloat16, device=q.device).permute(0, 2, 1, 3)
        attention128_bwd_raw(q, k, v, o, do, lse, dq, dk, dv, ctx.scale, o_res8=o_res8)
        return dq, dk, dv, None, None, None


def attention128(q, k, v, scale=None, o_pad=0, precise_delta="int8"):
    if precise_delta not in (None, "int8"):
        raise ValueError('attention128: precise_delta is "int8" or None (the bf16 residual form exists at head_dim 64 only)')
    return _Attention128Fn.apply(q, k, v, q.shape[-1] ** -0.5 if scale is None else scale, int(o_pad), precise_delta)


class _QKNormAttentionFn(torch.autograd.Function):

    @staticmethod
    def forward(ctx, qkv, wq, bq, wk, bk, rope_cos, rope_sin, text_len, H, eps, o_pad, grad_pad, rope_mode=0, recompute_qk=False, precise_delta=None, fwd_policy=None):
        _req(qkv, torch.bfloat16)
        B, S, W = qkv.shape
        Dh = W // (3 * H)
        qkv5 = qkv.view(B, S, 3, H, Dh)
        q_in, k_in, v = (qkv5[:, :, i].permute(0, 2, 1, 3) for i in range(3))
        qn = torch.empty(B, H, S, Dh, dtype=torch.bfloat16, device=qkv.device)
        kn = torch.empty_like(qn)
        _timed("qknorm_rope_fwd", 8.0 * B * H * S * Dh, lambda: _lib.call(
            "vgpa_qknorm_rope_fwd", q_in, k_in, qn, kn, _bhs_strides(q_in), _bhs_strides(k_in), _bhs_strides(qn), _bhs_strides(kn),
            wq, bq, wk, bk, rope_cos, rope_sin, text_len, B, H, S, Dh, float(eps), float(Dh ** -0.5 * LOG2E), int(rope_mode), _stream()), "byte")
        o_res = None
        if precise_delta and ctx.needs_input_grad[0]:
            o_res = torch.empty(B, S, H * Dh, dtype=torch.uint8 if precise_delta == "int8" else torch.bfloat16, device=qkv.device)
        o, lse = attention_fwd_raw(qn, kn, v, q_prescaled=True, o_pad=o_pad, o_res=o_res, policy=fwd_policy)
        if recompute_qk:
            ctx.save_for_backward(qkv, o, lse, wq, wk, rope_cos, rope_sin, bq, bk, o_res)
        else:
            ctx.save_for_backward(qkv, qn, kn, o, lse, wq, wk, rope_cos, rope_sin, o_res)
        ctx.meta = (text_len, H, eps, grad_pad, int(rope_mode), bool(recompute_qk))
        return o

    @staticmethod
    def backward(ctx, do):
        text_len, H, eps, grad_pad, rope_mode, recompute_qk = ctx.meta
        if recompute_qk:
            qkv, o, lse, wq, wk, rope_cos, rope_sin, bq, bk, o_res = ctx.saved_tensors
        else:
            qkv, qn, kn, o, lse, wq, wk, rope_cos, rope_sin, o_res = ctx.saved_tensors
        B, S, W = qkv.shape
        Dh = W // (3 * H)
        do = do.contiguous()
        qkv5 = qkv.view(B, S, 3, H, Dh)
        q_in, k_in, v = (qkv5[:, :, i].permute(0, 2, 1, 3) for i in range(3))
        if recompute_qk:
            qn = torch.empty(B, H, S, Dh, dtype=torch.bfloat16, device=qkv.device)
            kn = torch.empty_like(qn)
            _timed("qknorm_rope_fwd", 8.0 * B * H * S * Dh, lambda: _lib.call(
                "vgpa_qknorm_rope_fwd", q_in, k_in, qn, kn, _bhs_strides(q_in), _bhs_strides(k_in), _bhs_strides(qn), _bhs_strides(kn),
                wq, bq, wk, bk, rope_cos, rope_sin, text_len, B, H, S, Dh, float(eps), float(Dh ** -0.5 * LOG2E), int(rope_mode), _stream()), "byte")
        dqkv = _padded_empty((B, S), W, grad_pad, qkv.dtype, qkv.device) if grad_pad else torch.empty_like(qkv)
        d5 = dqkv.unflatten(-1, (3, H, Dh))
        dq_in, dk_in, dv = (d5[:, :, i].permute(0, 2, 1, 3) for i in range(3))
        dqn = torch.empty_like(qn)
        dkn = torch.empty_like(kn)
        ov = o.unflatten(-1, (H, Dh)).permute(0, 2, 1, 3)
        dov = do.view(B, S, H, Dh).permute(0, 2, 1, 3)
        attention_bwd_raw(qn, kn, v, ov, dov, lse, dqn, dkn, dv, q_prescaled=True,
                          o_res=None if o_res is None else o_res.unflatten(-1, (H, Dh)).permute(0, 2, 1, 3))
        _timed("qknorm_rope_bwd", 12.0 * B * H * S * Dh, lambda: _lib.call(
            "vgpa_qknorm_rope_bwd", dqn, dkn, q_in, k_in, dq_in, dk_in, _bhs_strides(dqn), _bhs_strides(dkn), _bhs_strides(q_in),
            _bhs_strides(k_in), _bhs_strides(dq_in), _bhs_strides(dk_in), wq, wk, rope_cos, rope_sin, text_len, B, H, S, Dh,
            float(eps), rope_mode, _stream()), "byte")
        return dqkv, None, None, None, None, None, None, None, None, None, None, None, None, None, None, None


def qknorm_attention(qkv, wq, bq, wk, bk, H, text_len=0, rope=None, eps=1e-6, o_pad=0, grad_pad=0, rope_mode=0, recompute_qk=False, precise_delta="int8", fwd_policy=None):
    cos, sin = (None, None) if rope is None else rope
    if precise_delta not in (None, "int8", "bf16"):
        raise ValueError(f'precise_delta: "int8", "bf16" or None, got {precise_delta!r}')
    return _QKNormAttentionFn.apply(qkv, wq, bq, wk, bk, cos, sin, text_len, H, eps, o_pad, grad_pad, rope_mode, bool(recompute_qk), precise_delta, fwd_policy)


def rope2d_tables(pos, head_dim=64, frequency=100.0):
    half = head_dim // 2
    inv = 1.0 / (frequency ** (torch.arange(0, half, 2, device=pos.device).float() / half))
    ang = pos.float()[:, :, None] * inv[None, None, :]
    ang = torch.cat([ang, ang], dim=-1).reshape(pos.shape[0], head_dim)
    return ang.cos().contiguous(), ang.sin().contiguous()


def _heads_in(*ts):
    for t in ts:
        if t is None:
            continue
        _req(t, torch.float32)
        if torch.is_grad_enabled() and t.requires_grad:
            raise RuntimeError("the fp32 head kernels are forward only: call them under torch.no_grad()")


def pack_conv_weight(w):
    return w.detach().float().permute(2, 3, 1, 0).contiguous()


def conv3x3_f32(x, w_packed, bias=None, res=None, res2=None, relu_in=False, relu_res=False, stride=1):
    _heads_in(x, w_packed, bias, res, res2)
    N, H, W, Cin = x.shape
    Cout = w_packed.shape[-1]
    if tuple(w_packed.shape) != (3, 3, Cin, Cout) or Cin % 16 or Cout % 16:
        raise RuntimeError(f"conv3x3_f32: weight {tuple(w_packed.shape)} does not fit input channels {Cin} (multiples of 16)")
    Ho, Wo = (H - 1) // stride + 1, (W - 1) // stride + 1
    out = torch.empty(N, Ho, Wo, Cout, device=x.device, dtype=torch.float32)
    for r in (res, res2):
        if r is not None and r.shape != out.shape:
            raise RuntimeError("conv3x3_f32: residual shape differs from the output's")
    _timed("conv3x3_f32", 2.0 * out.numel() * 9 * Cin,
           lambda: _lib.call("vgpa_conv3x3_f32", x, w_packed, bias, res, res2, out, N, H, W, Cin, Cout, stride,
                             (1 if relu_in else 0) | (2 if relu_res else 0), _stream()))
    return out


def conv1x1_f32(x, w_packed, bias=None):
    _heads_in(x, w_packed, bias)
    Cin, Cout = w_packed.shape
    if x.shape[-1] != Cin or Cin % 16 or Cout % 16:
        raise RuntimeError(f"conv1x1_f32: weight {tuple(w_packed.shape)} does not fit input {tuple(x.shape)} (channels in multiples of 16)")
    out = torch.empty(*x.shape[:-1], Cout, device=x.device, dtype=torch.float32)
    M = out.numel() // Cout
    _timed("conv1x1_f32", 2.0 * M * Cin * Cout, lambda: _lib.call("vgpa_conv1x1_f32", x, w_packed, bias, out, M, Cin, Cout, _stream()))
    return out


def uv_embed_tables(width, height, channels, aspect_ratio, device, ratio=0.1, f32_angles=False):
    if channels % 8:
        raise RuntimeError("uv_embed_tables: channels must be a multiple of 8")
    diag = (aspect_ratio ** 2 + 1.0) ** 0.5
    span_x, span_y = aspect_ratio / diag, 1.0 / diag
    xs = torch.linspace(-span_x * (width - 1) / width, span_x * (width - 1) / width, steps=width, dtype=torch.float32)
    ys = torch.linspace(-span_y * (height - 1) / height, span_y * (height - 1) / height, steps=height, dtype=torch.float32)
    half = channels // 2
    adt = torch.float32 if f32_angles else torch.float64
    omega = torch.arange(half // 2, dtype=adt)
    omega /= half / 2.0
    omega = 1.0 / 100 ** omega

    def table(pos):
        ang = torch.einsum("m,d->md", pos.to(adt), omega)
        return (torch.cat([ang.sin(), ang.cos()], dim=1).float() * ratio).contiguous().to(device)
    return table(xs), table(ys)


def upsample_bilinear_ac_f32(x, H, W, tabs=None):
    xt, yt = tabs if tabs is not None else (None, None)
    _heads_in(x, xt, yt)
    N, h, w, C = x.shape
    if xt is not None and (tuple(xt.shape) != (W, C // 2) or tuple(yt.shape) != (H, C // 2)):
        raise RuntimeError("upsample_bilinear_ac_f32: embedding tables do not fit the output")
    out = torch.empty(N, H, W, C, device=x.device, dtype=torch.float32)
    _timed("upsample_bilinear_ac_f32", 4.0 * out.numel(), lambda: _lib.call("vgpa_upsample_bilinear_ac_f32", x, xt, yt, out, N, h, w, C, H, W, _stream()),
           unit="byte")
    return out


_DPT_ACT = {"exp": 0, "inv_log": 1}


def _tail_fits(name, x, H, W, w1_packed, w2, xt, yt, grid):
    C, od = x.shape[3], w2.shape[0]
    if tuple(w1_packed.shape) != (3, 3, C, 32) or tuple(w2.shape) != (od, 32) or C % 16:
        raise RuntimeError(f"{name}: weights do not fit the input")
    if xt is not None and (tuple(xt.shape) != (W, C // 2) or tuple(yt.shape) != (H, C // 2)):
        raise RuntimeError(f"{name}: embedding tables do not fit the {grid}")


def dpt_tail_f32(x, H, W, w1_packed, b1, w2, b2, activation="exp", tabs=None):
    xt, yt = tabs if tabs is not None else (None, None)
    _heads_in(x, xt, yt, w1_packed, b1, w2, b2)
    if activation not in _DPT_ACT:
        raise NotImplementedError(f"dpt_tail_f32: activation {activation!r} (exp and inv_log are built)")
    N, h, w, C = x.shape
    od = w2.shape[0]
    _tail_fits("dpt_tail_f32", x, H, W, w1_packed, w2, xt, yt, "output")
    preds = torch.empty(N, H, W, od - 1, device=x.device, dtype=torch.float32)
    conf = torch.empty(N, H, W, device=x.device, dtype=torch.float32)
    _timed("dpt_tail_f32", 2.0 * N * H * W * (9 * C * 32 + 32 * od),
           lambda: _lib.call("vgpa_dpt_tail_f32", x, xt, yt, w1_packed, b1, w2, b2, preds, conf, N, h, w, C, H, W, od, _DPT_ACT[activation], _stream()))
    return preds, conf

# ... 221 lines not shown
```

Baseline: 0.4520 pair-steps/s.

## Fuse key-max into qknorm-rope forward and batch LoRA down/grad kernels

```diff
diff --git a/include/videogpa_hip.h b/include/videogpa_hip.h
--- a/include/videogpa_hip.h
+++ b/include/videogpa_hip.h
@@ -71,6 +71,13 @@
                              const float* wq, const float* bq, const float* wk, const float* bk, const float* rope_cos,
                              const float* rope_sin, int64_t text_len, int64_t B, int64_t H, int64_t S, int64_t head_dim,
                              float eps, float q_out_scale, int32_t rope_mode, vgpa_stream_t stream);
+size_t vgpa_qknorm_rope_fwd_kmax_workspace_bytes(int64_t B, int64_t H, int64_t S);
+int32_t vgpa_qknorm_rope_fwd_kmax(const void* q_in, const void* k_in, void* q_out, void* k_out, const int64_t* qin_strides,
+                                  const int64_t* kin_strides, const int64_t* qout_strides, const int64_t* kout_strides,
+                                  const float* wq, const float* bq, const float* wk, const float* bk, const float* rope_cos,
+                                  const float* rope_sin, int64_t text_len, int64_t B, int64_t H, int64_t S, int64_t head_dim,
+                                  float eps, float q_out_scale, int32_t rope_mode, uint32_t* kmax2, void* workspace, size_t ws_bytes,
+                                  vgpa_stream_t stream);
 int32_t vgpa_qknorm_rope_bwd(const void* dq_out, const void* dk_out, const void* q_in, const void* k_in, void* dq_in,
                              void* dk_in, const int64_t* dqout_strides, const int64_t* dkout_strides,
                              const int64_t* qin_strides, const int64_t* kin_strides, const int64_t* dqin_strides,
@@ -94,6 +101,10 @@
                              const int64_t* k_strides, const int64_t* v_strides, const int64_t* o_strides, const int64_t* ores_strides,
                              int64_t B, int64_t H, int64_t S, int64_t head_dim, float scale, int32_t split_mode, void* workspace,
                              size_t ws_bytes, vgpa_stream_t stream);
+int32_t vgpa_attn_fwd_w1_res_kmax(const void* q, const void* k, const void* v, void* o, void* o_res, int32_t res_kind, float* lse2, const int64_t* q_strides,
+                                  const int64_t* k_strides, const int64_t* v_strides, const int64_t* o_strides, const int64_t* ores_strides,
+                                  int64_t B, int64_t H, int64_t S, int64_t head_dim, float scale, int32_t split_mode, void* workspace,
+                                  size_t ws_bytes, const uint32_t* kmax2, vgpa_stream_t stream);
 int32_t vgpa_attn_fwd_online_res(const void* q, const void* k, const void* v, void* o, void* o_res, int32_t res_kind, float* lse2, const int64_t* q_strides,
                                  const int64_t* k_strides, const int64_t* v_strides, const int64_t* o_strides, const int64_t* ores_strides,
                                  int64_t B, int64_t H, int64_t S, int64_t head_dim, float scale, int32_t split_mode, void* workspace,
@@ -108,11 +119,17 @@
 
 int32_t vgpa_lora_down(const void* X, int64_t ldx, const void* A, void* T, int64_t ldt, int64_t M, int64_t K, int64_t R,
                        vgpa_stream_t stream);
+int32_t vgpa_lora_down_batched(const void* X, int64_t ldx, int64_t x_slice, const void* A, int64_t a_slice, void* T, int64_t ldt, int64_t t_slice,
+                               int64_t n_slices, int64_t M, int64_t K, int64_t R, vgpa_stream_t stream);
 int32_t vgpa_lora_up_add(void* Y, int64_t ldy, const void* T, int64_t ldt, const void* Bw, int64_t ldb, float s, int64_t M,
                          int64_t N, int64_t rp, int32_t accumulate, vgpa_stream_t stream);
 size_t vgpa_lora_grad_workspace_bytes(int64_t M, int64_t P, int64_t Q);
 int32_t vgpa_lora_grad_ws(const void* U, int64_t ldu, const void* V, int64_t ldv, float* G, int64_t ldg, float s, int64_t M,
                           int64_t P, int64_t Q, void* workspace, size_t ws_bytes, vgpa_stream_t stream);
+size_t vgpa_lora_grad_batched_workspace_bytes(int64_t n_slices, int64_t M, int64_t P, int64_t Q);
+int32_t vgpa_lora_grad_batched_ws(const void* U, int64_t ldu, int64_t u_slice, const void* V, int64_t ldv, int64_t v_slice, float* G, int64_t ldg,
+                                  int64_t g_slice, const float* s, int64_t n_slices, int64_t M, int64_t P, int64_t Q, void* workspace, size_t ws_bytes,
+                                  vgpa_stream_t stream);
 int32_t vgpa_lora_ext_refresh(const float* A, const float* B, float s, int64_t r, int64_t K, int64_t Dn, void* a_cat, void* wt_tail, int64_t ld_wt,
                               void* w_tail, int64_t ld_w, void* sbt, vgpa_stream_t stream);
 
diff --git a/videogpa_amd/_lib.py b/videogpa_amd/_lib.py
--- a/videogpa_amd/_lib.py
+++ b/videogpa_amd/_lib.py
@@ -26,6 +26,8 @@
     "vgpa_gelu_tanh_fwd": (I32, [P, I64, P, P]),
     "vgpa_gelu_tanh_bwd": (I32, [P, P, I64, P, P]),
     "vgpa_qknorm_rope_fwd": (I32, [P, P, P, P, P, P, P, P, P, P, P, P, P, P, I64, I64, I64, I64, I64, F32, F32, I32, P]),
+    "vgpa_qknorm_rope_fwd_kmax_workspace_bytes": (SZ, [I64, I64, I64]),
+    "vgpa_qknorm_rope_fwd_kmax": (I32, [P, P, P, P, P, P, P, P, P, P, P, P, P, P, I64, I64, I64, I64, I64, F32, F32, I32, P, P, SZ, P]),
     "vgpa_qknorm_rope_bwd": (I32, [P, P, P, P, P, P, P, P, P, P, P, P, P, P, P, P, I64, I64, I64, I64, I64, F32, I32, P]),
     "vgpa_grad_norm_workspace_bytes": (SZ, []),
     "vgpa_grad_norm": (I32, [P, I64, F32, P, P, SZ, P]),
@@ -35,13 +37,17 @@
     "vgpa_attn_fwd_w1_workspace_bytes": (SZ, [I64, I64, I64]),
     "vgpa_attn_bwd_prep_w1_res": (I32, [P, P, I32, P, P, P, P, P, P, P, I64, I64, I64, I64, P]),
     "vgpa_attn_fwd_w1_res": (I32, [P, P, P, P, P, I32, P, P, P, P, P, P, I64, I64, I64, I64, F32, I32, P, SZ, P]),
+    "vgpa_attn_fwd_w1_res_kmax": (I32, [P, P, P, P, P, I32, P, P, P, P, P, P, I64, I64, I64, I64, F32, I32, P, SZ, P, P]),
     "vgpa_attn_fwd_online_res": (I32, [P, P, P, P, P, I32, P, P, P, P, P, P, I64, I64, I64, I64, F32, I32, P, SZ, P]),
     "vgpa_attn_bwd_dkv_w1": (I32, [P, P, P, P, P, P, P, P, P, P, P, P, P, I64, I64, I64, I64, F32, I32, P, SZ, P]),
     "vgpa_attn_bwd_split_workspace_bytes": (SZ, [I64, I64, I64]),
     "vgpa_lora_down": (I32, [P, I64, P, P, I64, I64, I64, I64, P]),
+    "vgpa_lora_down_batched": (I32, [P, I64, I64, P, I64, P, I64, I64, I64, I64, I64, I64, P]),
     "vgpa_lora_up_add": (I32, [P, I64, P, I64, P, I64, F32, I64, I64, I64, I32, P]),
     "vgpa_lora_grad_workspace_bytes": (SZ, [I64, I64, I64]),
     "vgpa_lora_grad_ws": (I32, [P, I64, P, I64, P, I64, F32, I64, I64, I64, P, SZ, P]),
+    "vgpa_lora_grad_batched_workspace_bytes": (SZ, [I64, I64, I64, I64]),
+    "vgpa_lora_grad_batched_ws": (I32, [P, I64, I64, P, I64, I64, P, I64, I64, P, I64, I64, I64, I64, P, SZ, P]),
     "vgpa_lora_ext_refresh": (I32, [P, P, F32, I64, I64, I64, P, P, I64, P, I64, P, P]),
     "vgpa_attn128_fwd_workspace_bytes": (SZ, [I64, I64, I64]),
     "vgpa_attn128_fwd": (I32, [P, P, P, P, P, P, P, P, P, P, P, I64, I64, I64, I64, F32, P, SZ, P]),
diff --git a/videogpa_amd/csrc/attention_w1.hip b/videogpa_amd/csrc/attention_w1.hip
--- a/videogpa_amd/csrc/attention_w1.hip
+++ b/videogpa_amd/csrc/attention_w1.hip
@@ -600,7 +600,7 @@
 static int32_t fwd_w1_impl(const void* q, const void* k, const void* v, void* o, void* o_res, int32_t res_kind, float* lse2, const int64_t* q_strides,
                            const int64_t* k_strides, const int64_t* v_strides, const int64_t* o_strides, const int64_t* ores_strides, int64_t B,
                            int64_t H, int64_t S, int64_t head_dim, float scale, int32_t split_mode, void* workspace, size_t ws_bytes,
-                           hipStream_t stream, bool force_online) {
+                           hipStream_t stream, bool force_online, const uint32_t* kmax_given = nullptr) {
     (void)scale;
     if (!q || !k || !v || !o || !lse2 || !workspace || head_dim != HD || B <= 0 || H <= 0 || S <= 0 || S > (1 << 24)) return VGPA_ERR_INVALID;
     if (!view_ok(q_strides, B, H, S, HD) || !view_ok(k_strides, B, H, S, HD) || !view_ok(v_strides, B, H, S, HD) || !view_ok(o_strides, B, H, S, HD) ||
@@ -619,7 +619,7 @@
     const int n_qt = pl.n_t;
     const int64_t tasks = pl.tasks;
     const TailSplit& p = pl.p;
-    unsigned* kmax2 = (unsigned*)workspace;
+    const unsigned* kmax2 = kmax_given ? (const unsigned*)kmax_given : (const unsigned*)workspace;
     int* flags = (int*)workspace + B * H;
     float* part = (float*)((char*)workspace + head);
     if (S < W1_FWD_MIN_S || force_online) {
@@ -627,9 +627,13 @@
         return vgpa_internal_attn_fwd_redo(q, k, v, o, lse2, mk(q_strides), mk(k_strides), mk(v_strides), mk(o_strides), (int)S, (int)H, n_qt, tasks,
                                            flags, stream, ores, sor, rk);
     }
-    if (hipMemsetAsync(workspace, 0, head, stream) != hipSuccess) return VGPA_ERR_LAUNCH;
-    VGPA_LAUNCH((w1_kmax_kernel<HD / 8>), dim3(16, (unsigned)(B * H)), dim3(256), 0, stream, (const bf16_t*)k, mk(k_strides), (int)S, (int)H, kmax2);
-    VGPA_CHECK_LAUNCH();
+    if (kmax_given) {
+        if (hipMemsetAsync(flags, 0, head - (size_t)(B * H) * 4, stream) != hipSuccess) return VGPA_ERR_LAUNCH;
+    } else {
+        if (hipMemsetAsync(workspace, 0, head, stream) != hipSuccess) return VGPA_ERR_LAUNCH;
+        VGPA_LAUNCH((w1_kmax_kernel<HD / 8>), dim3(16, (unsigned)(B * H)), dim3(256), 0, stream, (const bf16_t*)k, mk(k_strides), (int)S, (int)H, (unsigned*)workspace);
+        VGPA_CHECK_LAUNCH();
+    }
     if (p.n_main > 0) {
         VGPA_LAUNCH((attn_fwd_w1_kernel<false>), dim3((unsigned)p.n_main), dim3(256), 0, stream, (const bf16_t*)q, (const bf16_t*)k, (const bf16_t*)v,
                     (bf16_t*)o, lse2, (const unsigned*)kmax2, flags, mk(q_strides), mk(k_strides), mk(v_strides), mk(o_strides), (int)S, (int)H, n_qt, 0, 1,
@@ -655,6 +659,14 @@
     return fwd_w1_impl(q, k, v, o, o_res, res_kind, lse2, q_strides, k_strides, v_strides, o_strides, ores_strides, B, H, S, head_dim, scale, split_mode, workspace,
                        ws_bytes, stream, false);
 }
+int32_t vgpa_attn_fwd_w1_res_kmax(const void* q, const void* k, const void* v, void* o, void* o_res, int32_t res_kind, float* lse2, const int64_t* q_strides,
+                                  const int64_t* k_strides, const int64_t* v_strides, const int64_t* o_strides, const int64_t* ores_strides, int64_t B,
+                                  int64_t H, int64_t S, int64_t head_dim, float scale, int32_t split_mode, void* workspace, size_t ws_bytes,
+                                  const uint32_t* kmax2, hipStream_t stream) {
+    if (!kmax2 || ((uintptr_t)kmax2 & 3)) return VGPA_ERR_INVALID;
+    return fwd_w1_impl(q, k, v, o, o_res, res_kind, lse2, q_strides, k_strides, v_strides, o_strides, ores_strides, B, H, S, head_dim, scale, split_mode, workspace,
+                       ws_bytes, stream, false, kmax2);
+}
 int32_t vgpa_attn_fwd_online_res(const void* q, const void* k, const void* v, void* o, void* o_res, int32_t res_kind, float* lse2, const int64_t* q_strides,
                                  const int64_t* k_strides, const int64_t* v_strides, const int64_t* o_strides, const int64_t* ores_strides, int64_t B,
                                  int64_t H, int64_t S, int64_t head_dim, float scale, int32_t split_mode, void* workspace, size_t ws_bytes,
diff --git a/videogpa_amd/csrc/attn_w1.h b/videogpa_amd/csrc/attn_w1.h
--- a/videogpa_amd/csrc/attn_w1.h
+++ b/videogpa_amd/csrc/attn_w1.h
@@ -256,9 +256,7 @@
         const int row = (int)(i >> SH), c = (int)(i & (LANES_PER_ROW - 1));
         float f[8];
         unpack8(*reinterpret_cast<const u32x4_t*>(Kb + ((size_t)row * sk.s + c * 8)), f);
-        float a = 0.f;
-#pragma unroll
-        for (int j = 0; j < 8; ++j) a += f[j] * f[j];
+        float a = sumsq8(f);
         a += __shfl_xor(a, 1, 64);
         a += __shfl_xor(a, 2, 64);
         a += __shfl_xor(a, 4, 64);
diff --git a/videogpa_amd/csrc/common.h b/videogpa_amd/csrc/common.h
--- a/videogpa_amd/csrc/common.h
+++ b/videogpa_amd/csrc/common.h
@@ -53,6 +53,12 @@
 #pragma unroll
     for (int i = 0; i < 4; ++i) v[i] = pack_bf16x2(f[2 * i], f[2 * i + 1]);
     return v;
+}
+__device__ __forceinline__ float sumsq8(const float* f) {
+    float a = f[0] * f[0];
+#pragma unroll
+    for (int j = 1; j < 8; ++j) a = __builtin_fmaf(f[j], f[j], a);
+    return a;
 }
 
 #define VGPA_RES_NONE 0
diff --git a/videogpa_amd/csrc/lora.hip b/videogpa_amd/csrc/lora.hip
--- a/videogpa_amd/csrc/lora.hip
+++ b/videogpa_amd/csrc/lora.hip
@@ -27,10 +27,15 @@
     }
 }
 
+struct LoraSlices { int64_t x, a, t; };
+
 template <int NCB>
 __global__ __launch_bounds__(256) void lora_down_kernel(const bf16_t* __restrict__ X, int64_t ldx, const bf16_t* __restrict__ A,
-                                                          bf16_t* __restrict__ T, int64_t ldt, int64_t M, int K, int R) {
+                                                          bf16_t* __restrict__ T, int64_t ldt, int64_t M, int K, int R, LoraSlices sl) {
     extern __shared__ __attribute__((aligned(16))) bf16_t smem[];
+    X += (int64_t)blockIdx.y * sl.x;
+    A += (int64_t)blockIdx.y * sl.a;
+    T += (int64_t)blockIdx.y * sl.t;
     constexpr int RP = 32 * NCB;
     constexpr int NACC = (NCB + 1) / 2;
     constexpr int BUF = (64 + RP) * PITCH;
@@ -116,10 +121,13 @@
 
 template <int NCB, int NS>
 __global__ __launch_bounds__(256) void lora_down_dma_kernel(const bf16_t* __restrict__ X, int64_t ldx, const bf16_t* __restrict__ A, bf16_t* __restrict__ T,
-                                                              int64_t ldt, int64_t M, int K, int R) {
+                                                              int64_t ldt, int64_t M, int K, int R, LoraSlices sl) {
     constexpr int RP = 32 * NCB;
     constexpr int NACC = (NCB + 1) / 2;
     constexpr int STAGE = 8192 + RP * 128;
+    X += (int64_t)blockIdx.y * sl.x;
+    A += (int64_t)blockIdx.y * sl.a;
+    T += (int64_t)blockIdx.y * sl.t;
     constexpr int PW = 2 + NCB;
     __shared__ __attribute__((aligned(1024))) uint8_t lds[NS * STAGE];
     const int lane = threadIdx.x & 63, hi = lane >> 5;
@@ -258,10 +266,18 @@
     }
 }
 
+#define LORA_MAX_SLICES 4
+struct LoraGradSlices { int64_t u, v, g, part; };
+struct LoraScales { float s[LORA_MAX_SLICES]; };
+
 __global__ __launch_bounds__(256) void lora_grad_kernel(const bf16_t* __restrict__ U, int64_t ldu, const bf16_t* __restrict__ V, int64_t ldv,
                                                           float* __restrict__ G, int64_t ldg, float s, int64_t M, int P, int Q,
-                                                          int64_t rows_per_split, int n_qt, float* __restrict__ part) {
+                                                          int64_t rows_per_split, int n_qt, float* __restrict__ part, LoraGradSlices sl) {
     __shared__ __attribute__((aligned(16))) bf16_t lds[4 * TILE_ELEMS];
+    U += (int64_t)blockIdx.z * sl.u;
+    V += (int64_t)blockIdx.z * sl.v;
+    G += (int64_t)blockIdx.z * sl.g;
+    if (part) part += (int64_t)blockIdx.z * sl.part;
     const int lane = threadIdx.x & 63, wave = threadIdx.x >> 6, hi = lane >> 5;
     const int pb = wave & 1, qb = wave >> 1;
     const int p0 = (blockIdx.x / n_qt) * 64, q0 = (blockIdx.x % n_qt) * 64;
@@ -308,10 +324,13 @@
     }
 }
 
-__global__ __launch_bounds__(256) void lora_grad_merge_kernel(const float* __restrict__ part, int nsplit, float* __restrict__ G, int64_t ldg, float s,
-                                                                int P, int Q) {
+__global__ __launch_bounds__(256) void lora_grad_merge_kernel(const float* __restrict__ part, int nsplit, float* __restrict__ G, int64_t ldg, LoraScales sc,
+                                                                int P, int Q, LoraGradSlices sl) {
     const int64_t i = (int64_t)blockIdx.x * 256 + threadIdx.x;
     if (i >= (int64_t)P * Q) return;
+    part += (int64_t)blockIdx.y * sl.part;
+    G += (int64_t)blockIdx.y * sl.g;
+    const float s = sc.s[blockIdx.y];
     float a = 0.f;
     for (int c = 0; c < nsplit; ++c) a += part[(int64_t)c * P * Q + i];
     G[(i / Q) * ldg + (i % Q)] = s * a;
@@ -340,15 +359,16 @@
 
 extern "C" {
 
-int32_t vgpa_lora_down(const void* X, int64_t ldx, const void* A, void* T, int64_t ldt, int64_t M, int64_t K, int64_t R, hipStream_t stream) {
+static int32_t lora_down_impl(const void* X, int64_t ldx, const void* A, void* T, int64_t ldt, int64_t M, int64_t K, int64_t R, LoraSlices sl, int64_t n_slices,
+                              hipStream_t stream) {
     if (!X || !A || !T || M <= 0 || K <= 0 || K % 64 != 0 || R <= 0 || R > 256 || ldx % 8 || ldt % 8 || ldt < R || !a16(X) || !a16(A)) return VGPA_ERR_INVALID;
     if (M > ((int64_t)1 << 31) * 32) return VGPA_ERR_INVALID;
     const int ncb = (int)((R + 31) / 32);
-    const dim3 grid((unsigned)((M + 63) / 64));
+    const dim3 grid((unsigned)((M + 63) / 64), (unsigned)n_slices);
     constexpr bool dma_off = LORA_DOWN_DMA == 0;
     constexpr int dma_max_ncb = LORA_DOWN_DMA_NCB;
     if (!dma_off && ncb <= dma_max_ncb && (uint64_t)64 * (uint64_t)ldx * 2 + (uint64_t)K * 2 + 1024 < (1ull << 32) && ((uint64_t)R + 8) * (uint64_t)K * 2 + 1024 < (1ull << 32)) {
-#define LDD(N, S) VGPA_LAUNCH((lora_down_dma_kernel<N, S>), grid, dim3(256), 0, stream, (const bf16_t*)X, ldx, (const bf16_t*)A, (bf16_t*)T, ldt, M, (int)K, (int)R)
+#define LDD(N, S) VGPA_LAUNCH((lora_down_dma_kernel<N, S>), grid, dim3(256), 0, stream, (const bf16_t*)X, ldx, (const bf16_t*)A, (bf16_t*)T, ldt, M, (int)K, (int)R, sl)
         constexpr int ns = LORA_DOWN_NS;
         switch (ncb * 10 + ns) {
             case 14: LDD(1, 4); break; case 24: LDD(2, 4); break;
@@ -364,7 +384,7 @@
 #define LD(N)                                                                                                                      \
     if (hipFuncSetAttribute((const void*)lora_down_kernel<N>, hipFuncAttributeMaxDynamicSharedMemorySize, (int)shmem) != hipSuccess) \
         return VGPA_ERR_LAUNCH;                                                                                                    \
-    VGPA_LAUNCH((lora_down_kernel<N>), grid, dim3(256), shmem, stream, (const bf16_t*)X, ldx, (const bf16_t*)A, (bf16_t*)T, ldt, M, (int)K, (int)R)
+    VGPA_LAUNCH((lora_down_kernel<N>), grid, dim3(256), shmem, stream, (const bf16_t*)X, ldx, (const bf16_t*)A, (bf16_t*)T, ldt, M, (int)K, (int)R, sl)
     switch (ncb) {
         case 1: LD(1); break; case 2: LD(2); break; case 3: LD(3); break; case 4: LD(4); break;
         case 5: LD(5); break; case 6: LD(6); break; case 7: LD(7); break; case 8: LD(8); break;
@@ -373,6 +393,14 @@
 #undef LD
     VGPA_CHECK_LAUNCH();
     return VGPA_OK;
+}
+int32_t vgpa_lora_down(const void* X, int64_t ldx, const void* A, void* T, int64_t ldt, int64_t M, int64_t K, int64_t R, hipStream_t stream) {
+    return lora_down_impl(X, ldx, A, T, ldt, M, K, R, LoraSlices{0, 0, 0}, 1, stream);
+}
+int32_t vgpa_lora_down_batched(const void* X, int64_t ldx, int64_t x_slice, const void* A, int64_t a_slice, void* T, int64_t ldt, int64_t t_slice,
+                               int64_t n_slices, int64_t M, int64_t K, int64_t R, hipStream_t stream) {
+    if (n_slices <= 0 || n_slices > 65535 || x_slice % 8 || a_slice % 8 || t_slice % 8) return VGPA_ERR_INVALID;
+    return lora_down_impl(X, ldx, A, T, ldt, M, K, R, LoraSlices{x_slice, a_slice, t_slice}, n_slices, stream);
 }
 
 int32_t vgpa_lora_up_add(void* Y, int64_t ldy, const void* T, int64_t ldt, const void* Bw, int64_t ldb, float s, int64_t M, int64_t N,
@@ -412,21 +440,41 @@
     lora_grad_plan(M, P, Q, &n_pt, &n_qt, &rows, &splits);
     return (size_t)splits * (size_t)P * (size_t)Q * sizeof(float);
 }
-int32_t vgpa_lora_grad_ws(const void* U, int64_t ldu, const void* V, int64_t ldv, float* G, int64_t ldg, float s, int64_t M, int64_t P,
-                          int64_t Q, void* workspace, size_t ws_bytes, hipStream_t stream) {
+static int32_t lora_grad_impl(const void* U, int64_t ldu, const void* V, int64_t ldv, float* G, int64_t ldg, LoraScales sc, int64_t M, int64_t P, int64_t Q,
+                              void* workspace, size_t ws_bytes, LoraGradSlices sl, int64_t n_slices, hipStream_t stream) {
     if (!U || !V || !G || !workspace || M <= 0 || P <= 0 || Q <= 0 || P % 8 || Q % 8 || ldu % 8 || ldv % 8 || !a16(U) || !a16(V) || !a16(workspace))
         return VGPA_ERR_INVALID;
     int n_pt, n_qt;
     int64_t rows, splits;
     lora_grad_plan(M, P, Q, &n_pt, &n_qt, &rows, &splits);
-    if (ws_bytes < (size_t)splits * (size_t)P * (size_t)Q * sizeof(float)) return VGPA_ERR_WORKSPACE;
-    VGPA_LAUNCH(lora_grad_kernel, dim3((unsigned)(n_pt * n_qt), (unsigned)splits), dim3(256), 0, stream, (const bf16_t*)U, ldu, (const bf16_t*)V, ldv,
-                G, ldg, s, M, (int)P, (int)Q, rows, n_qt, (float*)workspace);
+    if (ws_bytes < (size_t)n_slices * (size_t)splits * (size_t)P * (size_t)Q * sizeof(float)) return VGPA_ERR_WORKSPACE;
+    sl.part = splits * P * Q;
+    const size_t pad_lds = n_slices > 1 ? 16384 : 0;
+    VGPA_LAUNCH(lora_grad_kernel, dim3((unsigned)(n_pt * n_qt), (unsigned)splits, (unsigned)n_slices), dim3(256), pad_lds, stream, (const bf16_t*)U, ldu,
+                (const bf16_t*)V, ldv, G, ldg, 1.f, M, (int)P, (int)Q, rows, n_qt, (float*)workspace, sl);
     VGPA_CHECK_LAUNCH();
-    VGPA_LAUNCH(lora_grad_merge_kernel, dim3((unsigned)((P * Q + 255) / 256)), dim3(256), 0, stream, (const float*)workspace, (int)splits, G, ldg, s,
-                (int)P, (int)Q);
+    VGPA_LAUNCH(lora_grad_merge_kernel, dim3((unsigned)((P * Q + 255) / 256), (unsigned)n_slices), dim3(256), 0, stream, (const float*)workspace, (int)splits, G,
+                ldg, sc, (int)P, (int)Q, sl);
     VGPA_CHECK_LAUNCH();
     return VGPA_OK;
+}
+int32_t vgpa_lora_grad_ws(const void* U, int64_t ldu, const void* V, int64_t ldv, float* G, int64_t ldg, float s, int64_t M, int64_t P,
+                          int64_t Q, void* workspace, size_t ws_bytes, hipStream_t stream) {
+    LoraScales sc = {};
+    sc.s[0] = s;
+    return lora_grad_impl(U, ldu, V, ldv, G, ldg, sc, M, P, Q, workspace, ws_bytes, LoraGradSlices{0, 0, 0, 0}, 1, stream);
+}
+size_t vgpa_lora_grad_batched_workspace_bytes(int64_t n_slices, int64_t M, int64_t P, int64_t Q) {
+    if (n_slices <= 0) return 0;
+    return (size_t)n_slices * vgpa_lora_grad_workspace_bytes(M, P, Q);
+}
+int32_t vgpa_lora_grad_batched_ws(const void* U, int64_t ldu, int64_t u_slice, const void* V, int64_t ldv, int64_t v_slice, float* G, int64_t ldg,
+                                  int64_t g_slice, const float* s, int64_t n_slices, int64_t M, int64_t P, int64_t Q, void* workspace, size_t ws_bytes,
+                                  hipStream_t stream) {
+    if (!s || n_slices <= 0 || n_slices > LORA_MAX_SLICES || u_slice % 8 || v_slice % 8) return VGPA_ERR_INVALID;
+    LoraScales sc = {};
+    for (int64_t i = 0; i < n_slices; ++i) sc.s[i] = s[i];
+    return lora_grad_impl(U, ldu, V, ldv, G, ldg, sc, M, P, Q, workspace, ws_bytes, LoraGradSlices{u_slice, v_slice, g_slice, 0}, n_slices, stream);
 }
 
 int32_t vgpa_lora_ext_refresh(const float* A, const float* B, float s, int64_t r, int64_t K, int64_t Dn, void* a_cat, void* wt_tail, int64_t ld_wt, void* w_tail,
diff --git a/videogpa_amd/csrc/qknorm.hip b/videogpa_amd/csrc/qknorm.hip
--- a/videogpa_amd/csrc/qknorm.hip
+++ b/videogpa_amd/csrc/qknorm.hip
@@ -7,6 +7,62 @@
     v += __shfl_xor(v, 2, 64);
     v += __shfl_xor(v, 4, 64);
     return v;
+}
+template <int CTRL>
+__device__ __forceinline__ float dpp_lane(float v) {
+    return __int_as_float(__builtin_amdgcn_update_dpp(__float_as_int(v), __float_as_int(v), CTRL, 0xf, 0xf, false));
+}
+__device__ __forceinline__ float group8_sum_dpp(float v) {
+    v += dpp_lane<0xB1>(v);
+    v += dpp_lane<0x4E>(v);
+    v += dpp_lane<0x141>(v);
+    return v;
+}
+
+template <bool DPP>
+__device__ __forceinline__ u32x4_t qknorm_rope_row(const u32x4_t raw, bf16_t* op, const float* w, const float* bb, const float* __restrict__ rope_cos,
+                                                   const float* __restrict__ rope_sin, int which, int s, int c8, int text_len, float eps, float q_out_scale,
+                                                   int rope_mode) {
+    float x[8];
+    unpack8(raw, x);
+    float sum = 0.f;
+#pragma unroll
+    for (int j = 0; j < 8; ++j) sum += x[j];
+    const float mean = (DPP ? group8_sum_dpp(sum) : group8_sum(sum)) * (1.f / 64.f);
+    float sq = 0.f;
+#pragma unroll
+    for (int j = 0; j < 8; ++j) { const float d = x[j] - mean; sq += d * d; }
+    const float rstd = rsqrtf((DPP ? group8_sum_dpp(sq) : group8_sum(sq)) * (1.f / 64.f) + eps);
+    float y[8];
+#pragma unroll
+    for (int j = 0; j < 8; ++j) y[j] = (x[j] - mean) * rstd * w[c8 * 8 + j] + bb[c8 * 8 + j];
+    if (rope_cos && rope_mode == 1) {
+        const bool on = s >= text_len;
+        const float* cp = rope_cos + (int64_t)(on ? s - text_len : 0) * 64 + c8 * 8;
+        const float* sp = rope_sin + (int64_t)(on ? s - text_len : 0) * 64 + c8 * 8;
+        const float sgn = (c8 & 2) ? 1.f : -1.f;
+#pragma unroll
+        for (int j = 0; j < 8; ++j) {
+            const float partner = __shfl_xor(y[j], 2, 64);
+            if (on) y[j] = y[j] * cp[j] + sgn * partner * sp[j];
+        }
+    } else if (rope_cos && s >= text_len) {
+        const float* cp = rope_cos + (int64_t)(s - text_len) * 64 + c8 * 8;
+        const float* sp = rope_sin + (int64_t)(s - text_len) * 64 + c8 * 8;
+#pragma unroll
+        for (int j = 0; j < 8; j += 2) {
+            const float a = y[j], bq2 = y[j + 1];
+            y[j] = a * cp[j] - bq2 * sp[j];
+            y[j + 1] = bq2 * cp[j + 1] + a * sp[j + 1];
+        }
+    }
+    if (!which) {
+#pragma unroll
+        for (int j = 0; j < 8; ++j) y[j] *= q_out_scale;
+    }
+    const u32x4_t packed = pack8(y);
+    *reinterpret_cast<u32x4_t*>(op + c8 * 8) = packed;
+    return packed;
 }
 
 __global__ __launch_bounds__(256) void qknorm_rope_fwd_kernel(const bf16_t* __restrict__ q_in, const bf16_t* __restrict__ k_in,
@@ -28,46 +84,63 @@
     const int b = (int)(r / (uint32_t)S);
     const bf16_t* ip = which ? (k_in + b * si_k.b + h * si_k.h + (int64_t)s * si_k.s) : (q_in + b * si_q.b + h * si_q.h + (int64_t)s * si_q.s);
     bf16_t* op = which ? (k_out + b * so_k.b + h * so_k.h + (int64_t)s * so_k.s) : (q_out + b * so_q.b + h * so_q.h + (int64_t)s * so_q.s);
-    const float* w = which ? wk : wq;
-    const float* bb = which ? bk : bq;
-    float x[8];
-    unpack8(*reinterpret_cast<const u32x4_t*>(ip + c8 * 8), x);
-    float sum = 0.f;
-#pragma unroll
-    for (int j = 0; j < 8; ++j) sum += x[j];
-    const float mean = group8_sum(sum) * (1.f / 64.f);
-    float sq = 0.f;
-#pragma unroll
-    for (int j = 0; j < 8; ++j) { const float d = x[j] - mean; sq += d * d; }
-    const float rstd = rsqrtf(group8_sum(sq) * (1.f / 64.f) + eps);
-    float y[8];
-#pragma unroll
-    for (int j = 0; j < 8; ++j) y[j] = (x[j] - mean) * rstd * w[c8 * 8 + j] + bb[c8 * 8 + j];
-    if (rope_cos && rope_mode == 1) {
-        const bool on = s >= text_len;
-        const float* cp = rope_cos + (int64_t)(on ? s - text_len : 0) * 64 + c8 * 8;
-        const float* sp = rope_sin + (int64_t)(on ? s - text_len : 0) * 64 + c8 * 8;
-        const float sgn = (c8 & 2) ? 1.f : -1.f;
-#pragma unroll
-        for (int j = 0; j < 8; ++j) {
-            const float partner = __shfl_xor(y[j], 2, 64);
-            if (on) y[j] = y[j] * cp[j] + sgn * partner * sp[j];
-        }
-    } else if (rope_cos && s >= text_len) {
-        const float* cp = rope_cos + (int64_t)(s - text_len) * 64 + c8 * 8;
-        const float* sp = rope_sin + (int64_t)(s - text_len) * 64 + c8 * 8;
-#pragma unroll
-        for (int j = 0; j < 8; j += 2) {
-            const float a = y[j], bq2 = y[j + 1];
-            y[j] = a * cp[j] - bq2 * sp[j];
-            y[j + 1] = bq2 * cp[j + 1] + a * sp[j + 1];
-        }
-    }
-    if (!which) {
-#pragma unroll
-        for (int j = 0; j < 8; ++j) y[j] *= q_out_scale;
-    }
-    *reinterpret_cast<u32x4_t*>(op + c8 * 8) = pack8(y);
+    qknorm_rope_row<false>(*reinterpret_cast<const u32x4_t*>(ip + c8 * 8), op, which ? wk : wq, which ? bk : bq, rope_cos, rope_sin, which, s, c8, text_len, eps, q_out_scale, rope_mode);
+}
+
+__global__ __launch_bounds__(256) void qknorm_rope_fwd_norms_kernel(const bf16_t* __restrict__ q_in, const bf16_t* __restrict__ k_in,
+                                                                      bf16_t* __restrict__ q_out, bf16_t* __restrict__ k_out, QStride si_q,
+                                                                      QStride si_k, QStride so_q, QStride so_k, const float* __restrict__ wq,
+                                                                      const float* __restrict__ bq, const float* __restrict__ wk,
+                                                                      const float* __restrict__ bk, const float* __restrict__ rope_cos,
+                                                                      const float* __restrict__ rope_sin, int text_len, int B, int H, int S,
+                                                                      float eps, float q_out_scale, int rope_mode, float* __restrict__ knorm2) {
+    const int64_t nvec = (int64_t)B * S * H;
+    const int64_t gid = (int64_t)blockIdx.x * 256 + threadIdx.x;
+    const int64_t vid = gid >> 3;
+    const int c8 = (int)(gid & 7);
+    if (vid >= 2 * nvec) return;
+    const int which = vid >= nvec;
+    uint32_t r = (uint32_t)(which ? vid - nvec : vid);
+    const uint32_t row = r;
+    const int h = (int)(r % (uint32_t)H); r /= (uint32_t)H;
+    const int s = (int)(r % (uint32_t)S);
+    const int b = (int)(r / (uint32_t)S);
+    const bf16_t* ip = which ? (k_in + b * si_k.b + h * si_k.h + (int64_t)s * si_k.s) : (q_in + b * si_q.b + h * si_q.h + (int64_t)s * si_q.s);
+    bf16_t* op = which ? (k_out + b * so_k.b + h * so_k.h + (int64_t)s * so_k.s) : (q_out + b * so_q.b + h * so_q.h + (int64_t)s * so_q.s);
+    const u32x4_t packed = qknorm_rope_row<true>(*reinterpret_cast<const u32x4_t*>(ip + c8 * 8), op, which ? wk : wq, which ? bk : bq, rope_cos, rope_sin, which, s, c8,
+                                                 text_len, eps, q_out_scale, rope_mode);
+    if (which) {
+        float f[8];
+        unpack8(packed, f);
+        const float a = group8_sum_dpp(sumsq8(f));
+        if (c8 == 0) knorm2[row] = a;
+    }
+}
+
+#define QKN_REDUCE_ELEMS 8192
+#define QKN_KMAX_MAX_HEADS 1024
+__global__ __launch_bounds__(256) void qknorm_kmax_reduce_kernel(const float* __restrict__ knorm2, int H, int S, unsigned* __restrict__ kmax2) {
+    __shared__ unsigned lmax[QKN_KMAX_MAX_HEADS];
+    const int b = blockIdx.y;
+    for (int i = threadIdx.x; i < H; i += 256) lmax[i] = 0u;
+    __syncthreads();
+    const int64_t n = (int64_t)S * H;
+    const float* src = knorm2 + (int64_t)b * n;
+    const int64_t e0 = (int64_t)blockIdx.x * QKN_REDUCE_ELEMS + threadIdx.x;
+#pragma unroll 8
+    for (int i = 0; i < QKN_REDUCE_ELEMS / 256; ++i) {
+        const int64_t e = e0 + 256 * i;
+        if (e < n) {
+            const float a = src[e];
+            if (a > 0.f) atomicMax(&lmax[(uint32_t)(e % H)], __float_as_uint(a));
+        }
+    }
+    __syncthreads();
+    for (int i = threadIdx.x; i < H; i += 256) {
+        const unsigned v = lmax[i];
+        unsigned* kp = kmax2 + b * H + i;
+        if (v > 0u && v > __hip_atomic_load(kp, __ATOMIC_RELAXED, __HIP_MEMORY_SCOPE_AGENT)) atomicMax(kp, v);
+    }
 }
 
 __global__ __launch_bounds__(256) void qknorm_rope_bwd_kernel(const bf16_t* __restrict__ dq_out, const bf16_t* __restrict__ dk_out,
@@ -143,21 +216,53 @@
 
 extern "C" {
 
+static int32_t qknorm_fwd_impl(const void* q_in, const void* k_in, void* q_out, void* k_out, const int64_t* qin_strides, const int64_t* kin_strides,
+                               const int64_t* qout_strides, const int64_t* kout_strides, const float* wq, const float* bq, const float* wk, const float* bk,
+                               const float* rope_cos, const float* rope_sin, int64_t text_len, int64_t B, int64_t H, int64_t S, int64_t head_dim, float eps,
+                               float q_out_scale, int32_t rope_mode, uint32_t* kmax2, float* knorm2, hipStream_t stream) {
+    if (!q_in || !k_in || !q_out || !k_out || !wq || !bq || !wk || !bk || head_dim != 64 || B <= 0 || H <= 0 || S <= 0) return VGPA_ERR_INVALID;
+    if (!qs_ok(qin_strides) || !qs_ok(kin_strides) || !qs_ok(qout_strides) || !qs_ok(kout_strides)) return VGPA_ERR_INVALID;
+    if ((rope_cos == nullptr) != (rope_sin == nullptr) || text_len < 0 || text_len > S || (rope_mode != 0 && rope_mode != 1)) return VGPA_ERR_INVALID;
+    const int64_t threads = 2 * B * S * H * 8;
+    if (2 * B * S * H >= ((int64_t)1 << 31) || threads / 256 >= ((int64_t)1 << 31)) return VGPA_ERR_INVALID;
+#define QKN_ARGS                                                                                                                                   \
+    (const bf16_t*)q_in, (const bf16_t*)k_in, (bf16_t*)q_out, (bf16_t*)k_out, qmk(qin_strides), qmk(kin_strides), qmk(qout_strides), qmk(kout_strides), wq, bq, \
+        wk, bk, rope_cos, rope_sin, (int)text_len, (int)B, (int)H, (int)S, eps, q_out_scale, (int)rope_mode
+    if (kmax2) {
+        if (H > QKN_KMAX_MAX_HEADS || B > 65535) return VGPA_ERR_INVALID;
+        if (hipMemsetAsync(kmax2, 0, (size_t)(B * H) * sizeof(uint32_t), stream) != hipSuccess) return VGPA_ERR_LAUNCH;
+        VGPA_LAUNCH(qknorm_rope_fwd_norms_kernel, dim3((unsigned)((threads + 255) / 256)), dim3(256), 0, stream, QKN_ARGS, knorm2);
+        VGPA_CHECK_LAUNCH();
+        VGPA_LAUNCH(qknorm_kmax_reduce_kernel, dim3((unsigned)((S * H + QKN_REDUCE_ELEMS - 1) / QKN_REDUCE_ELEMS), (unsigned)B), dim3(256), 0, stream,
+                    (const float*)knorm2, (int)H, (int)S, (unsigned*)kmax2);
+    } else {
+        VGPA_LAUNCH(qknorm_rope_fwd_kernel, dim3((unsigned)((threads + 255) / 256)), dim3(256), 0, stream, QKN_ARGS);
+    }
+#undef QKN_ARGS
+    VGPA_CHECK_LAUNCH();
+    return VGPA_OK;
+}
 int32_t vgpa_qknorm_rope_fwd(const void* q_in, const void* k_in, void* q_out, void* k_out, const int64_t* qin_strides,
                              const int64_t* kin_strides, const int64_t* qout_strides, const int64_t* kout_strides, const float* wq,
                              const float* bq, const float* wk, const float* bk, const float* rope_cos, const float* rope_sin,
                              int64_t text_len, int64_t B, int64_t H, int64_t S, int64_t head_dim, float eps, float q_out_scale,
                              int32_t rope_mode, hipStream_t stream) {
-    if (!q_in || !k_in || !q_out || !k_out || !wq || !bq || !wk || !bk || head_dim != 64 || B <= 0 || H <= 0 || S <= 0) return VGPA_ERR_INVALID;
-    if (!qs_ok(qin_strides) || !qs_ok(kin_strides) || !qs_ok(qout_strides) || !qs_ok(kout_strides)) return VGPA_ERR_INVALID;
-    if ((rope_cos == nullptr) != (rope_sin == nullptr) || text_len < 0 || text_len > S || (rope_mode != 0 && rope_mode != 1)) return VGPA_ERR_INVALID;
-    const int64_t threads = 2 * B * S * H * 8;
-    if (2 * B * S * H >= ((int64_t)1 << 31) || threads / 256 >= ((int64_t)1 << 31)) return VGPA_ERR_INVALID;
-    VGPA_LAUNCH(qknorm_rope_fwd_kernel, dim3((unsigned)((threads + 255) / 256)), dim3(256), 0, stream, (const bf16_t*)q_in,
-                       (const bf16_t*)k_in, (bf16_t*)q_out, (bf16_t*)k_out, qmk(qin_strides), qmk(kin_strides), qmk(qout_strides),
-                       qmk(kout_strides), wq, bq, wk, bk, rope_cos, rope_sin, (int)text_len, (int)B, (int)H, (int)S, eps, q_out_scale, (int)rope_mode);
-    VGPA_CHECK_LAUNCH();
-    return VGPA_OK;
+    return qknorm_fwd_impl(q_in, k_in, q_out, k_out, qin_strides, kin_strides, qout_strides, kout_strides, wq, bq, wk, bk, rope_cos, rope_sin, text_len, B, H, S,
+                           head_dim, eps, q_out_scale, rope_mode, nullptr, nullptr, stream);
+}
+size_t vgpa_qknorm_rope_fwd_kmax_workspace_bytes(int64_t B, int64_t H, int64_t S) {
+    if (B <= 0 || H <= 0 || S <= 0) return 0;
+    return (size_t)B * (size_t)H * (size_t)S * sizeof(float);
+}
+int32_t vgpa_qknorm_rope_fwd_kmax(const void* q_in, const void* k_in, void* q_out, void* k_out, const int64_t* qin_strides,
+                                  const int64_t* kin_strides, const int64_t* qout_strides, const int64_t* kout_strides, const float* wq,
+                                  const float* bq, const float* wk, const float* bk, const float* rope_cos, const float* rope_sin,
+                                  int64_t text_len, int64_t B, int64_t H, int64_t S, int64_t head_dim, float eps, float q_out_scale,
+                                  int32_t rope_mode, uint32_t* kmax2, void* workspace, size_t ws_bytes, hipStream_t stream) {
+    if (!kmax2 || ((uintptr_t)kmax2 & 3) || !workspace || ((uintptr_t)workspace & 15)) return VGPA_ERR_INVALID;
+    if (B > 0 && H > 0 && S > 0 && ws_bytes < vgpa_qknorm_rope_fwd_kmax_workspace_bytes(B, H, S)) return VGPA_ERR_WORKSPACE;
+    return qknorm_fwd_impl(q_in, k_in, q_out, k_out, qin_strides, kin_strides, qout_strides, kout_strides, wq, bq, wk, bk, rope_cos, rope_sin, text_len, B, H, S,
+                           head_dim, eps, q_out_scale, rope_mode, kmax2, (float*)workspace, stream);
 }
 
 int32_t vgpa_qknorm_rope_bwd(const void* dq_out, const void* dk_out, const void* q_in, const void* k_in, void* dq_in, void* dk_in,
diff --git a/videogpa_amd/ops.py b/videogpa_amd/ops.py
--- a/videogpa_amd/ops.py
+++ b/videogpa_amd/ops.py
@@ -381,6 +381,52 @@
     _timed("lora_down_kernel", 2.0 * M * (K + R), lambda: _lib.call("vgpa_lora_down", x2, x2.stride(0), a_cat, t, t.stride(0), M, K, R, _stream()),
            "byte")
     return t
+
+
+def _slice_step(views):
+    v0 = views[0]
+    if any(v.shape != v0.shape or v.stride() != v0.stride() or v.dtype != v0.dtype or v.untyped_storage().data_ptr() != v0.untyped_storage().data_ptr()
+           for v in views[1:]):
+        return None
+    step = views[1].storage_offset() - v0.storage_offset()
+    if any(v.storage_offset() != v0.storage_offset() + i * step for i, v in enumerate(views)):
+        return None
+    return step
+
+
+LORA_BATCH_MAX = 4
+
+
+def lora_down_batched(xs, a_s, outs):
+    n = len(xs)
+    if n < 2 or n > LORA_BATCH_MAX or any(not a.is_contiguous() for a in a_s):
+        return False
+    sx, sa, st = _slice_step(xs), _slice_step(a_s), _slice_step(outs)
+    if sx is None or sa is None or st is None or sx % 8 or sa % 8 or st % 8 or xs[0].stride(1) != 1 or outs[0].stride(1) != 1:
+        return False
+    M, K = xs[0].shape
+    R = a_s[0].shape[0]
+    _timed("lora_down_kernel", 2.0 * n * M * (K + R), lambda: _lib.call("vgpa_lora_down_batched", xs[0], xs[0].stride(0), sx, a_s[0], sa, outs[0], outs[0].stride(0),
+                                                                       st, n, M, K, R, _stream()), "byte")
+    return True
+
+
+def lora_grad_batched(us, vs, scales):
+    n = len(us)
+    if n < 2 or n > LORA_BATCH_MAX:
+        return None
+    su, sv = _slice_step(us), _slice_step(vs)
+    if su is None or sv is None or su % 8 or sv % 8 or us[0].stride(1) != 1 or vs[0].stride(1) != 1:
+        return None
+    M, P = us[0].shape
+    Q = vs[0].shape[1]
+    g = torch.empty(n, P, Q, dtype=torch.float32, device=us[0].device)
+    ws_bytes = _lib.query("vgpa_lora_grad_batched_workspace_bytes", n, M, P, Q)
+    ws = torch.empty(ws_bytes, dtype=torch.uint8, device=us[0].device)
+    sc = (ctypes.c_float * n)(*[float(x) for x in scales])
+    _timed("lora_grad_kernel", 2.0 * n * M * (P + Q), lambda: _lib.call("vgpa_lora_grad_batched_ws", us[0], us[0].stride(0), su, vs[0], vs[0].stride(0), sv, g, Q,
+                                                                       P * Q, sc, n, M, P, Q, ws, ws_bytes, _stream()), "byte")
+    return g
 
 
 def lora_up_add(y2, t, bw, s, accumulate=True):
@@ -835,8 +881,11 @@
             dy_ext = torch.zeros(M, N + R, dtype=dy.dtype, device=dy.device) if not enabled else torch.empty(M, N + R, dtype=dy.dtype, device=dy.device)
             dy_ext[:, :N].copy_(dy2)
         if enabled:
-            for j, i in enumerate(act):
-                lora_down(dy_ext[:, i * Dn:(i + 1) * Dn], ext.sBt[j], out=dy_ext[:, N + j * rp:N + (j + 1) * rp])
+            dys = [dy_ext[:, i * Dn:(i + 1) * Dn] for i in act]
+            dts = [dy_ext[:, N + j * rp:N + (j + 1) * rp] for j in range(len(act))]
+            if not lora_down_batched(dys, [ext.sBt[j] for j in range(len(act))], dts):
+                for j in range(len(act)):
+                    lora_down(dys[j], ext.sBt[j], out=dts[j])
         dx = _gemm(dy_ext, ext.Wt_ext, ext=True, split=ctx.rows_per_call)
         out_grads = [None] * len(ctx.needs_input_grad[6:])
         if enabled:
@@ -844,8 +893,10 @@
                 t_all, xh = saved, ctx.x_fn(*srcs).reshape(M, K)
             else:
                 t_all, xh = saved[:, K:], saved[:, :K]
+            ts = [t_all[:, j * rp:(j + 1) * rp] for j in range(len(act))]
+            dB = lora_grad_batched(dys, ts, ctx.scalings)
             for j, i in enumerate(act):
-                out_grads[2 * i + 1] = lora_grad(dy_ext[:, i * Dn:(i + 1) * Dn], t_all[:, j * rp:(j + 1) * rp], ctx.scalings[j])[:, :r]
+                out_grads[2 * i + 1] = (lora_grad(dys[j], ts[j], ctx.scalings[j]) if dB is None else dB[j])[:, :r]
             dA = lora_grad(dy_ext[:, N:], xh)
             for j, i in enumerate(act):
                 out_grads[2 * i] = dA[j * rp:j * rp + r]
@@ -939,7 +990,7 @@
     return float((_strip_flags(ws, B * H, B, H, S) != 0).float().mean())
 
 
-def attention_fwd_raw(q, k, v, scale=None, q_prescaled=False, split_mode=None, o_pad=0, o_res=None, policy=None):
+def attention_fwd_raw(q, k, v, scale=None, q_prescaled=False, split_mode=None, o_pad=0, o_res=None, policy=None, kmax2=None):
     B, H, S, Dh = q.shape
     scale = Dh ** -0.5 if scale is None else scale
     if not q_prescaled:
@@ -952,9 +1003,14 @@
     ws = torch.empty(ws_bytes, dtype=torch.uint8, device=q.device)
     rv = None if o_res is None else o_res.unflatten(-1, (H, Dh)).permute(0, 2, 1, 3)
     entry = "vgpa_attn_fwd_online_res" if (policy is not None and policy.mode == "online") else "vgpa_attn_fwd_w1_res"
+    extra = ()
+    if kmax2 is not None and entry == "vgpa_attn_fwd_w1_res":
+        if kmax2.dtype != torch.int32 or kmax2.numel() != B * H or not kmax2.is_contiguous():
+            raise TypeError("attention_fwd_raw: kmax2 is a contiguous int32 [B*H] tensor")
+        entry, extra = "vgpa_attn_fwd_w1_res_kmax", (kmax2,)
     _timed("attn_fwd_kernel", 4.0 * S * S * Dh * B * H, lambda: _lib.call(
         entry, q, k, v, o, o_res, _res_kind(o_res), lse, _bhs_strides(q), _bhs_strides(k), _bhs_strides(v), _bhs_strides(ov), None if rv is None else _bhs_strides(rv),
-        B, H, S, Dh, float(scale), int(split_mode), ws, ws_bytes, _stream()))
+        B, H, S, Dh, float(scale), int(split_mode), ws, ws_bytes, *extra, _stream()))
     if policy is not None:
         if policy.wants_flags() and not torch.cuda.is_current_stream_capturing():
             policy.observe(attention_redo_fraction(ws, B, H, S))
@@ -1122,13 +1178,19 @@
         q_in, k_in, v = (qkv5[:, :, i].permute(0, 2, 1, 3) for i in range(3))
         qn = torch.empty(B, H, S, Dh, dtype=torch.bfloat16, device=qkv.device)
         kn = torch.empty_like(qn)
+        kmax2, kx = None, ()
+        if not (fwd_policy is not None and fwd_policy.mode == "online") and H <= 1024:
+            kmax2 = torch.empty(B * H, dtype=torch.int32, device=qkv.device)
+            nws = _lib.query("vgpa_qknorm_rope_fwd_kmax_workspace_bytes", B, H, S)
+            kx = (kmax2, torch.empty(nws, dtype=torch.uint8, device=qkv.device), nws)
         _timed("qknorm_rope_fwd", 8.0 * B * H * S * Dh, lambda: _lib.call(
-            "vgpa_qknorm_rope_fwd", q_in, k_in, qn, kn, _bhs_strides(q_in), _bhs_strides(k_in), _bhs_strides(qn), _bhs_strides(kn),
-            wq, bq, wk, bk, rope_cos, rope_sin, text_len, B, H, S, Dh, float(eps), float(Dh ** -0.5 * LOG2E), int(rope_mode), _stream()), "byte")
+            "vgpa_qknorm_rope_fwd" if kmax2 is None else "vgpa_qknorm_rope_fwd_kmax", q_in, k_in, qn, kn, _bhs_strides(q_in), _bhs_strides(k_in), _bhs_strides(qn),
+            _bhs_strides(kn), wq, bq, wk, bk, rope_cos, rope_sin, text_len, B, H, S, Dh, float(eps), float(Dh ** -0.5 * LOG2E), int(rope_mode),
+            *kx, _stream()), "byte")
         o_res = None
         if precise_delta and ctx.needs_input_grad[0]:
             o_res = torch.empty(B, S, H * Dh, dtype=torch.uint8 if precise_delta == "int8" else torch.bfloat16, device=qkv.device)
-        o, lse = attention_fwd_raw(qn, kn, v, q_prescaled=True, o_pad=o_pad, o_res=o_res, policy=fwd_policy)
+        o, lse = attention_fwd_raw(qn, kn, v, q_prescaled=True, o_pad=o_pad, o_res=o_res, policy=fwd_policy, kmax2=kmax2)
         if recompute_qk:
             ctx.save_for_backward(qkv, o, lse, wq, wk, rope_cos, rope_sin, bq, bk, o_res)
         else:
```

After: 0.4519 pair-steps/s. No clear change (-0.0%).
